# sebhaan/geobo

Measured on AMD Instinct MI355X. Metric: voxels/sec posterior (mean+var) for 64^3 x 2-prop joint inversion; fp64 roofline %, higher is better.
Workload: dtype f64

## Files before the change

geobo_amd/_lib.py:

```python
import ctypes as C
import os

LIB_PATH = os.environ.get("GEOBO_HIP_LIB") or os.path.join(os.path.dirname(os.path.abspath(__file__)), "lib", "libgeobo_hip.so")

_dp = C.c_void_p
_i64 = C.c_int64
_f64 = C.c_double
_int = C.c_int
_sz = C.c_size_t

SIGNATURES = {
    "geobo_version": (_int, []),
    "geobo_pad_m": (_i64, [_i64]),
    "geobo_pad_n": (_i64, [_i64]),
    "geobo_k_block": (_int, [_int, _dp, _dp, _dp, _i64, _dp, _dp, _dp, _i64, _f64, _f64, _f64, _f64, _dp, _i64, _dp]),
    "geobo_k_block_f32": (_int, [_int, _dp, _dp, _dp, _i64, _dp, _dp, _dp, _i64, _f64, _f64, _f64, _f64, _dp, _i64, _dp]),
    "geobo_k_block_grid": (_int, [_int, _int, _int, _dp, _dp, _i64, _i64, _i64, _i64, _int, _dp, _i64, _dp]),
    "geobo_lattice_wbuild": (_int, [_i64, _int, _int, _int, _dp, _dp, _dp, _dp]),
    "geobo_lattice_wplanes": (_int, [_i64, _int, _int, _int, _dp, _dp, _dp, _dp]),
    "geobo_xz2d_fold_inv_strided": (_int, [_int, _i64, _int, _dp, _i64, _i64, _dp, _dp, _dp, _i64, _i64, _i64, _dp]),
    "geobo_xz2d_fold_inv_mul": (_int, [_int, _i64, _int, _dp, _i64, _dp, _i64, _dp, _dp, _dp, _i64, _i64, _i64, _dp]),
    "geobo_xz2d_fold_conv_fwd": (_int, [_int, _i64, _int, _dp, _i64, _dp, _i64, _dp, _i64, _dp, _dp, _dp, _i64, _i64, _dp]),
    "geobo_sumsq_accum": (_int, [_i64, _i64, _dp, _i64, _dp, _i64, _int, _dp, _i64, _dp]),
    "geobo_lamdot_z": (_int, [_i64, _int, _int, _int, _dp, _dp, _dp, _dp]),
    "geobo_centro_fill": (_int, [_dp, _i64, _i64, _i64, _dp]),
    "geobo_transpose": (_int, [_i64, _i64, _dp, _i64, _dp, _i64, _dp]),
    "geobo_mirror_rows": (_int, [_dp, _i64, _i64, _i64, _i64, _int, _dp]),
    "geobo_mirror_dev_ws_bytes": (_sz, []),
    "geobo_mirror_dev": (_int, [_dp, _i64, _dp, _i64, _i64, _int, _int, _dp, _dp, _sz, _dp]),
    "geobo_colgemv_ws_bytes": (_sz, [_i64, _i64]),
    "geobo_colgemv": (_int, [_i64, _i64, _dp, _i64, _dp, _dp, _dp, _sz, _dp]),
    "geobo_rowgemv": (_int, [_i64, _i64, _dp, _i64, _dp, _dp, _dp]),
    "geobo_convert": (_int, [_int, _dp, _i64, _dp, _i64, _i64, _i64, _dp]),
    "geobo_round_f32": (_int, [_dp, _i64, _dp]),
    "geobo_k_eval": (_int, [_int, _dp, _i64, _f64, _f64, _f64, _f64, _dp, _dp]),
    "geobo_a_sens": (_int, [_int, C.POINTER(_f64), _dp, _i64, _int, _int, _int, _dp, _dp, _dp, _f64, _f64, _dp, _i64, _dp]),
    "geobo_a_sens_slab": (_int, [_int, C.POINTER(_f64), _dp, _i64, _int, _int, _int, _dp, _dp, _dp, _f64, _f64, _int, _int, _dp, _i64, _i64, _dp]),
    "geobo_potential": (_int, [_int, C.POINTER(_f64), _dp, _dp, _dp, _i64, _dp, _dp]),
    "geobo_ak_fused": (_int, [_int, _dp, _i64, _i64, _i64, _dp, _dp, _dp, _i64, _i64, _f64, _f64, _f64, _f64, _dp, _i64, _dp]),
    "geobo_ak_points": (_int, [_int, _dp, _i64, _i64, _i64, _dp, _dp, _dp, _dp, _dp, _dp, _i64, _f64, _f64, _f64, _f64, _dp, _i64, _dp]),
    "geobo_cov_table": (_int, [_int, _int, _int, _int, _f64, _f64, _f64, _f64, _f64, _f64, _f64, _dp, _dp]),
    "geobo_ak_fused_grid": (_int, [_dp, _i64, _i64, _i64, _int, _int, _int, _dp, _i64, _i64, _dp, _i64, _dp]),
    "geobo_gemm_nt": (_int, [_i64, _i64, _i64, _f64, _dp, _i64, _dp, _i64, _f64, _dp, _i64, _int, _i64, _dp]),
    "geobo_tile_order": (_i64, [_int, _int, _int, _int, _int, _int, _int, C.POINTER(_int), _i64]),
    "geobo_gemm_map": (_int, [_int, _int, _int, _int, _int, _int, _int, _int, C.POINTER(_int)]),
    "geobo_gemm_nt_splitk": (_int, [_i64, _i64, _i64, _int, _dp, _i64, _dp, _i64, _dp, _i64, _int, _i64, _dp, _sz, _dp]),
    "geobo_gemm_nn": (_int, [_i64, _i64, _i64, _f64, _dp, _i64, _dp, _i64, _f64, _dp, _i64, _int, _int, _dp]),
    "geobo_gemm_batched": (_int, [_int, _i64, _i64, _i64, _f64, _dp, _i64, _i64, _dp, _i64, _i64, _f64, _dp, _i64, _i64, _i64, _i64, _int, _dp]),
    "geobo_gemm_fold_lamdot": (_int, [_i64, _i64, _i64, _dp, _i64, _dp, _i64, _i64, _dp, _int, _i64, _dp, _i64, _dp]),
    "geobo_gemm_fold": (_int, [_int, _int, _i64, _i64, _i64, _dp, _i64, _i64, _dp, _i64, _i64, _dp, _i64, _i64, _i64, _i64, _i64, _dp]),
    "geobo_scale_broadcast": (_int, [_dp, _dp, _i64, _i64, _dp, _dp]),
    "geobo_scale_broadcast2": (_int, [_dp, _dp, _dp, _i64, _i64, _dp, _dp, _dp]),
    "geobo_a_sens_lattice_ws_bytes": (_sz, [_int, _int, _int]),
    "geobo_a_sens_lattice": (_int, [_int, C.POINTER(_f64), _i64, _int, _int, _int, _dp, _dp, _dp, _dp, _dp, _f64, _f64, _int, _int, _dp, _i64,
                                    _i64, _dp, _sz, _dp]),
    "geobo_xz2d": (_int, [_int, _int, _int, _i64, _int, _dp, _i64, _i64, _dp, _i64, _dp, _i64, _dp, _i64, _i64, _dp]),
    "geobo_xz2d_fold": (_int, [_int, _int, _i64, _int, _dp, _i64, _i64, _dp, _dp, _dp, _i64, _i64, _dp]),
    "geobo_xz2d_fold_quad": (_int, [_int, _int, _i64, _int, _dp, _i64, _i64, _dp, _dp, _dp, _i64, _i64, _dp]),
    "geobo_xcorr_reduce_fold": (_int, [_int, _i64, _int, _dp, _i64, _i64, _dp, _dp, _dp, _i64, _i64, _dp]),
    "geobo_xz2d_fold_lattice": (_int, [_int, _i64, _int, _dp, _dp, _i64, _dp, _i64, _dp, _dp, _dp, _i64, _i64, _dp]),
    "geobo_xz2d_fold_inv_ss_slots": (_int, [_int, _i64, _int]),
    "geobo_xz2d_fold_inv_ss": (_int, [_int, _i64, _int, _dp, _i64, _i64, _dp, _i64, _i64, _dp, _dp, _dp, _dp]),
    "geobo_ymul": (_int, [_int, _int, _i64, _i64, _dp, _i64, _dp, _i64, _dp, _i64, _dp]),
    "geobo_ymul_fold": (_int, [_int, _int, _i64, _i64, _dp, _i64, _dp, _i64, _dp, _i64, _dp]),
    "geobo_xcorr_reduce": (_int, [_int, _int, _i64, _int, _dp, _i64, _i64, _dp, _i64, _dp, _dp, _i64, _i64, _dp]),
    "geobo_toeplitz_y": (_int, [_int, _i64, _i64, _i64, _int, _dp, _dp, _dp, _dp, _dp, _int, _int, _dp]),
    "geobo_toeplitz_y2t": (_int, [_int, _i64, _i64, _i64, _dp, _dp, _dp, _dp, _dp, _dp, _dp, _dp, _dp]),
    "geobo_toeplitz_y2s": (_int, [_int, _i64, _i64, _i64, _dp, _dp, _dp, _dp, _dp, _dp, _dp, _dp]),
    "geobo_toeplitz_y3": (_int, [_int, _i64, _i64, _i64, _int, _dp, C.POINTER(_dp), C.POINTER(_dp), _int, _int, _dp]),
    "geobo_toeplitz_y3_add": (_int, [_int, _i64, _i64, _i64, _int, _dp, C.POINTER(_dp), C.POINTER(_dp), _int, _int, _dp]),
    "geobo_spectral_y_basis_doubles": (_i64, [_int]),
    "geobo_spectral_y_basis": (_int, [_int, _dp, _dp]),
    "geobo_spectral_y": (_int, [_int, _i64, _i64, _i64, _int, _dp, _dp, _dp, _dp, _dp, _int, _int, _dp, _dp]),
    "geobo_spectral_y_lattice": (_int, [_int, _i64, _i64, _i64, _int, _dp, _dp, _dp, _i64, _dp, _dp, _dp, _dp, _dp, _int, _int, _dp, _dp]),
    "geobo_spectral_y2s": (_int, [_int, _i64, _i64, _i64, _dp, _dp, _dp, _dp, _dp, _dp, _dp, _dp, _dp]),
    "geobo_spectral_y3": (_int, [_int, _i64, _i64, _i64, _int, _dp, C.POINTER(_dp), C.POINTER(_dp), _int, _int, _int, _dp, _dp]),
    "geobo_spectral_y3t": (_int, [_int, _i64, _i64, _i64, _int, _dp, _dp, C.POINTER(_dp), C.POINTER(_dp), C.POINTER(_dp), _dp, _dp]),
    "geobo_spectral_axis": (_int, [_int, _int, _i64, _i64, _i64, _i64, _i64, _i64, _dp, _dp, _dp, _int, _dp]),
    "geobo_potrf_ws_bytes": (_sz, [_i64]),
    "geobo_potrf_ctx_create": (_int, [C.POINTER(C.c_void_p)]),
    "geobo_potrf_ctx_destroy": (_int, [_dp]),
    "geobo_potrf_inv": (_int, [_i64, _dp, _i64, _dp, _i64, _dp, _dp, _sz, _dp, _int, _dp]),
    "geobo_posterior_ws_bytes": (_sz, [_i64, _i64]),
    "geobo_posterior_reduce": (_int, [_i64, _i64, _dp, _i64, _dp, _i64, _dp, _f64, _dp, _dp, _i64, _dp, _sz, _dp]),
    "geobo_kinv_dot_ws_bytes": (_sz, [_i64, _int]),
    "geobo_kinv_dot": (_int, [_i64, _dp, _i64, _dp, _int, C.POINTER(_dp), _i64, C.POINTER(_i64), _dp, _dp, _sz, _dp]),
    "geobo_philox_fill": (_int, [_int, C.c_uint64, C.c_uint64, _i64, _i64, _i64, _i64, C.c_uint64, _dp, _dp]),
    "geobo_torus_table": (_int, [_int, _int, _int, _int, _f64, _f64, _f64, _f64, _f64, _f64, _f64, _dp, _dp]),
    "geobo_fft_lines": (_int, [_int, _i64]),
    "geobo_fft_axis": (_int, [_int, _i64, _int, _i64, _int, _int, _dp, _dp, _int, _i64, _i64, _dp]),
    "geobo_sample_factor_ws_bytes": (_sz, []),
    "geobo_sample_factor": (_int, [_int, _int, _int, _int, _dp, _dp, _dp, _dp, _sz, _dp, _dp]),
    "geobo_sample_zpass": (_int, [_int, _i64, _i64, _int, _int, _int, _int, _dp, _dp, C.c_uint64, _dp, _dp]),
    "geobo_spectral_mix": (_int, [_int, _i64, _int, _int, _int, _dp, _f64, _dp, _dp, _dp]),
    "geobo_set_gram": (_int, [_i64, _int, _dp, _i64, _dp, _i64, _i64, _int, _dp, _dp]),
    "geobo_set_logdet": (_int, [_i64, _int, _dp, _dp, _i64, _f64, _dp, _dp, _i64, _dp, _dp, _dp]),
    "geobo_kinv_diag_ws_bytes": (_sz, [_i64]),
    "geobo_kinv_diag": (_int, [_i64, _dp, _i64, _dp, _dp, _dp, _dp, _sz, _dp]),
    "geobo_set_loo": (_int, [_i64, _int, _dp, _dp, _dp, _i64, _dp, _dp, _dp, _dp, _dp, _dp]),
    "geobo_block_cov_ws_bytes": (_sz, [_i64, _int, _int, _int, _int, _int, _int]),
    "geobo_block_cov": (_int, [_i64, _dp, _dp, _dp, _i64, _int, _int, _int, _int, _int, _int, _int, _dp, _dp, _sz, _dp]),
    "geobo_box_means": (_int, [_i64, _dp, _i64, _i64, _int, _int, _int, _int, _int, _int, _dp, _dp, _dp]),
    "geobo_cutoff_stats_ws_bytes": (_sz, [_i64, _i64, _int]),
    "geobo_cutoff_stats": (_int, [_i64, _dp, _i64, _i64, _i64, _int, _int, C.POINTER(_f64), C.POINTER(_f64), _dp, _dp, _dp, _dp, _dp, _dp, _sz, _dp]),
    "geobo_bodies_ws_bytes": (_sz, [_i64, _int, _int, _int, _int]),
    "geobo_bodies": (_int, [_i64, _dp, _i64, _i64, _int, _int, _int, _int, _int, C.POINTER(_f64), C.POINTER(_f64), _dp, _dp, _int, _i64, _i64,
                            C.POINTER(C.c_int32), _dp, _dp, _dp, _dp, _dp, _dp, _int, _dp, _sz, _dp]),
    "geobo_trace_stats_ws_bytes": (_sz, [_i64, _i64, _int]),
    "geobo_trace_stats": (_int, [_i64, _dp, _i64, _i64, _int, _int, _int, _int, _int, C.POINTER(_f64), C.POINTER(_f64), _dp, _i64, _dp, _dp, _int,
                                 _int, _int, _dp, _dp, _dp, _dp, _dp, _dp, _dp, _dp, _dp, _dp, _dp, _sz, _dp]),
    "geobo_factor_append": (_int, [_int, _dp, _i64, _dp, _i64, _dp, _dp, _i64, _dp, _i64, _dp, _dp, _dp, _dp]),
    "geobo_rows_downdate": (_int, [_dp, _i64, _i64, _i64, _dp, _dp, _dp, _dp]),
    "geobo_trmv_stats": (_int, [_i64, _dp, _i64, _dp, _dp, _i64, _dp, _dp, _dp]),
    "geobo_mfma_f64_peak": (_int, [_int, _int, _dp, _dp]),
    "geobo_mfma_mix": (_int, [_int, _int, _int, _int, _dp, _dp]),
}


class GeoboHipUnavailable(RuntimeError):
    pass


_lib = None


def load():
    global _lib
    if _lib is not None:
        return _lib
    if not os.path.exists(LIB_PATH):
        raise GeoboHipUnavailable(
            "%s not found. Build the HIP extension first: `python -m geobo_amd.build` "
            "(hipcc --offload-arch=gfx950). There is no CPU fallback for the inversion hot path." % LIB_PATH)
    import torch
    try:
        lib = C.CDLL(LIB_PATH)
    except OSError as e:
        raise GeoboHipUnavailable("cannot load %s: %s" % (LIB_PATH, e)) from e
    for name, (res, args) in SIGNATURES.items():
        try:
            fn = getattr(lib, name)
        except AttributeError as e:
            raise GeoboHipUnavailable("libgeobo_hip.so lacks symbol %s (stale build?)" % name) from e
        fn.restype = res
        fn.argtypes = args
    _lib = lib
    return lib
# ... 9 lines not shown
```

geobo_amd/csrc/xz2d.hip:

```cpp
#include <hip/hip_runtime.h>
#include <atomic>
#include <stdint.h>
#include "geobo_hip.h"
#include "lds_optin.h"

namespace {

typedef double v4d __attribute__((ext_vector_type(4)));
typedef double v2d __attribute__((ext_vector_type(2)));
typedef __attribute__((address_space(3))) void* lds_ptr_t;
typedef const __attribute__((address_space(1))) void* glb_ptr_t;

struct XZArgs {
  const double* in; int64_t in_row, in_plane;
  double* out; int64_t out_row, out_plane;
  const double* Mz; int64_t ldmz;
  const double* Mx; int64_t ldmx;
  int ppr;
  int64_t nplanes;
};

constexpr int RING = 4;

constexpr int vmcnt_imm(int v) { return (v & 15) | (7 << 4) | (15 << 8) | ((v >> 4) << 14); }
// ... 321 lines not shown
        for (int r = 0; r < 4; ++r) {
          if constexpr (FOLD)
            op[(int64_t)(2 * (16 * w + q + 4 * r) + mt) * g.C + 16 * nt] = mt ? acc[0][nt][r] - acc[1][nt][r] : acc[0][nt][r] + acc[1][nt][r];
          else
            op[(int64_t)(32 * w + 16 * mt + q + 4 * r) * g.C + 16 * nt] = acc[mt][nt][r];
        }
  };
  for (; tile < g.ntiles; tile += gridDim.x) {
    __builtin_amdgcn_s_waitcnt(vmcnt_imm(0));
    __builtin_amdgcn_s_barrier();
    const int64_t nxt = tile + gridDim.x;
    if (nxt < g.ntiles) stage(nxt, b ^ 1);
    if (prev_tile >= 0) store(prev, prev_tile);
    v4d acc[2][4];
#pragma unroll
    for (int mt = 0; mt < 2; ++mt)
#pragma unroll
      for (int nt = 0; nt < 4; ++nt) acc[mt][nt] = (v4d){0., 0., 0., 0.};
    if constexpr (FOLD) {
      unsigned xe[4], xo[4];
#pragma unroll
      for (int nt = 0; nt < 4; ++nt) {
        xe[nt] = (unsigned)(uintptr_t)(lds_ptr_t)&xs[b][(2 * q) * CB + 16 * (nt ^ ((2 * q) & 3)) + lr];
        xo[nt] = (unsigned)(uintptr_t)(lds_ptr_t)&xs[b][(2 * q + 1) * CB + 16 * (nt ^ ((2 * q + 1) & 3)) + lr];
      }
      double be[2][4], bo[2][4];
#pragma unroll
      for (int nt = 0; nt < 4; ++nt) {
        asm volatile("ds_read_b64 %0, %1" : "=v"(be[0][nt]) : "v"(xe[nt]));
        asm volatile("ds_read_b64 %0, %1" : "=v"(bo[0][nt]) : "v"(xo[nt]));
      }
#pragma unroll
      for (int t = 0; t < 8; ++t) {
        if (t + 1 < 8) {
#pragma unroll
          for (int nt = 0; nt < 4; ++nt) {
            asm volatile("ds_read_b64 %0, %1 offset:%2" : "=v"(be[(t + 1) & 1][nt]) : "v"(xe[nt]), "n"(8 * (t + 1) * CB * 8));
            asm volatile("ds_read_b64 %0, %1 offset:%2" : "=v"(bo[(t + 1) & 1][nt]) : "v"(xo[nt]), "n"(8 * (t + 1) * CB * 8));
          }
          asm volatile("s_waitcnt lgkmcnt(8)" : "+v"(be[t & 1][0]), "+v"(be[t & 1][1]), "+v"(be[t & 1][2]), "+v"(be[t & 1][3]),
                       "+v"(bo[t & 1][0]), "+v"(bo[t & 1][1]), "+v"(bo[t & 1][2]), "+v"(bo[t & 1][3]));
        } else {
          asm volatile("s_waitcnt lgkmcnt(0)" : "+v"(be[t & 1][0]), "+v"(be[t & 1][1]), "+v"(be[t & 1][2]), "+v"(be[t & 1][3]),
                       "+v"(bo[t & 1][0]), "+v"(bo[t & 1][1]), "+v"(bo[t & 1][2]), "+v"(bo[t & 1][3]));
        }
#pragma unroll
        for (int nt = 0; nt < 4; ++nt) {
          acc[0][nt] = __builtin_amdgcn_mfma_f64_16x16x4f64(a[0][t], be[t & 1][nt], acc[0][nt], 0, 0, 0);
          acc[1][nt] = __builtin_amdgcn_mfma_f64_16x16x4f64(a[1][t], bo[t & 1][nt], acc[1][nt], 0, 0, 0);
        }
      }
    } else {
    unsigned xaddr[4];
#pragma unroll
    for (int nt = 0; nt < 4; ++nt) xaddr[nt] = (unsigned)(uintptr_t)(lds_ptr_t)&xs[b][q * CB + 16 * (nt ^ q) + lr];
    double bv[2][4];
#pragma unroll
    for (int nt = 0; nt < 4; ++nt) asm volatile("ds_read_b64 %0, %1" : "=v"(bv[0][nt]) : "v"(xaddr[nt]));
#pragma unroll
    for (int t = 0; t < 16; ++t) {
      if (t + 1 < 16) {
#pragma unroll
        for (int nt = 0; nt < 4; ++nt)
          asm volatile("ds_read_b64 %0, %1 offset:%2" : "=v"(bv[(t + 1) & 1][nt]) : "v"(xaddr[nt]), "n"(4 * (t + 1) * CB * 8));
        asm volatile("s_waitcnt lgkmcnt(4)" : "+v"(bv[t & 1][0]), "+v"(bv[t & 1][1]), "+v"(bv[t & 1][2]), "+v"(bv[t & 1][3]));
      } else {
        asm volatile("s_waitcnt lgkmcnt(0)" : "+v"(bv[t & 1][0]), "+v"(bv[t & 1][1]), "+v"(bv[t & 1][2]), "+v"(bv[t & 1][3]));
      }
#pragma unroll
      for (int mt = 0; mt < 2; ++mt)
#pragma unroll
        for (int nt = 0; nt < 4; ++nt)
          acc[mt][nt] = __builtin_amdgcn_mfma_f64_16x16x4f64(a[mt][t], bv[t & 1][nt], acc[mt][nt], 0, 0, 0);
    }
    }
#pragma unroll
    for (int mt = 0; mt < 2; ++mt)
#pragma unroll
      for (int nt = 0; nt < 4; ++nt) prev[mt][nt] = acc[mt][nt];
    prev_tile = tile;
    b ^= 1;
  }
  if (prev_tile >= 0) store(prev, prev_tile);
}

}

extern "C" int geobo_xz2d(int inverse, int nx, int nz, int64_t rows, int planes_per_row, const double* in, int64_t in_row,
                          int64_t in_plane, const double* Mx, int64_t ldmx, const double* Mz, int64_t ldmz, double* out,
                          int64_t out_row, int64_t out_plane, void* stream) {
  if (!in || !out || !Mx || !Mz) return GEOBO_E_ARG;
  if (rows <= 0 || planes_per_row <= 0) return GEOBO_OK;
  if ((in_row & 1) || (in_plane & 1) || ((uintptr_t)in & 15)) return GEOBO_E_ALIGN;
  XZArgs g;
  g.in = in; g.in_row = in_row; g.in_plane = in_plane; g.out = out; g.out_row = out_row; g.out_plane = out_plane;
  g.Mz = Mz; g.ldmz = ldmz; g.Mx = Mx; g.ldmx = ldmx; g.ppr = planes_per_row; g.nplanes = rows * planes_per_row;
  hipStream_t st = (hipStream_t)stream;
  if (nz == 32 && nx == 64) {
    return inverse ? launch<128, 64, 64, 32>(g, st) : launch<64, 32, 128, 64>(g, st);
  }
  if (nz != 64) return GEOBO_E_UNSUPPORTED;
  if (!inverse) {
    if (nx == 64) return launch<64, 64, 128, 128>(g, st);
    if (nx == 48) return launch<48, 64, 96, 128>(g, st);
  } else {
    if (nx == 64) return launch<128, 128, 64, 64>(g, st);
    if (nx == 48) return launch<96, 128, 48, 64>(g, st);
  }
  return GEOBO_E_UNSUPPORTED;
}

extern "C" int geobo_xcorr_reduce(int nx, int nz, int64_t rows, int planes, const double* in, int64_t in_row, int64_t in_plane,
                                  const double* Mx, int64_t ldmx, const double* lamT, double* out, int64_t out_row,
                                  int64_t out_plane, void* stream) {
  if (!in || !out || !Mx || !lamT) return GEOBO_E_ARG;
  if (rows <= 0 || planes <= 0) return GEOBO_OK;
  if ((in_row & 1) || (in_plane & 1) || ((uintptr_t)in & 15)) return GEOBO_E_ALIGN;
  if (nx != 64 || nz != 64) return GEOBO_E_UNSUPPORTED;
  XCArgs g;
  g.in = in; g.in_row = in_row; g.in_plane = in_plane; g.Mx = Mx; g.ldmx = ldmx; g.lamT = lamT;
  g.out = out; g.out_row = out_row; g.out_plane = out_plane; g.rows = rows; g.nplanes = rows * planes;
  constexpr int NX = 64, NZ = 64, PX = 128;
  constexpr size_t lds = (size_t)RING * 16 * NZ * 8 + (size_t)NX * (PX + 16) * 8 + 2 * 4 * PX * 8;
  constexpr int NW = 8;
  auto kern = xcorr_kernel<NX, NZ, PX, NW>;
  static std::atomic<uint64_t> attr_done{0};
  if (int rc = ensure_lds_attr(attr_done, kern, lds)) return rc;
  const int64_t nwg = g.nplanes < 1024 ? g.nplanes : 1024;
  hipLaunchKernelGGL(kern, dim3((unsigned)nwg), dim3(64 * NW), lds, (hipStream_t)stream, g);
  return hipGetLastError() == hipSuccess ? GEOBO_OK : GEOBO_E_LAUNCH;
}

extern "C" int geobo_ymul(int m, int k, int64_t C, int64_t rows, const double* G, int64_t ldg, const double* in, int64_t in_row,
                          double* out, int64_t out_row, void* stream) {
  if (!G || !in || !out) return GEOBO_E_ARG;
  if (rows <= 0 || C <= 0) return GEOBO_OK;
  if (m != 128 || k != 64) return GEOBO_E_UNSUPPORTED;
  if (C % 64 || (in_row & 1) || ((uintptr_t)in & 15) || (C & 1)) return GEOBO_E_ALIGN;
  YMulArgs g;
  g.in = in; g.in_row = in_row; g.G = G; g.ldg = ldg; g.out = out; g.out_row = out_row; g.C = C; g.R = rows;
  g.ntiles = rows * (C / 64);
  const int64_t nwg = g.ntiles < 512 ? g.ntiles : 512;
  hipLaunchKernelGGL(ymul_kernel<false>, dim3((unsigned)nwg), dim3(256), 0, (hipStream_t)stream, g);
  return hipGetLastError() == hipSuccess ? GEOBO_OK : GEOBO_E_LAUNCH;
}

extern "C" int geobo_ymul_fold(int m, int k, int64_t C, int64_t rows, const double* G, int64_t ldg, const double* in, int64_t in_row,
                               double* out, int64_t out_row, void* stream) {
  if (!G || !in || !out) return GEOBO_E_ARG;
  if (rows <= 0 || C <= 0) return GEOBO_OK;
  if (m != 128 || k != 64) return GEOBO_E_UNSUPPORTED;
  if (C % 64 || (in_row & 1) || ((uintptr_t)in & 15) || (C & 1)) return GEOBO_E_ALIGN;
  YMulArgs g;
  g.in = in; g.in_row = in_row; g.G = G; g.ldg = ldg; g.out = out; g.out_row = out_row; g.C = C; g.R = rows;
  g.ntiles = rows * (C / 64);
  const int64_t nwg = g.ntiles < 512 ? g.ntiles : 512;
  hipLaunchKernelGGL(ymul_kernel<true>, dim3((unsigned)nwg), dim3(256), 0, (hipStream_t)stream, g);
  return hipGetLastError() == hipSuccess ? GEOBO_OK : GEOBO_E_LAUNCH;
}
```

geobo_amd/csrc/xz2d_fold.hip:

```cpp
#include <hip/hip_runtime.h>
#include <atomic>
#include <stdint.h>
#include <type_traits>
#include "geobo_hip.h"
#include "lds_optin.h"

#ifndef XZF_NT_ST
#define XZF_NT_ST 0
#endif
#ifndef XZF_NT_LD
#define XZF_NT_LD 0
#endif

namespace {

typedef double v4d __attribute__((ext_vector_type(4)));
typedef double v2d __attribute__((ext_vector_type(2)));
typedef __attribute__((address_space(3))) void* lds_ptr_t;
typedef const __attribute__((address_space(1))) void* glb_ptr_t;

struct FoldArgs {
  const double* in; int64_t in_row, in_plane;
  double* out; int64_t out_row, out_plane;
  int64_t out_rs;
  const double* Fz;
  const double* Fx;
  int ppr; int64_t nplanes;
  const int64_t* row_off; const double* edge; int64_t edge_row;
  const double* in2; int64_t in2_row, r2_first; double* ss;
  int in_rowB, in_halfB, in_botB;
  int out_rowB, out_halfB, out_botB;
};

constexpr int vmcnt_imm(int v) { return (v & 15) | (7 << 4) | (15 << 8) | ((v >> 4) << 14); }

__device__ __forceinline__ int rowperm(int i) { return 8 * (i >> 3) + 2 * (i & 3) + ((i >> 2) & 1); }

__device__ __forceinline__ int rowperm4(int i) { return 4 * (i & 3) + (i >> 2); }

template <int I, int E, class F>
__device__ __forceinline__ void static_for(F&& f) {
  if constexpr (I < E) {
    f(std::integral_constant<int, I>{});
    static_for<I + 1, E>(f);
  }
}

template <int N, int RING>
struct FwdCfg {
  static constexpr int NW = 4, RT = N / 16, KP = N / 8, ROWB = N * 8, CHB = 16 * ROWB, ND = CHB / 1024 / NW;
  static constexpr int LPR = ROWB / 16, RPI = 64 / LPR, MT = N / 16;
  static constexpr size_t LDS = (size_t)RING * CHB + (size_t)N * N * 8;
  static_assert(N == 64 && ND >= 1 && RT >= RING - 1 && RT % RING == 0 && N / 16 == NW, "shape");
};

template <int N, bool QUAD>
__global__ void __launch_bounds__(256, 2) xz_fold_fwd_kernel(FoldArgs g) {
  constexpr int RING = 4;
  const int in_rowB = QUAD ? g.in_rowB : N * 8, in_halfB = QUAD ? g.in_halfB : N * 4, in_botB = QUAD ? g.in_botB : 0;
  const int out_rowB = QUAD ? g.out_rowB : 2 * N * 8, out_halfB = QUAD ? g.out_halfB : N * 8, out_botB = QUAD ? g.out_botB : 0;
  using K = FwdCfg<N, RING>;
  constexpr int RT = K::RT, KP = K::KP, MT = K::MT, H = N / 2;
  extern __shared__ __attribute__((aligned(16))) double smem[];
  char* const ring = reinterpret_cast<char*>(smem);
  double* const mxf = smem + RING * K::CHB / 8;
  const unsigned ring_lds = (unsigned)(uintptr_t)(lds_ptr_t)ring;
  const unsigned mxf_lds = ring_lds + RING * K::CHB;
  const int tid = threadIdx.x, lane = tid & 63;
  const int w = __builtin_amdgcn_readfirstlane(tid >> 6);
  const int lr = lane & 15, q = lane >> 4;

  constexpr bool R4 = !QUAD;
  if constexpr (R4) {
    for (int idx = tid; idx < 4 * 16 * 16; idx += 64 * K::NW) {
      const int rho = idx >> 8, om = (idx >> 4) & 15, j = idx & 15, i = 4 * j + rho;
      const double c = g.Fx[(((int64_t)(4 * om) * H + (i >> 1)) << 1) + (i & 1)];
      const double sn = g.Fx[(((int64_t)(4 * om + 1) * H + (i >> 1)) << 1) + (i & 1)];
      *reinterpret_cast<v2d*>(mxf + ((((rho * 16 + om) * 16) + (j ^ om)) << 1)) = (v2d){c, om ? sn : ((j & 1) ? -c : c)};
    }
  } else {
  for (int idx = tid; idx < N * H; idx += 64 * K::NW) {
    const int bx = idx / H, j = idx % H;
    *reinterpret_cast<v2d*>(mxf + ((bx * H + (j ^ (bx & 15))) << 1)) = *reinterpret_cast<const v2d*>(g.Fx + ((int64_t)idx << 1));
  }
  }
  const unsigned fx4 = mxf_lds + lr * 256 + (((lr & 12) | (q ^ (lr & 3))) << 4);
  double gE[KP], gO[KP];
#pragma unroll
  for (int t = 0; t < KP; ++t) {
    const v2d f = *reinterpret_cast<const v2d*>(g.Fz + (((int64_t)(16 * w + lr) * H + 4 * t + q) << 1));
    gE[t] = f.x;
    gO[t] = f.y;
  }
  unsigned raddr[KP];
#pragma unroll
  for (int t = 0; t < KP; ++t) raddr[t] = ring_lds + lr * K::ROWB + (((4 * t + q) ^ lr) << 4);
  unsigned faddr[2][2];
#pragma unroll
  for (int r1 = 0; r1 < 2; ++r1)
#pragma unroll
    for (int h = 0; h < 2; ++h) faddr[r1][h] = mxf_lds + lr * (H * 16) + (((8 * r1 + 4 * h + q) ^ lr) << 4);

  const int64_t first = blockIdx.x, pstep = gridDim.x;
  if (first >= g.nplanes) return;
  const int drow = lane / K::LPR, dpos = lane % K::LPR;
  unsigned doff[K::ND];
#pragma unroll
  for (int j = 0; j < K::ND; ++j) {
    const int row = (w + K::NW * j) * K::RPI + drow;
    const int sl = dpos ^ (row & 15);
    doff[j] = (R4 ? rowperm4(row) : rowperm(row)) * in_rowB + ((sl & (K::LPR / 2 - 1)) << 4) + (sl / (K::LPR / 2)) * in_halfB;
  }
// ... 156 lines not shown
}

template <int KP, int T>
__device__ __forceinline__ void inv_step1(v2d (&a)[KP], const double (&gz)[KP], double sgn, v4d (&d)[4]) {
  asm volatile("s_waitcnt lgkmcnt(%1)" : "+v"(a[T]) : "n"(KP - 1 - T));
  const double uv = __builtin_fma(sgn, a[T].y, a[T].x);
  d[T & 3] = __builtin_amdgcn_mfma_f64_16x16x4f64(uv, gz[T], d[T & 3], 0, 0, 0);
  if constexpr (T + 1 < KP) inv_step1<KP, T + 1>(a, gz, sgn, d);
}

template <int KH, int T, int G0, int KP>
__device__ __forceinline__ void inv_step1h(v2d (&a)[KH], const double (&gz)[KP], double sgn, v4d (&d)[2]) {
  asm volatile("s_waitcnt lgkmcnt(%1)" : "+v"(a[T]) : "n"(KH - 1 - T));
  const double uv = __builtin_fma(sgn, a[T].y, a[T].x);
  d[T & 1] = __builtin_amdgcn_mfma_f64_16x16x4f64(uv, gz[G0 + T], d[T & 1], 0, 0, 0);
  if constexpr (T + 1 < KH) inv_step1h<KH, T + 1, G0, KP>(a, gz, sgn, d);
}

template <int KW, int T, int KP>
__device__ __forceinline__ void inv_step1r(v2d (&a)[KW], const double (&gz)[KP], double sgn, v4d (&d)[2], unsigned xs, int q, int lr) {
  asm volatile("s_waitcnt lgkmcnt(%1)" : "+v"(a[T % KW]) : "n"(T + KW < KP ? KW - 1 : KP - 1 - T));
  const double uv = __builtin_fma(sgn, a[T % KW].y, a[T % KW].x);
  if constexpr (T + KW < KP)
    asm volatile("ds_read_b128 %0, %1" : "=v"(a[T % KW]) : "v"(xs + (((4 * (T + KW) + q) ^ lr) << 4)), "v"(uv));
  d[T & 1] = __builtin_amdgcn_mfma_f64_16x16x4f64(uv, gz[T], d[T & 1], 0, 0, 0);
  if constexpr (T + 1 < KP) inv_step1r<KW, T + 1, KP>(a, gz, sgn, d, xs, q, lr);
}

struct R4Lane {
  double s1, s2, s3;
  double cB, cP, dB, dP, dQ;
  int eP, eQ;
};

__device__ __forceinline__ R4Lane r4_lane(int rho, int q) {
  R4Lane c;
  const double r2 = 1.4142135623730951;
  c.s1 = (rho & 1) ? -1.0 : 1.0;
  c.s2 = rho >= 2 ? -1.0 : 1.0;
  c.s3 = (rho == 1 || rho == 2) ? 1.0 : -1.0;
  c.eP = (rho & 1) ? 3 : 2;
  c.eQ = (rho & 1) ? 2 : 3;
  if (q == 0) {
    c.cB = rho < 2 ? 1.0 : -1.0; c.cP = 0.0; c.dB = 0.0;
    c.dP = rho == 0 ? r2 : rho == 2 ? 0.0 : 1.0;
    c.dQ = rho == 0 ? 0.0 : rho == 1 ? 1.0 : rho == 2 ? r2 : -1.0;
  } else {
    c.cB = 0.0; c.cP = c.s2; c.dB = 1.0; c.dP = 0.0; c.dQ = c.s3;
  }
  return c;
}

template <int T, int SB>
__device__ __forceinline__ void r4_issue(v2d (&oo)[4], unsigned xq, unsigned pP, unsigned pQ) {
  asm volatile("ds_read_b128 %0, %1 offset:%2" : "=v"(oo[0]) : "v"(xq ^ (unsigned)((4 * T) << 4)), "n"(SB));
  asm volatile("ds_read_b128 %0, %1 offset:%2" : "=v"(oo[1]) : "v"(xq ^ (unsigned)((4 * T + 1) << 4)), "n"(SB));
  asm volatile("ds_read_b128 %0, %1 offset:%2" : "=v"(oo[2]) : "v"(xq ^ ((unsigned)((4 * T) << 4) | pP)), "n"(SB));
  asm volatile("ds_read_b128 %0, %1 offset:%2" : "=v"(oo[3]) : "v"(xq ^ ((unsigned)((4 * T) << 4) | pQ)), "n"(SB));
}

template <bool FIRST>
__device__ __forceinline__ void r4_sums(const v2d (&o)[4], const R4Lane& c, double& Cp, double& Sp) {
  const double A_ = __builtin_fma(c.s1, o[0].y, o[0].x), B_ = __builtin_fma(c.s1, o[1].y, o[1].x);
  const double P_ = __builtin_fma(c.s1, o[2].y, o[2].x), Q_ = __builtin_fma(c.s1, o[3].y, o[3].x);
  if constexpr (FIRST) {
    Cp = __builtin_fma(c.cP, P_, __builtin_fma(c.cB, B_, A_));
    Sp = __builtin_fma(c.dQ, Q_, __builtin_fma(c.dP, P_, c.dB * B_));
  } else {
    Cp = __builtin_fma(c.s2, P_, A_);
    Sp = __builtin_fma(c.s3, Q_, B_);
  }
}

template <int N, int RING>
struct InvCfg {
  static constexpr int NW = 4, P = 2 * N, RT = P / 16, KP = N / 4, ROWB = P * 8, CHB = 16 * ROWB, ND = CHB / 1024 / NW;
  static constexpr int LPR = ROWB / 16, RPI = 64 / LPR > 0 ? 64 / LPR : 1, MT = N / 32;
  static constexpr size_t LDS = (size_t)RING * CHB + (size_t)N * N * 8;
  static_assert(N == 64 && ND >= 1 && RT >= RING - 1 && N / 16 == NW && LPR == 64, "shape");
};

template <int N, int MODE, bool QUAD>
__global__ void __launch_bounds__(256, 2) xz_fold_inv_kernel(FoldArgs g) {
  constexpr bool RED = MODE == 1, MUL = MODE == 2;
  const int in_rowB = QUAD ? g.in_rowB : 2 * N * 8, in_halfB = QUAD ? g.in_halfB : N * 8, in_botB = QUAD ? g.in_botB : 0;
  const int out_halfB = QUAD ? g.out_halfB : N * 4, out_botB = QUAD ? g.out_botB : 0;
  constexpr bool R4 = !QUAD;
  constexpr int RING = R4 ? 4 : 3;
  using K = InvCfg<N, RING>;
  constexpr int RT = K::RT, KP = K::KP, MT = K::MT, H = N / 2;
  static_assert((size_t)RING * K::CHB + (R4 ? 16384 : N * N * 8) <= InvCfg<N, 3>::LDS, "LDS");
  extern __shared__ __attribute__((aligned(16))) double smem[];
  char* const ring = reinterpret_cast<char*>(smem);
  double* const mxf = smem + RING * K::CHB / 8;
  const unsigned ring_lds = (unsigned)(uintptr_t)(lds_ptr_t)ring;
  const int tid = threadIdx.x, lane = tid & 63;
  const int w = __builtin_amdgcn_readfirstlane(tid >> 6);
  const int lr = lane & 15, q = lane >> 4;
  const int par = w >> 1, jt = w & 1;

  if constexpr (R4) {
    for (int idx = tid; idx < 4 * 16 * 16; idx += 64 * K::NW) {
      const int rho = idx >> 8, j = (idx >> 4) & 15, om = idx & 15, i = 4 * j + rho;
      const double c = g.Fx[(((int64_t)(4 * om) * H + (i >> 1)) << 1) + (i & 1)];
      const double sn = g.Fx[(((int64_t)(4 * om + 1) * H + (i >> 1)) << 1) + (i & 1)];
      *reinterpret_cast<v2d*>(mxf + ((((rho * 16 + j) * 16) + (om ^ j)) << 1)) = (v2d){c, om ? sn : ((j & 1) ? -c : c)};
    }
  } else {
  for (int idx = tid; idx < N * H; idx += 64 * K::NW) {
    const int bx = idx / H, j = idx % H;
    *reinterpret_cast<v2d*>(mxf + ((j * N + (bx ^ (j & 15))) << 1)) = *reinterpret_cast<const v2d*>(g.Fx + ((int64_t)idx << 1));
  }
  }
  const unsigned fx4 = (unsigned)(uintptr_t)(lds_ptr_t)mxf + lr * 256 + (((lr & 12) | (q ^ (lr & 3))) << 4);
  double gz[R4 ? 1 : KP];
  double gzc[4], gzs[4];
  if constexpr (R4) {
    const int i = 4 * lr + w;
#pragma unroll
    for (int t = 0; t < 4; ++t) {
      const int om = t + 4 * q;
      const double c = g.Fz[(((int64_t)(4 * om) * H + (i >> 1)) << 1) + (i & 1)];
      const double sn = g.Fz[(((int64_t)(4 * om + 1) * H + (i >> 1)) << 1) + (i & 1)];
      gzc[t] = c;
      gzs[t] = om ? sn : ((lr & 1) ? -c : c);
    }
    gz[0] = 0.0;
  } else {
#pragma unroll
    for (int t = 0; t < KP; ++t) gz[t] = g.Fz[(((int64_t)(4 * t + q) * H + 16 * jt + lr) << 1) + par];
  }
  const double sgn = par ? -1.0 : 1.0;
  const R4Lane r4 = r4_lane(w, q);
  const unsigned xq0 = ring_lds + lr * K::ROWB + (unsigned)((q << 8) | (lr << 4));
  unsigned faddr[2][2];
#pragma unroll
  for (int r1 = 0; r1 < 2; ++r1)
#pragma unroll
    for (int h = 0; h < 2; ++h)
      faddr[r1][h] = (unsigned)(uintptr_t)(lds_ptr_t)mxf + lr * (N * 16) + (((8 * r1 + 4 * h + q) ^ lr) << 4);

  const int64_t first = blockIdx.x, pstep = gridDim.x;
  if (first >= g.nplanes) return;
  auto nterms = [&](int64_t p) { return (RED && g.in2 && p / g.ppr >= g.r2_first) ? 2 : 1; };
  auto plane_ptr = [&](int64_t p, int term) {
    const int64_t r = p / g.ppr;
    if (RED && term == 1) return g.in2 + (r - g.r2_first) * g.in2_row + (p % g.ppr) * g.in_plane;
    return g.in + r * g.in_row + (p % g.ppr) * g.in_plane;
  };
  auto stage = [&](const double* plane, int c, int slot) {
#pragma unroll
    for (int j = 0; j < K::ND; ++j) {
      const int row = w + K::NW * j;
      const int sl = lane ^ (row & 15);
      const int mrow = R4 ? 32 * (c >> 1) + 8 * (row & 3) + 4 * (c & 1) + (row >> 2) : 16 * c + rowperm(row);
      const char* src = reinterpret_cast<const char*>(plane) + (int64_t)mrow * in_rowB + (c >= RT / 2 ? in_botB : 0) +
                        ((sl & 31) << 4) + (sl >> 5) * in_halfB;
      __builtin_amdgcn_global_load_lds((glb_ptr_t)src, (lds_ptr_t)(ring + slot * K::CHB + row * 1024), 16, 0, XZF_NT_LD ? 2 : 0);
    }
  };
  using rsrc_t = __amdgpu_buffer_rsrc_t;
  using u32x4 = decltype(__builtin_amdgcn_raw_buffer_load_b128(*static_cast<rsrc_t*>(nullptr), 0, 0, 0));
  auto planeA = [&](int64_t p) {
    return __builtin_amdgcn_make_buffer_rsrc(const_cast<double*>(g.in + (p % g.ppr) * g.in_plane), 0, RT * K::CHB, 0x00020000);
  };
  auto planeB = [&](int64_t p) {
    return __builtin_amdgcn_make_buffer_rsrc(const_cast<double*>(g.in2 + (p / g.ppr) * g.in2_row), 0, RT * K::CHB, 0x00020000);
// ... 106 lines not shown
        d2[0] = d2[1] = (v4d){0., 0., 0., 0.};
#pragma unroll
        for (int t = 0; t < KH; ++t) asm volatile("ds_read_b128 %0, %1" : "=v"(ah[t]) : "v"(xs + (((4 * t + q) ^ lr) << 4)));
        inv_step1r<KH, 0, KP>(ah, gz, sgn, d2, xs, q, lr);
        tc = d2[0] + d2[1];
      } else {
      v4d d[4];
      d[0] = d[1] = d[2] = d[3] = (v4d){0., 0., 0., 0.};
      v2d a[KP];
#pragma unroll
      for (int t = 0; t < KP; ++t) {
        const unsigned addr = xs + (((4 * t + q) ^ lr) << 4);
        asm volatile("ds_read_b128 %0, %1" : "=v"(a[t]) : "v"(addr));
      }
      inv_step1<KP, 0>(a, gz, sgn, d);
      tc = (d[0] + d[1]) + (d[2] + d[3]);
      }
      if constexpr (R4) {
        if constexpr ((c & 1) == 0) {
          tcA = tc;
        } else {
          constexpr int cp = c >> 1;
          v2d f[4];
          const unsigned fa4 = fx4 ^ (unsigned)(cp << 6);
#pragma unroll
          for (int rho = 0; rho < 4; ++rho) asm volatile("ds_read_b128 %0, %1 offset:%2" : "=v"(f[rho]) : "v"(fa4), "n"(rho * 4096));
          const double Ap = tcA[0] + tcA[1], Am = tcA[0] - tcA[1], Bp = tcA[2] + tcA[3], Bm = tcA[2] - tcA[3];
          const double Pp = tc[0] + tc[1], Pm = tc[0] - tc[1], Qp = tc[2] + tc[3], Qm = tc[2] - tc[3];
          double Cs[4] = {Ap + Pp, Am + Qm, Ap - Pp, Am - Qm};
          double Ss[4] = {Bp - Qp, Bm + Pm, Bp + Qp, Bm - Pm};
          if constexpr (cp == 0) {
            const bool w0 = q == 0;
            const double r2 = 1.4142135623730951;
            Cs[0] = w0 ? Ap + Bp : Cs[0]; Cs[1] = w0 ? Am + Bm : Cs[1]; Cs[2] = w0 ? Ap - Bp : Cs[2]; Cs[3] = w0 ? Am - Bm : Cs[3];
            Ss[0] = w0 ? r2 * Pp : Ss[0]; Ss[1] = w0 ? Pm + Qm : Ss[1]; Ss[2] = w0 ? r2 * Qp : Ss[2]; Ss[3] = w0 ? Qm - Pm : Ss[3];
          }
          static_for<0, 4>([&](auto rr) {
            constexpr int rho = decltype(rr)::value;
            asm volatile("s_waitcnt lgkmcnt(%1)" : "+v"(f[rho]) : "n"(3 - rho));
            xe[rho >> 1][rho & 1] = __builtin_amdgcn_mfma_f64_16x16x4f64(f[rho].x, Cs[rho], xe[rho >> 1][rho & 1], 0, 0, 0);
          });
          static_for<0, 4>([&](auto rr) {
            constexpr int rho = decltype(rr)::value;
            xe[rho >> 1][rho & 1] = __builtin_amdgcn_mfma_f64_16x16x4f64(f[rho].y, Ss[rho], xe[rho >> 1][rho & 1], 0, 0, 0);
          });
        }
      } else
      static_for<0, 2>([&](auto hh) {
        constexpr int h = decltype(hh)::value;
        v2d f[MT];
        static_for<0, MT>([&](auto mm) {
          constexpr int m = decltype(mm)::value;
          lds_read_b128<m * 16 * N * 16 + (c >> 1) * 256>(f[m], faddr[c & 1][h]);
        });
        const double u = tc[2 * h] + tc[2 * h + 1], v = tc[2 * h] - tc[2 * h + 1];
        static_for<0, MT>([&](auto mm) {
          constexpr int m = decltype(mm)::value;
          wait_lgkmcnt<MT - 1 - m>(f[m]);
          xe[m][h] = __builtin_amdgcn_mfma_f64_16x16x4f64(f[m].x, u, xe[m][h], 0, 0, 0);
          xo[m][h] = __builtin_amdgcn_mfma_f64_16x16x4f64(f[m].y, v, xo[m][h], 0, 0, 0);
        });
      });
    });
    warm = true;
    slot0 = (slot0 + RT) % RING;
    cur = nxt;
    curA = nxtA;
    curB = nxtB;
    }
    if constexpr (RED && R4) {
#pragma unroll
      for (int m = 0; m < MT; ++m) {
        sse[m] += xe[m][0] * xe[m][0];
        sso[m] += xe[m][1] * xe[m][1];
      }
    } else if constexpr (RED) {
#pragma unroll
      for (int m = 0; m < MT; ++m) {
        const v4d ev = xe[m][0] + xe[m][1], od = xo[m][0] + xo[m][1];
        sse[m] += ev * ev;
        sso[m] += od * od;
      }
    } else {
      if constexpr (MUL) fetch(curA, curB, 2);
      else __builtin_amdgcn_s_waitcnt(vmcnt_imm(0));
      int64_t ors = g.out_rs;
      asm volatile("" : "+s"(ors));
      double* const op = g.out + (p / g.ppr) * g.out_row + (p % g.ppr) * g.out_plane + 2 * q * ors +
                         (R4 ? 4 * lr + w : 2 * lr + par + jt * (out_halfB >> 3));
      if constexpr (R4) {
        double* const op4 = op + (int64_t)(2 * q) * ors;
#pragma unroll
        for (int rho = 0; rho < 4; ++rho)
#pragma unroll
          for (int r = 0; r < 4; ++r) op4[(int64_t)(16 * r + rho) * ors] = xe[rho >> 1][rho & 1][r];
      } else
#pragma unroll
      for (int m = 0; m < MT; ++m) {
        const v4d ev = xe[m][0] + xe[m][1], od = xo[m][0] + xo[m][1];
        double* const om = op + (m >= MT / 2 ? (out_botB >> 3) : 0);
#pragma unroll
        for (int r = 0; r < 4; ++r) {
          const int j0 = 16 * m + 4 * r;
          om[(int64_t)(2 * j0) * ors] = ev[r];
          om[(int64_t)(2 * j0 + 1) * ors] = od[r];
        }
      }
    }
  }
  if constexpr (RED) {
    __builtin_amdgcn_s_waitcnt(vmcnt_imm(0));
    double* const sp = g.ss + ((int64_t)(blockIdx.x / g.ppr) * g.ppr + (first % g.ppr)) * (N * N) + (R4 ? 4 * lr + w : 2 * (16 * jt + lr) + par);
#pragma unroll
    for (int m = 0; m < MT; ++m)
#pragma unroll
      for (int r = 0; r < 4; ++r) {
        if constexpr (R4) {
          const int x0 = 4 * (q + 4 * r) + 2 * m;
          sp[(int64_t)x0 * N] += sse[m][r];
          sp[(int64_t)(x0 + 1) * N] += sso[m][r];
        } else {
        const int j = 16 * m + q + 4 * r;
        sp[(int64_t)(2 * j) * N] += sse[m][r];
        sp[(int64_t)(2 * j + 1) * N] += sso[m][r];
        }
      }
  }
}

#ifndef XZF_CF_RING
#define XZF_CF_RING 3
#endif
#ifndef XZF_CF_NT_ST
#define XZF_CF_NT_ST 1
#endif

template <int N, int RING>
struct ConvFwdCfg {
  using KI = InvCfg<N, RING>;
  using KF = FwdCfg<N, 4>;
  static constexpr size_t RINGB = (size_t)RING * KI::CHB, LDS = RINGB + 2 * 16384;
  static_assert(RING >= 3 && RINGB >= (size_t)KF::RT * KF::CHB && KF::RT == 4 && KI::RT == 8, "the plane overlays the ring");
};

template <int N, int RING>
__global__ void __launch_bounds__(256, 2) xz_conv_fwd_kernel(FoldArgs g) {
  using KC = ConvFwdCfg<N, RING>;
  using KI = typename KC::KI;
  using KF = typename KC::KF;
  constexpr int H = N / 2, RTI = KI::RT, RTF = KF::RT, KPF = KF::KP, ND = KI::ND;
  constexpr int out_rowB = 2 * N * 8;
  extern __shared__ __attribute__((aligned(16))) double smem[];
  char* const ring = reinterpret_cast<char*>(smem);
  double* const mxi = smem + KC::RINGB / 8;
  double* const mxf = mxi + 2048;
  const unsigned ring_lds = (unsigned)(uintptr_t)(lds_ptr_t)ring;
  const int tid = threadIdx.x, lane = tid & 63;
  const int w = __builtin_amdgcn_readfirstlane(tid >> 6);
  const int lr = lane & 15, q = lane >> 4;

  for (int idx = tid; idx < 4 * 16 * 16; idx += 64 * 4) {
    const int rho = idx >> 8, a = (idx >> 4) & 15, b = idx & 15;
    {
      const int j = a, om = b, i = 4 * j + rho;
      const double c = g.Fx[(((int64_t)(4 * om) * H + (i >> 1)) << 1) + (i & 1)];
      const double sn = g.Fx[(((int64_t)(4 * om + 1) * H + (i >> 1)) << 1) + (i & 1)];
      *reinterpret_cast<v2d*>(mxi + ((((rho * 16 + j) * 16) + (om ^ j)) << 1)) = (v2d){c, om ? sn : ((j & 1) ? -c : c)};
    }
    {
      const int om = a, j = b, i = 4 * j + rho;
      const double c = g.Fx[(((int64_t)(4 * om) * H + (i >> 1)) << 1) + (i & 1)];
      const double sn = g.Fx[(((int64_t)(4 * om + 1) * H + (i >> 1)) << 1) + (i & 1)];
      *reinterpret_cast<v2d*>(mxf + ((((rho * 16 + om) * 16) + (j ^ om)) << 1)) = (v2d){c, om ? sn : ((j & 1) ? -c : c)};
    }
  }
  const unsigned fxoff = lr * 256 + (((lr & 12) | (q ^ (lr & 3))) << 4);
  const unsigned fx4i = (unsigned)(uintptr_t)(lds_ptr_t)mxi + fxoff, fx4f = (unsigned)(uintptr_t)(lds_ptr_t)mxf + fxoff;
  double gzc[4], gzs[4];
  {
    const int i = 4 * lr + w;
#pragma unroll
    for (int t = 0; t < 4; ++t) {
      const int om = t + 4 * q;
      const double c = g.Fz[(((int64_t)(4 * om) * H + (i >> 1)) << 1) + (i & 1)];
      const double sn = g.Fz[(((int64_t)(4 * om + 1) * H + (i >> 1)) << 1) + (i & 1)];
      gzc[t] = c;
      gzs[t] = om ? sn : ((lr & 1) ? -c : c);
    }
  }
// ... 425 lines not shown
      ((uintptr_t)Fx & 15) || ((uintptr_t)Fz & 15))
    return GEOBO_E_ALIGN;
  if (n != 32 || in_plane * 8 >= (1ll << 29) || out_plane * 8 >= (1ll << 29)) return GEOBO_E_UNSUPPORTED;
  const int N = 64, h = N / 2;
  FoldArgs g;
  g.in = in; g.in_row = in_row; g.in_plane = 4 * in_plane; g.out = out; g.out_row = out_row; g.out_plane = 4 * out_plane;
  g.Fz = Fz; g.Fx = Fx; g.ppr = groups_per_row; g.nplanes = rows * groups_per_row;
  g.row_off = nullptr; g.edge = nullptr; g.edge_row = 0;
  g.in2 = nullptr; g.in2_row = 0; g.r2_first = 0; g.ss = nullptr;
  if (!inverse) {
    g.out_rs = N;
    g.in_rowB = h * 8; g.in_halfB = (int)(in_plane * 8); g.in_botB = (int)(2 * in_plane * 8) - h * h * 8;
    g.out_rowB = N * 8; g.out_halfB = (int)(out_plane * 8); g.out_botB = (int)(2 * out_plane * 8) - N * N * 8;
    return launch_fwd<64, true>(g, (hipStream_t)stream);
  }
  g.out_rs = h;
  g.in_rowB = N * 8; g.in_halfB = (int)(in_plane * 8); g.in_botB = (int)(2 * in_plane * 8) - N * N * 8;
  g.out_rowB = 0; g.out_halfB = (int)(out_plane * 8); g.out_botB = (int)(2 * out_plane * 8) - h * h * 8;
  return launch_inv<64, 0, true>(g, (hipStream_t)stream);
}

extern "C" int geobo_xz2d_fold_lattice(int n, int64_t rows, int planes_per_row, const double* Q, const int64_t* row_off,
                                       int64_t q_plane, const double* edge, int64_t edge_row, const double* Fx, const double* Fz,
                                       double* out, int64_t out_row, int64_t out_plane, void* stream) {
  if (!Q || !row_off || !edge || !out || !Fx || !Fz) return GEOBO_E_ARG;
  if (rows <= 0 || planes_per_row <= 0) return GEOBO_OK;
  if (planes_per_row < 3) return GEOBO_E_ARG;
  if ((q_plane & 1) || (edge_row & 1) || (out_row & 1) || (out_plane & 1) || ((uintptr_t)Q & 15) || ((uintptr_t)edge & 15) ||
      ((uintptr_t)out & 15) || ((uintptr_t)Fx & 15) || ((uintptr_t)Fz & 15))
    return GEOBO_E_ALIGN;
  if (n != 64) return GEOBO_E_UNSUPPORTED;
  FoldArgs g;
  g.in = Q; g.in_row = 0; g.in_plane = q_plane; g.out = out; g.out_row = out_row; g.out_plane = out_plane;
  g.Fz = Fz; g.Fx = Fx; g.ppr = planes_per_row; g.nplanes = rows * planes_per_row; g.out_rs = n;
  g.row_off = row_off; g.edge = edge; g.edge_row = edge_row;
  g.in2 = nullptr; g.in2_row = 0; g.r2_first = 0; g.ss = nullptr;
  dense_fwd(g, 64);
  return launch_fwd<64>(g, (hipStream_t)stream);
}

extern "C" int geobo_xz2d_fold_inv_ss_slots(int n, int64_t rows, int planes_per_row) {
  if (n != 64 || rows <= 0 || planes_per_row <= 0) return 0;
  const int64_t np = rows * planes_per_row;
  const int64_t nwg = (np < 2048 ? np : 2048) / planes_per_row * planes_per_row;
  return (int)(nwg / planes_per_row);
}

extern "C" int geobo_xz2d_fold_inv_ss(int n, int64_t rows, int planes_per_row, const double* in, int64_t in_row, int64_t in_plane,
                                      const double* in2, int64_t in2_row, int64_t r2_first, const double* Fx, const double* Fz,
                                      double* ss, void* stream) {
  if (!in || !Fx || !Fz || !ss) return GEOBO_E_ARG;
  if (rows <= 0 || planes_per_row <= 0) return GEOBO_OK;
  if (in2 && (r2_first < 0 || r2_first > rows)) return GEOBO_E_ARG;
  if ((in_row & 1) || (in_plane & 1) || (in2_row & 1) || ((uintptr_t)in & 15) || ((uintptr_t)in2 & 15) || ((uintptr_t)Fx & 15) ||
      ((uintptr_t)Fz & 15))
    return GEOBO_E_ALIGN;
  if (n != 64 || planes_per_row > 2048) return GEOBO_E_UNSUPPORTED;
  FoldArgs g;
  g.in = in; g.in_row = in_row; g.in_plane = in_plane; g.out = nullptr; g.out_row = 0; g.out_plane = 0; g.out_rs = n;
  g.Fz = Fz; g.Fx = Fx; g.ppr = planes_per_row; g.nplanes = rows * planes_per_row;
  g.row_off = nullptr; g.edge = nullptr; g.edge_row = 0;
  g.in2 = in2; g.in2_row = in2_row; g.r2_first = in2 ? r2_first : rows; g.ss = ss;
  dense_inv(g, 64);
  return launch_inv<64, 1>(g, (hipStream_t)stream);
}

extern "C" int geobo_xz2d_fold_inv_strided(int n, int64_t rows, int planes_per_row, const double* in, int64_t in_row, int64_t in_plane,
                                           const double* Fx, const double* Fz, double* out, int64_t out_row, int64_t out_plane,
                                           int64_t out_rowstride, void* stream) {
  if (!in || !out || !Fx || !Fz) return GEOBO_E_ARG;
  if (rows <= 0 || planes_per_row <= 0) return GEOBO_OK;
  if (out_rowstride < n) return GEOBO_E_ARG;
  if ((in_row & 1) || (in_plane & 1) || ((uintptr_t)in & 15) || ((uintptr_t)Fx & 15) || ((uintptr_t)Fz & 15)) return GEOBO_E_ALIGN;
  if (n != 64) return GEOBO_E_UNSUPPORTED;
  FoldArgs g;
  g.in = in; g.in_row = in_row; g.in_plane = in_plane; g.out = out; g.out_row = out_row; g.out_plane = out_plane; g.out_rs = out_rowstride;
  g.Fz = Fz; g.Fx = Fx; g.ppr = planes_per_row; g.nplanes = rows * planes_per_row;
  g.row_off = nullptr; g.edge = nullptr; g.edge_row = 0;
  g.in2 = nullptr; g.in2_row = 0; g.r2_first = 0; g.ss = nullptr;
  dense_inv(g, 64);
  return launch_inv<64, 0>(g, (hipStream_t)stream);
}

extern "C" int geobo_xz2d_fold_inv_mul(int n, int64_t rows, int planes_per_row, const double* a, int64_t a_plane, const double* b,
                                       int64_t b_row, const double* Fx, const double* Fz, double* out, int64_t out_row,
                                       int64_t out_plane, int64_t out_rowstride, void* stream) {
  if (!a || !b || !out || !Fx || !Fz) return GEOBO_E_ARG;
  if (rows <= 0 || planes_per_row <= 0) return GEOBO_OK;
  if (out_rowstride < n) return GEOBO_E_ARG;
  if ((a_plane & 1) || (b_row & 1) || ((uintptr_t)a & 15) || ((uintptr_t)b & 15) || ((uintptr_t)Fx & 15) || ((uintptr_t)Fz & 15))
    return GEOBO_E_ALIGN;
  if (n != 64) return GEOBO_E_UNSUPPORTED;
  FoldArgs g;
  g.in = a; g.in_row = 0; g.in_plane = a_plane; g.out = out; g.out_row = out_row; g.out_plane = out_plane; g.out_rs = out_rowstride;
  g.Fz = Fz; g.Fx = Fx; g.ppr = planes_per_row; g.nplanes = rows * planes_per_row;
  g.row_off = nullptr; g.edge = nullptr; g.edge_row = 0;
  g.in2 = b; g.in2_row = b_row; g.r2_first = 0; g.ss = nullptr;
  dense_inv(g, 64);
  return launch_inv<64, 2>(g, (hipStream_t)stream);
}

extern "C" int geobo_xz2d_fold_conv_fwd(int n, int64_t rows, int planes_per_row, const double* a, int64_t a_plane, const double* b,
                                        int64_t b_row, const double* slab, int64_t slab_row, const double* Fx, const double* Fz,
                                        double* out, int64_t out_row, int64_t out_plane, void* stream) {
  if (!a || !b || !out || !Fx || !Fz) return GEOBO_E_ARG;
  if (rows <= 0 || planes_per_row <= 0) return GEOBO_OK;
  if ((a_plane & 1) || (b_row & 1) || (out_row & 1) || (out_plane & 1) || ((uintptr_t)a & 15) || ((uintptr_t)b & 15) ||
      ((uintptr_t)out & 15) || ((uintptr_t)slab & 7) || ((uintptr_t)Fx & 15) || ((uintptr_t)Fz & 15))
    return GEOBO_E_ALIGN;
  if (n != 64) return GEOBO_E_UNSUPPORTED;
  FoldArgs g;
  g.in = a; g.in_row = 0; g.in_plane = a_plane; g.out = out; g.out_row = out_row; g.out_plane = out_plane; g.out_rs = n;
  g.Fz = Fz; g.Fx = Fx; g.ppr = planes_per_row; g.nplanes = rows * planes_per_row;
  g.row_off = nullptr; g.edge = slab; g.edge_row = slab_row;
  g.in2 = b; g.in2_row = b_row; g.r2_first = 0; g.ss = nullptr;
  dense_fwd(g, 64);
  return launch_conv_fwd(g, (hipStream_t)stream);
}
```

geobo_amd/engine.py:

```python
import math
import os
import time

import numpy as np
import torch

from . import geometry, hip
from .plan import COLUMN_FORM_MAX_BYTES, engine_options, plan_route
from .columnform import ColumnExchangeMixin
from .rowform import RowFormMixin
from .operators import StreamedOperator
from .transposed import TransposedPosteriorMixin
from .information import SetStatisticsMixin
from .crossval import CrossValidationMixin
from .blocksupport import BlockSupportMixin
from .pointpred import PointPredictionMixin
from .resources import ResourceMixin
from .geobodies import GeobodyMixin
from .intercepts import InterceptMixin
from .append import AppendRowsMixin
from .step import Prior, Step
from .sharding import (EmulatedGroup, allreduce_sum_, assemble_columns, backend_of, exchange_blocks, exchange_blocks_finish,
                       exchange_blocks_start, gather_rows, gather_slices, shard_columns)

F64 = hip.F64


class CholeskyError(RuntimeError):

    def __init__(self, info):
        super().__init__("Cholesky failed at pivot %d" % info)
        self.info = info


class FactorisationTimeout(RuntimeError):
    """The persistent tile-DAG factorisation gave up on a hand-off (info = -7: a spin ran into its 4 s wall-clock bound -- a device
    shared with other processes can do that); the result is undefined.  Inversion retries the step once on the stream schedule."""


class _LastStep(dict):
    complete = None

    def __getitem__(self, key):
        if key == "AK_partial" and self.complete is not None:
            fill, self.complete = self.complete, None
            fill()
        return dict.__getitem__(self, key)


def create_cov_lengths(gplength):
    p = np.asarray(gplength)
    if p[1] == p[0]:
        p[1] = 1.01 * p[0]
    if p[2] == p[0]:
        p[1] = 1.02 * p[0]
    if p[2] == p[1]:
        p[2] = 1.01 * p[1]
    return p


def weight_matrix(crossweights):
    w1, w2, w3 = [float(v) for v in np.asarray(crossweights)]
    return [[1.0, w3, w1], [w3, 1.0, w2], [w1, w2, 1.0]]


WEIGHT_PAIRS = ((0, 2), (1, 2), (0, 1))

_XGROUPS = {}


def _exchange_group(ranks, backend):
    key = (ranks, backend)
    if key not in _XGROUPS:
        _XGROUPS[key] = torch.distributed.new_group(ranks=list(ranks), backend=backend)
    return _XGROUPS[key]


def lattice_gram_form(exchange, chunked, world, Ms, c0, c1, plane, N):
    if exchange and not chunked:
        return "rows" if (Ms // world) % 128 == 0 else None
    Ly = (c1 - c0) // plane
    if world > 4 or (c1 - c0) % plane or Ly % 16 or c1 > N or Ly <= 0:
        return None
    return "columns"


def _on_device(fn):
    import functools

    @functools.wraps(fn)
    def wrapper(self, *args, **kw):
        with torch.cuda.device(self.device):
            return fn(self, *args, **kw)
    return wrapper


class PosteriorEngine(RowFormMixin, TransposedPosteriorMixin, ColumnExchangeMixin, SetStatisticsMixin, CrossValidationMixin, BlockSupportMixin,
                      PointPredictionMixin, ResourceMixin, GeobodyMixin, InterceptMixin, AppendRowsMixin):
    def __init__(self, settings, device=None, rank=0, world=1, group=None, profile=False, method="auto", assembly="f64",
                 operators="resident"):
        hip.require_gpu()
        if assembly not in ("f64", "f32") or operators not in ("resident", "streamed", "auto"):
            raise ValueError("assembly must be 'f64' or 'f32', operators 'resident', 'streamed' or 'auto'")
        self.f32 = assembly == "f32"
        self.streamed = operators == "streamed"
        self.auto_ops = operators == "auto"
        self.s = settings
        self.device = torch.device(device if device is not None else "cuda:%d" % torch.cuda.current_device())
        if self.device.type != "cuda":
            raise ValueError("PosteriorEngine needs a CUDA (ROCm) device, got %r" % (device,))
        if self.device.index is None:
            self.device = torch.device("cuda:%d" % torch.cuda.current_device())
        self.rank, self.world, self.group = rank, world, group
        self.profile = profile
        self.timings = {}
        s = settings
        self.nx, self.ny, self.nz = int(s.xNcube), int(s.yNcube), int(s.zNcube)
        self.N = self.nx * self.ny * self.nz
        self.N_pad = hip.pad_n(self.N)
        self.Ms = self.nx * self.ny
        self.Ms_pad = hip.pad_m(self.Ms)
        self.c0, self.c1 = shard_columns(self.N_pad, world, rank)
        self.nc = self.c1 - self.c0
        self._xyz = None
        self._A = {}
        self._ws = {}
        self._host = {}
        self._auto_denied = set()
        self._pending_exchange = None
        self.use_grid = self.nz >= 16 and self.nz % 2 == 0
        if method not in ("auto", "dense", "spectral"):
            raise ValueError("method must be 'auto', 'dense' or 'spectral'")
        self.method = method
        env = os.environ
        self.route = plan_route(self.nx, self.ny, self.nz, world=world, rank=rank, assembly=assembly, operators=operators, method=method,
                                env=env)
        self.options = engine_options(env)
        self.use_spectral = self.route.spectral
        if method == "spectral" and not self.use_spectral:
            raise ValueError("spectral method needs grid extents % 16 == 0 and column shards on y-slab boundaries")
        if self.route.operators == "streamed":
            self.streamed = True
        if self.route.note and self.N >= 32768:
            import warnings
            warnings.warn("geobo_amd route %s: %s" % (self.route.describe(), self.route.note), RuntimeWarning, stacklevel=3)
        self._spectral = None
        self._lattice_plan = None
        self._gram, self._lam, self._edgeV = None, {}, {}
        self._lamW, self._edgeVt = {}, {}
        self.aka_mirror_on = self.options.aka_mirror
        self.aka_mirror, self._mirror, self._mirror_meas = {}, {}, None
        self.z_spectrum_on = self.options.z_spectrum
        self.rows_static = self.route.rows
        self.exchange = self.route.exchange
        self._deny = {}
        self.step_route = None
        self._step = None
        self.last = None
        if self.streamed and not self.use_spectral:
            raise ValueError("streamed operators feed the spectral product: needs the spectral method's grid conditions")
        self._xgroup = group
        self.async_exchange = self.options.async_exchange
        if (self.exchange and self.options.exchange_comm == "own" and self.async_exchange
                and not isinstance(group, EmulatedGroup) and torch.distributed.is_available() and torch.distributed.is_initialized()):
            ranks = torch.distributed.get_process_group_ranks(group) if group is not None else list(range(torch.distributed.get_world_size()))
            if len(ranks) == world:
                self._xgroup = _exchange_group(tuple(ranks), torch.distributed.get_backend(group))
        self._Arows, self._Aedge, self._rowsrc, self._op_args = {}, {}, {}, {}
        self._slab_ops = set()
        self._potrf_ctx = None
        self.force_collectives = self.options.force_collectives
        self.kernel_events = None
        self.aka_hook = None

    def grid_points(self):
        if self._xyz is None:
            s = self.s
            xr = np.arange(1, self.nx + 1) * s.xvoxsize
            yr = np.arange(1, self.ny + 1) * s.yvoxsize
            zr = np.arange(1, self.nz + 1) * s.zvoxsize
            X, Y, Z = np.meshgrid(xr, yr, zr)
            out = []
            for a in (X, Y, Z):
                v = np.empty(self.N_pad)
                v[:self.N] = a.ravel()
                v[self.N:] = v[self.N - 1]
                out.append(hip.to_dev(v, self.device))
            self._xyz = tuple(out)
        return self._xyz

    def node_axes(self):
        return geometry.node_axes(self.s)

    @_on_device
    def operator(self, func, sensor_locations, B=None, axes=None, full=False):
        s = self.s
        loc = np.ascontiguousarray(sensor_locations, dtype=np.float64)
        assert loc.shape == (self.Ms, 3), "A_sens handles exactly xNcube*yNcube sensors (sensormodel.py:54,58)"
        xe, ye, ze = self.node_axes() if axes is None else axes
        skey = (loc.tobytes(), xe.tobytes(), ye.tobytes(), ze.tobytes())
        if self._lattice_plan is None or self._lattice_plan[0] != skey:
            self._lattice_plan = (skey, hip.lattice_plan(loc, xe, ye, ze, self.nx, self.ny, self.nz, self.device))
        plan = self._lattice_plan[1]
        Bkey = None if B is None else tuple(np.asarray(B, dtype=float))
        if self._deny.get("survey", (skey,))[0] != skey:
            self._allow_rows("survey")
        if self._deny.get(func, ((skey, Bkey),))[0] != (skey, Bkey):
            self._allow_rows(func)
        if self.rows_static and not self._rows_denied and not full and (plan is None or not plan["rowmajor"]):
            self._deny_rows("survey", skey, "the survey is not a row-major x-y lattice of the cube")
        rows_mode = self.rows_static and not self._rows_denied and not full
        self._op_args[func] = (sensor_locations, B, axes)
        partial = self.exchange and not full and not rows_mode
        dkey = (func, Bkey, None if plan is None else self._lattice_plan[0])
        stream_it = (self.streamed or (self.auto_ops and dkey not in self._auto_denied and self._implicit_operators_pay(plan))) and not full
        if rows_mode and self.auto_ops and not stream_it and self.world == 1 and not self.route.single:
            stream_it = True
        key = (func, loc.tobytes(), Bkey, partial, stream_it, rows_mode)
        if key in self._A:
            return self._A[key]
# ... 235 lines not shown
        if not self.profile:
            return None
        torch.cuda.synchronize(self.device)
        now = time.perf_counter()
        if t0 is not None:
            self.timings[name] = self.timings.get(name, 0.0) + (now - t0)
        return now

    @property
    def _rowpath(self):
        return self._step is not None and self._step.rowpath

    def _new_step(self, prior, props, sel_t, noise, **kw):
        Md = 0 if sel_t is None else sel_t.numel()
        return Step(prior, tuple(props), sel_t, Md, hip.pad_m(2 * self.Ms_pad + Md), noise, **kw)

    def _assemble_AK(self, step, A_g, A_m):
        xyz = self.grid_points()
        props, sel_t, Md, M_pad = step.props, step.sel_t, step.Md, step.M_pad
        off_d = 2 * self.Ms_pad
        nc = self.nc
        step.rowpath = False
        if self.rows_static:
            self._spectral_product()
            if self._rows_agree(self._rows_ok(A_g, A_m)):
                self._finish_exchange()
                step.rowpath = True
                step.fullrows = {}
                return None
        ak_bytes = M_pad * len(props) * nc * (4 if self.f32 else 8)
        if ak_bytes > COLUMN_FORM_MAX_BYTES and self.use_spectral:
            raise RuntimeError("A K of this grid would take %.0f GB on this rank and only the row form avoids it (%s)"
                               % (ak_bytes / 1e9, self.route.note or "GEOBO_ROWS=0 / GEOBO_POSTERIOR=dense switch it off"))
        AK = self._workspace2d(step.ak_slot, M_pad, len(props) * nc, dtype=hip.F32 if self.f32 else F64)
        for r0, r1 in ((self.Ms, self.Ms_pad), (self.Ms_pad + self.Ms, off_d), (off_d + Md, M_pad)):
            if r1 > r0:
                AK[r0:r1].zero_()
        if self.c1 > self.N:
            for jj in range(len(props)):
                AK[:, jj * nc + max(self.N - self.c0, 0):(jj + 1) * nc].zero_()
        if self.use_spectral:
            self._assemble_AK_spectral(step, AK, A_g, A_m)
        for jj, j in enumerate(props):
            cols = slice(jj * nc, (jj + 1) * nc)
            for s_, A in ((0, A_g), (1, A_m)):
                if self.use_spectral:
                    break
                out = AK[s_ * self.Ms_pad:(s_ + 1) * self.Ms_pad, cols]
                out64 = out if not self.f32 else self._workspace2d("ak_block64", self.Ms_pad, nc)
                if self.use_grid:
                    tab = step.prior.table(self, s_, j)
                    self._timed("ak_fused_grid", 2.0 * self.Ms_pad * self.N_pad * nc,
                                lambda: hip.ak_fused_grid(A, self.nx, self.ny, self.nz, tab, self.c0, nc, out64),
                                alg=2.0 * self.Ms * self.N * min(nc, max(self.N - self.c0, 0)))
                else:
                    self._timed("ak_fused", 2.0 * self.Ms_pad * self.N_pad * nc,
                                lambda: step.prior.ak_fused(self, s_, j, A, xyz, nc, out64),
                                alg=2.0 * self.Ms * self.N * min(nc, max(self.N - self.c0, 0)))
                if self.f32:
                    hip.convert(out64, out)
            if Md:
                self._cov_rows(step.prior, 2, j, sel_t, self.c0, AK[off_d:off_d + Md, cols])
        return AK

    def _cov_rows(self, prior, i, j, rows_t, col0, out):
        ncv = min(out.shape[1], max(self.N - col0, 0))
        if ncv <= 0:
            return out
        if self.use_grid and col0 % 2 == 0:
            tab = prior.table(self, i, j)
            return hip.k_block_grid(tab, self.nx, self.ny, self.nz, rows_t, col0, out[:, :ncv])
        xyz = self.grid_points()
        rows = tuple(c[rows_t] for c in xyz)
        colc = tuple(c[col0:col0 + out.shape[1]] for c in xyz)
        return prior.k_block(self, i, j, rows, colc, out)

    def _assemble_AK_spectral(self, step, AK, A_g, A_m):
        sp, nc, props = self._spectral_product(), self.nc, step.props
        plane = self.nx * self.nz
        y0, y1 = self.c0 // plane, self.c1 // plane
        if self.exchange:
            return self._assemble_AK_spectral_exchange(step, AK)
        for s_, A in ((0, A_g), (1, A_m)):
            lams, outs = [], []
            for jj, j in enumerate(props):
                gen = sp.eigenvalues(step.prior.table(self, s_, j))
                step.gens[(s_, j)] = gen
                if step.sym and (s_, j) not in ((0, 0), (0, 1), (1, 1)):
                    continue
                lams.append(gen)
                outs.append(AK[s_ * self.Ms_pad:s_ * self.Ms_pad + self.Ms, jj * nc:(jj + 1) * nc])
            pooled = (isinstance(A, StreamedOperator) and A.lattice is not None and A.lattice.jy is not None and not self.f32
                      and sp.pool_applies())
            Mrun = step.mirror if (s_ == 1 and step.mirror) else self.Ms
            fl = sp.flops(Mrun, len(lams), y1 - y0, fwd_planes=sp.pool_planes(Mrun) if pooled else None)
            fv = sp.flops_valu(Mrun, len(lams), y1 - y0)
            if not self.f32 and not isinstance(A, StreamedOperator):
                self._timed("spectral_product", fl, lambda: sp.product(A, Mrun, lams, [o[:Mrun] for o in outs], y0, y1), valu=fv)
                continue

            def batches():
                Rb = sp.R
                abuf = self._op_rows_buffer() if isinstance(A, StreamedOperator) else None
                scr = [self._workspace2d("ak_rows64_%d" % jj, Rb, nc) for jj in range(len(lams))] if self.f32 else None
                pool = sp.plane_pool(A.lattice, Mrun, A.lattice.jy, A.lattice.jx) if pooled else None
                for r0 in range(0, Mrun, Rb):
                    R = min(Rb, Mrun - r0)
                    if pool is not None:
                        src = pool.rows(r0)
                    elif abuf is not None and A.lattice is not None:
                        src = A.lattice.rows(r0)
                    else:
                        src = A.rows_into(abuf, r0, R) if abuf is not None else A[r0:r0 + R]
                    dst = [b[:R] for b in scr] if scr is not None else [o[r0:r0 + R] for o in outs]
                    sp.product(src, R, lams, dst, y0, y1)
                    if scr is not None:
                        for jj in range(len(lams)):
                            hip.convert(dst[jj], outs[jj][r0:r0 + R])
            self._timed("spectral_product", fl, batches, valu=fv)

    def _edge_spectrum(self, func, k, ycols):
        key = (func, k)
        hit = self._edgeV.get(key)
        if hit is None or hit[0] != ycols.data_ptr():
            hit = self._edgeV[key] = (ycols.data_ptr(), self._gram.edge_eigen(ycols))
        return hit[1]

    MIRROR_BOUND = 2.0 ** -48

    def _mirror_static(self, plan):
        return bool(self.aka_mirror_on and plan is not None and plan["rowmajor"] and self.route.family == "single" and self.world == 1
                    and not self.exchange and not self.f32 and self.Ms_pad == self.Ms)

    def _mirror_record(self, func, A, mirror):
        meas, self._mirror_meas = self._mirror_meas, None
        if mirror is None or meas is None:
            return
        dq, mq, de, me = meas
        scale = max(mq, me)
        ok = bool(dq <= self.MIRROR_BOUND * scale and de <= self.MIRROR_BOUND * scale and scale > 0.0)
        self._mirror[func] = (A, ok)
        self.aka_mirror[func] = dict(deviation=max(dq, de) / scale if scale > 0.0 else float("nan"), bound=self.MIRROR_BOUND,
                                     table=(dq, mq), slabs=(de, me), symmetric=ok, taken=False)

    def _mirror_rows(self, step, A_m):
        hit = self._mirror.get("magn")
        if not (self.aka_mirror_on and step.sym and hit is not None and hit[0] is A_m and hit[1] and 1 in step.props):
            return 0
        R = self._spectral_product().R
        return min(self.Ms, ((self.Ms + 1) // 2 + R - 1) // R * R)

    def _gram_eigen(self, plan, lws, rows=False, mirror=None):
        from .lattice_gram import LatticeGram
        plane = self.nx * self.nz
        Ly = (self.c1 - self.c0) // plane
        if (not self.use_spectral or not plan["rowmajor"] or self.Ms_pad != self.Ms
                or not LatticeGram.supported(self.nx, self.ny, self.nz) or not self.route.opt("aka_lattice")):
            return None
        if not rows:
            if not LatticeGram.fast(self.nx, self.ny, self.nz):
                return None
            form = lattice_gram_form(self.exchange, self.f32 or self.streamed, self.world, self.Ms, self.c0, self.c1, plane, self.N)
            if form is None:
                return None
        if self._gram is None:
            self._gram = LatticeGram(self._spectral_product(), self.device)
        if mirror is None:
            return self._timed("aka_lattice_eigen", 0.0, lambda: self._gram.eigen(hip.a_sens_lattice_stencil(lws, self.nx, self.ny, self.nz)))
        Q, E0, E1 = mirror

        def measured():
            nqx, ws = 2 * self.nx - 1, self._workspace("mirror_ws", (hip.mirror_dev_ws_doubles(),))
            out = self._workspace("mirror_out", (4,))
            Q2 = Q.view(2 * self.ny - 3, nqx * self.nz)
            hip.mirror_dev(Q2, Q2, 2 * self.ny - 3, nqx, self.nz, out=out[0:2], ws=ws)
            hip.mirror_dev(E0, E1, self.Ms, self.nx, self.nz, out=out[2:4], ws=ws)
            lam = self._gram.eigen(Q, extra=out)
            self._mirror_meas = tuple(self._gram.extra_host)
            return lam
        return self._timed("aka_lattice_eigen", 0.0, measured)

    def _assemble_AkA(self, step, AK, A_g, A_m):
        nc = self.nc
        props, Md, M_pad = step.props, step.Md, step.M_pad
        off_d = 2 * self.Ms_pad
        AkA = self._workspace(step.aka_slot, (M_pad, M_pad))
        AkA.zero_()
        if step.rowpath or (self._row_gram() and step.fullrows):
            return self._assemble_AkA_rows(step, AkA)
        if step.sym:
            return self._assemble_AkA_sym(step, AkA, AK, A_g, A_m)
        for s_, A in ((0, A_g), (1, A_m)):
            jj = props.index(s_)
            r0 = s_ * self.Ms_pad
            rows = M_pad - r0
            tiles = sum(min(2 * (bi + 1), self.Ms_pad // 128) for bi in range(rows // 256))
            splits = 1
            for cand in ((8, 4, 2) if tiles < 512 else (4, 2)):
                if nc % (16 * cand) == 0 and nc // cand >= 2048 and tiles < 4096:
                    splits = cand
                    break
            streamed = isinstance(A, StreamedOperator)
# ... 132 lines not shown
            ctx=self._potrf_ctx, schedule=potrf_schedule or self.options.potrf), alg=(2 * self.Ms + len(sel)) ** 3 * 2.0 / 3.0)
        L = AkA
        self._finish_exchange()
        u, stats = hip.trmv_stats(Linv, y, L)
        t = self._tick("cholesky", t)
        out = dict(info=0, M_pad=M_pad, lengths=[float(v) for v in lengths])

        def check_factor():
            h_info = self._to_host_async(info, "info")
            st = self._to_host_async(stats, "stats") if calclogl else None
            resid = getattr(self._spectral, "sym_residual", None)
            h_res = self._to_host_async(resid.reshape(1), "sym_residual") if resid is not None else None
            if resid is not None:
                self._spectral.sym_residual = None
            torch.cuda.current_stream(self.device).synchronize()
            info_h = int(h_info[0])
            if info_h == -7:
                raise FactorisationTimeout("geobo_potrf_inv: the tile DAG timed out on a hand-off (info = -7)")
            if info_h != 0:
                raise CholeskyError(info_h)
            if h_res is not None:
                if not float(h_res[0]) <= 1e-12:
                    raise RuntimeError("the covariance blocks (0, 1) and (1, 0) differ (relative %.3e): this prior is not symmetric; "
                                       "set GEOBO_Y2S=0 for the four-product y stage" % float(h_res[0]))
            if calclogl:
                out["uu"], out["logdet"] = float(st[0]), float(st[1])
                out["logl"] = -0.5 * (st[0] + st[1] + self.N * math.log(2 * math.pi))
            else:
                out["logl"] = 0.0
        mv = None
        if not want_mean_var:
            check_factor()
        if want_mean_var and step.rowpath:
            mu_f, var_f = self._posterior_rows(step, Linv, u)
            mv = (mu_f, var_f, self.N)
            N_ = len(props) * self.N
            hq = self._to_host_async(torch.cat([mu_f.reshape(-1)[:N_], var_f.reshape(-1)[:N_]]), 0)
            check_factor()
            t = self._tick("posterior", t)
            out["mu"], out["var"] = self._results_to_host(mu_f, var_f, props, queued=hq)
            self._tick("d2h", t)
        elif want_mean_var:
            Mv = 2 * self.Ms_pad + len(sel)
            fl = 2.0 * AK.shape[1] * sum(64.0 * 64 * g + 2560.0 for g in range((Mv + 63) // 64))
            Mu = 2 * self.Ms + len(sel)
            nv = len(props) * min(self.nc, max(self.N - self.c0, 0))
            zp = self._zpath_ok(step, AK)
            if step.sym and not zp:
                raise RuntimeError("internal: A K was assembled for the transposed posterior, which is not available")
            if zp:
                mu_l, var_l = self._posterior_zpath(step, Linv, AK, u, A_g, A_m)
            elif AK.dtype == F64:
                mu_l, var_l = self._timed("posterior_reduce", fl, lambda: hip.posterior_reduce(
                    Linv, AK, u, gp_amp * 1.0, self._workspace("post_ws", (hip.posterior_ws_doubles(M_pad, AK.shape[1]),)), m_valid=Mv),
                    alg=(1.0 * Mu * Mu + 4.0 * Mu) * nv)
            else:
                ncols = AK.shape[1]
                pw = max(128, min(ncols, int((3 << 30) // (8 * M_pad)) // 128 * 128))

                def panels():
                    ws = self._workspace("post_ws", (hip.posterior_ws_doubles(M_pad, pw),))
                    parts = [hip.posterior_reduce(Linv, self._panel64("post_panel64", AK[:, cs:min(ncols, cs + pw)], cols=pw), u,
                                                  gp_amp * 1.0, ws, m_valid=Mv) for cs in range(0, ncols, pw)]
                    return torch.cat([p[0] for p in parts]), torch.cat([p[1] for p in parts])
                mu_l, var_l = self._timed("posterior_reduce", fl, panels, alg=(1.0 * Mu * Mu + 4.0 * Mu) * nv)
            one = self.world == 1 and self.N == self.N_pad
            mv = (mu_l, var_l, self.nc) if self.world == 1 else None
            N_ = len(props) * self.N
            hq = self._to_host_async(torch.cat([mu_l.reshape(-1)[:N_], var_l.reshape(-1)[:N_]]), 0) if one else None
            check_factor()
            t = self._tick("posterior", t)
            if one:
                out["mu"], out["var"] = self._results_to_host(mu_l, var_l, props, queued=hq)
            else:
                mu = assemble_columns(gather_slices(mu_l, len(props), self.N_pad, self.world, self.group), props, self.N,
                                      self.N_pad, self.world, to_host=self._to_host)
                var = assemble_columns(gather_slices(var_l, len(props), self.N_pad, self.world, self.group), props, self.N,
                                       self.N_pad, self.world, to_host=self._to_host)
                out["mu"], out["var"] = mu, var
            self._tick("d2h", t)
        whole = AK is not None and not step.sym
        self.last = _LastStep(L=L, Linv=Linv, u=u, AK=AK if whole else None, AK_partial=None if whole else AK, AK_complete=whole, props=props,
                              sel=sel, ops=(A_g, A_m), step=step, mv=mv, uu=out.get("uu"), logdet=out.get("logdet"))
        if step.mirror and step.mirror < self.Ms:
            jj, nc, Msp, Mm = props.index(1), self.nc, self.Ms_pad, step.mirror
            self.last.complete = lambda: hip.mirror_rows(AK[Msp:Msp + self.Ms, jj * nc:jj * nc + self.N], self.Ms, Mm, self.nx * self.ny, self.nz)
        return out

    def _derivative_gram(self, A_g, A_m, sel_t, prior, slot):
        step = self._new_step(prior, (0, 1, 2), sel_t, None, ak_slot="dK_AK", aka_slot=slot,
                              sym=not self.rows_static and self._sym_ok(A_g, A_m))
        return self._assemble_AkA(step, self._assemble_AK(step, A_g, A_m), A_g, A_m)

    @_on_device
    def logl_grad(self, A_g, A_m, sel, y_g, y_m, y_d, lengths, crossweights, kernelfunc, gp_sigma, gp_amp, directions,
                  potrf_schedule=None):
        if self.world > 1:
            raise ValueError("logl_grad runs on one rank (world = %d): the multi-rank gradient is not implemented" % self.world)
        if self.f32:
            raise ValueError("logl_grad needs the fp64 assembly (assembly='f32' keeps fp32 covariance tables)")
        directions = [np.asarray(d, dtype=float).reshape(3) for d in directions]
        if len(directions) > 3:
            raise ValueError("at most three length directions per evaluation")
        props = (0, 1, 2)
        r = self.posterior(A_g, A_m, sel, y_g, y_m, y_d, lengths, crossweights, kernelfunc, gp_sigma, gp_amp=gp_amp, props=props,
                           calclogl=True, want_mean_var=False, keep_K=True, potrf_schedule=potrf_schedule)
        W = weight_matrix(crossweights)
        Linv, u = self.last["Linv"], self.last["u"]
        M_pad = Linv.shape[0]
        sel = np.asarray(sel, dtype=np.int64)
        sel_t = torch.as_tensor(sel, device=self.device) if sel.size else None
        alpha = hip.colgemv(Linv, u, ws=self._workspace("grad_colgemv_ws", (hip.colgemv_ws_doubles(M_pad, M_pad),)))
        G0 = self._workspace("K_signal", (M_pad, M_pad))
        wvals = [W[a][b] for a, b in WEIGHT_PAIRS]
        if any(w == 0.0 for w in wvals):
            Wu = [[0.0] * 3 for _ in range(3)]
            for (a, b), w in zip(WEIGHT_PAIRS, wvals):
                if w == 0.0:
                    Wu[a][b] = Wu[b][a] = 1.0
            G0.add_(self._derivative_gram(A_g, A_m, sel_t, Prior(kernelfunc, lengths, Wu, gp_amp), "dK_unit"))
        Gs = [G0] + [self._derivative_gram(A_g, A_m, sel_t, Prior(kernelfunc, lengths, W, gp_amp, deriv=d), "dK_dir%d" % t)
                     for t, d in enumerate(directions)]
        segs = ((0, self.Ms), (self.Ms_pad, self.Ms_pad + self.Ms), (2 * self.Ms_pad, 2 * self.Ms_pad + len(sel)))
        out = self._timed("kinv_dot", M_pad ** 3 / 3.0, lambda: hip.kinv_dot(
            Linv, alpha, Gs, segs, ws=self._workspace("kinv_dot_ws", (hip.kinv_dot_ws_doubles(M_pad, len(Gs)),))))
        o = self._to_host(out, "kinv_dot").reshape(len(Gs), 3, 3).copy()
        pair = lambda t, a, b: float(o[t, a, b])
        diag = sum(pair(0, a, a) for a in range(3))
        d_w = np.empty(3)
        off = 0.0
        for k, ((a, b), w) in enumerate(zip(WEIGHT_PAIRS, wvals)):
            if w == 0.0:
                d_w[k] = 0.5 * pair(0, a, b)
            else:
                d_w[k] = 0.5 * pair(0, a, b) / w
                off += pair(0, a, b)
        d_dir = np.array([0.5 * sum(pair(t, a, b) for a in range(3) for b in range(a, 3)) for t in range(1, len(Gs))])
        return dict(uu=r["uu"], logdet=r["logdet"], d_amp=0.5 * (diag + off) / gp_amp, d_w=d_w, d_dir=d_dir)

    @_on_device
    def posterior_covariance(self, kernelfunc, lengths, crossweights, gp_amp=1.0, limit_bytes=48 << 30):
        last = getattr(self, "last", None)
        if last is not None and not last.get("AK_complete", True):
            raise RuntimeError("full covariance needs A K from the last posterior(), and this step kept only the blocks AkA needs "
                               "(symmetric / row form of the transposed order): rerun with GEOBO_POSTERIOR=dense for predict3(full_cov=True)")
        if last is None or tuple(last["props"]) != (0, 1, 2) or self.world != 1 or last["AK"].dtype != F64:
            raise RuntimeError("full covariance needs a single-rank fp64 posterior() with all three property blocks")
        n3 = 3 * self.N_pad
        if n3 * n3 * 8 * 2 > limit_bytes:
            raise MemoryError("full posterior covariance of %d voxels needs %.1f GB; use the diagonal (np.diag(cov))"
                              % (self.N, n3 * n3 * 8 / 1e9))
        W = weight_matrix(crossweights)
        Linv, AK = last["Linv"], last["AK"]
        M_pad = Linv.shape[0]
        V = torch.empty((M_pad, n3), dtype=F64, device=self.device)
        hip.gemm_nn(Linv, AK, V, x_lower=True)
        Vt = V.t().contiguous()
        del V
        C = torch.empty((n3, n3), dtype=F64, device=self.device)
        xyz = self.grid_points()
        for i in range(3):
            for j in range(3):
                hip.k_block(hip.kernel_id(kernelfunc, i != j), xyz, xyz, lengths[i], lengths[j], W[i][j], gp_amp,
                            C[i * self.N_pad:(i + 1) * self.N_pad, j * self.N_pad:(j + 1) * self.N_pad])
        hip.gemm_nt(Vt, Vt, C, alpha=-1.0, beta=1.0)
        idx = torch.cat([torch.arange(self.N, device=self.device) + j * self.N_pad for j in range(3)])
        return C[idx][:, idx].cpu().numpy()

    def _operator_rows(self, A, rows=256, slot="cond_op_rows"):
# ... 56 lines not shown
```

geobo_amd/hip.py:

```python
import ctypes as C

import numpy as np
import torch

from . import _lib

F64 = torch.float64

KERNEL_IDS = {"d2": 0, "exp": 1, "exp_x": 2, "matern32": 3, "matern32_x": 4, "sparse": 5, "sparse_x": 6,
              "exp_dl": 7, "exp_x_dl1": 8, "exp_x_dl2": 9, "matern32_dl": 10, "matern32_x_dl1": 11, "matern32_x_dl2": 12,
              "sparse_dl": 13, "sparse_x_dl1": 14, "sparse_x_dl2": 15}
FUNC_IDS = {"grav": 0, "magn": 1}
from .plan import (PAD_M, PAD_N, SPECTRAL_AXIS_N, SPECTRAL_Y3T_NY, SPECTRAL_Y_NY, TOEPLITZ_ADD_NY, TOEPLITZ_NY, TOEPLITZ_Y2T_NY,
                   XZ2D_FOLD_N, XZ2D_SHAPES, YMUL_SHAPES)


def kernel_id(name, cross, deriv=None):
    if name not in ("exp", "matern32", "sparse"):
        raise ValueError("unknown kernelfunc %r (expected 'sparse', 'exp' or 'matern32')" % (name,))
    if deriv is None:
        return KERNEL_IDS[name + ("_x" if cross else "")]
    if isinstance(deriv, bool) or deriv not in (1, 2):
        raise ValueError("deriv must be None, 1 or 2, got %r" % (deriv,))
    if not cross:
# ... 471 lines not shown
        _lib.check(lib.geobo_gemm_batched((1 if y_is_kn else 0) | (X_KM if x_km else 0), int(m), int(n), int(k), float(alpha),
                                          C.c_void_p(X.data_ptr() + done * strideX * esz), int(ldx), int(strideX),
                                          C.c_void_p(Y.data_ptr() + done * strideY * esz), int(ldy), int(strideY), float(beta),
                                          C.c_void_p(C_.data_ptr() + done * strideC * esz), int(ldc), int(strideC),
                                          int(m_valid), int(n_valid), int(nb), _stream()), "geobo_gemm_batched")
        done += nb
    return C_


def scale_broadcast(a, b, out):
    lib = require_gpu()
    _lib.check(lib.geobo_scale_broadcast(_p(_chk(a, "a")), _p(_chk(b, "b")), a.numel(), b.numel(), _p(out), _stream()),
               "geobo_scale_broadcast")
    return out


def scale_broadcast2(a, b0, b1, out0, out1):
    lib = require_gpu()
    _lib.check(lib.geobo_scale_broadcast2(_p(_chk(a, "a")), _p(_chk(b0, "b0")), _p(_chk(b1, "b1")), a.numel(), b0.numel(),
                                          _p(out0), _p(out1), _stream()), "geobo_scale_broadcast2")




def xz2d(inverse, nx, nz, rows, ppr, src, in_row, in_plane, Mx, Mz, out, out_row, out_plane):
    lib = require_gpu()
    _lib.check(lib.geobo_xz2d(1 if inverse else 0, int(nx), int(nz), int(rows), int(ppr), _p(_chk(src, "src")), int(in_row),
                              int(in_plane), _p(_chk(Mx, "Mx")), int(Mx.stride(0)), _p(_chk(Mz, "Mz")), int(Mz.stride(0)),
                              _p(_chk(out, "out")), int(out_row), int(out_plane), _stream()), "geobo_xz2d")




def xz2d_fold(inverse, n, rows, ppr, src, in_row, in_plane, Fx, Fz, out, out_row, out_plane):
    lib = require_gpu()
    _lib.check(lib.geobo_xz2d_fold(1 if inverse else 0, int(n), int(rows), int(ppr), _p(_chk(src, "src")), int(in_row), int(in_plane),
                                   _p(_chk(Fx, "Fx")), _p(_chk(Fz, "Fz")), _p(_chk(out, "out")), int(out_row), int(out_plane), _stream()),
               "geobo_xz2d_fold")


def xz2d_fold_quad(inverse, n, rows, groups, src, in_row, in_plane, Fx, Fz, out, out_row, out_plane):
    lib = require_gpu()
    _lib.check(lib.geobo_xz2d_fold_quad(1 if inverse else 0, int(n), int(rows), int(groups), _p(_chk(src, "src")), int(in_row), int(in_plane),
                                        _p(_chk(Fx, "Fx")), _p(_chk(Fz, "Fz")), _p(_chk(out, "out")), int(out_row), int(out_plane), _stream()),
               "geobo_xz2d_fold_quad")


def xz2d_fold_inv_ss_slots(n, rows, ppr):
    return _lib.load().geobo_xz2d_fold_inv_ss_slots(int(n), int(rows), int(ppr))


def xz2d_fold_inv_ss(n, rows, ppr, src, in_row, in_plane, Fx, Fz, ss, src2=None, in2_row=0, r2_first=0):
    lib = require_gpu()
    assert _chk(ss, "ss").numel() >= xz2d_fold_inv_ss_slots(n, rows, ppr) * ppr * n * n
    _lib.check(lib.geobo_xz2d_fold_inv_ss(int(n), int(rows), int(ppr), _p(_chk(src, "src")), int(in_row), int(in_plane),
                                          _p(_chk(src2, "src2")) if src2 is not None else None, int(in2_row), int(r2_first),
                                          _p(_chk(Fx, "Fx")), _p(_chk(Fz, "Fz")), _p(ss), _stream()), "geobo_xz2d_fold_inv_ss")


def tile_rows(m, m_valid, tile=256, group=64):
    m_valid = m if not m_valid or m_valid > m else m_valid
    out = []
    for r0 in range(0, m, tile):
        v = min(max(m_valid - r0, 0), tile)
        out.append((v + group - 1) // group * group)
    return out


def xz2d_fold_lattice(n, rows, ppr, Q, row_off, q_plane, edge, edge_row, Fx, Fz, out, out_row, out_plane):
    lib = require_gpu()
    assert row_off.dtype == torch.int64 and row_off.is_contiguous() and row_off.numel() >= rows
    _lib.check(lib.geobo_xz2d_fold_lattice(int(n), int(rows), int(ppr), _p(_chk(Q, "Q")), row_off.data_ptr(), int(q_plane),
                                           _p(_chk(edge, "edge")), int(edge_row), _p(_chk(Fx, "Fx")), _p(_chk(Fz, "Fz")),
                                           _p(_chk(out, "out")), int(out_row), int(out_plane), _stream()), "geobo_xz2d_fold_lattice")




def ymul(m, k, C, rows, G, src, in_row, out, out_row, fold=False):
    lib = require_gpu()
    fn, name = (lib.geobo_ymul_fold, "geobo_ymul_fold") if fold else (lib.geobo_ymul, "geobo_ymul")
    _lib.check(fn(int(m), int(k), int(C), int(rows), _p(_chk(G, "G")), int(G.stride(0)), _p(_chk(src, "src")), int(in_row),
                  _p(_chk(out, "out")), int(out_row), _stream()), name)


def xcorr_reduce(nx, nz, rows, planes, src, in_row, in_plane, Mx, lam, out, out_row, out_plane):
    lib = require_gpu()
    _lib.check(lib.geobo_xcorr_reduce(int(nx), int(nz), int(rows), int(planes), _p(_chk(src, "src")), int(in_row), int(in_plane),
                                      _p(_chk(Mx, "Mx")), int(Mx.stride(0)), _p(_chk(lam, "lam")), _p(_chk(out, "out")),
                                      int(out_row), int(out_plane), _stream()), "geobo_xcorr_reduce")


def xcorr_reduce_fold(n, rows, planes, src, in_row, in_plane, F, lam, out, out_row, out_plane):
    lib = require_gpu()
    _lib.check(lib.geobo_xcorr_reduce_fold(int(n), int(rows), int(planes), _p(_chk(src, "src")), int(in_row), int(in_plane),
                                           _p(_chk(F, "F")), _p(_chk(lam, "lam")), _p(_chk(out, "out")), int(out_row), int(out_plane),
                                           _stream()), "geobo_xcorr_reduce_fold")


def a_sens_lattice_stencil(ws, nx, ny, nz):
    np_ = (2 * ny - 2) * (2 * nx) * (nz + 1)
    return ws[np_:np_ + (2 * ny - 3) * (2 * nx - 1) * nz].view(2 * ny - 3, 2 * nx - 1, nz)






def toeplitz_y(ny, C, R, src, tabs, outs, y0=0, y1=None, plane=None, accumulate=False):
    lib = require_gpu()
    y1 = ny if y1 is None else y1
    n = len(tabs)
    assert 1 <= n <= 3 and len(outs) == n
    tp, op = _ptrs(tabs, "tab"), _ptrs(outs, "out")
    fn, name = (lib.geobo_toeplitz_y3_add, "geobo_toeplitz_y3_add") if accumulate else (lib.geobo_toeplitz_y3, "geobo_toeplitz_y3")
    _lib.check(fn(int(ny), int(C), int(C if plane is None else plane), int(R), n, _p(_chk(src, "src")), tp, op, int(y0), int(y1), _stream()), name)




def toeplitz_y2t(ny, C, R, src_g, src_m, tabs_g, tabs_m, outs, plane=None):
    lib = require_gpu()
    assert len(tabs_g) == 2 and len(tabs_m) == 2 and len(outs) == 2
    _lib.check(lib.geobo_toeplitz_y2t(int(ny), int(C), int(C if plane is None else plane), int(R), _p(_chk(src_g, "src_g")), _p(_chk(src_m, "src_m")),
                                      _p(_chk(tabs_g[0], "tab")), _p(_chk(tabs_g[1], "tab")), _p(_chk(tabs_m[0], "tab")), _p(_chk(tabs_m[1], "tab")),
                                      _p(_chk(outs[0], "out")), _p(_chk(outs[1], "out")), _stream()), "geobo_toeplitz_y2t")


def toeplitz_y2s(ny, C, R, src_g, src_m, tab_d0, tab_x, tab_d1, outs, plane=None):
    lib = require_gpu()
    assert len(outs) == 2
    _lib.check(lib.geobo_toeplitz_y2s(int(ny), int(C), int(C if plane is None else plane), int(R), _p(_chk(src_g, "src_g")), _p(_chk(src_m, "src_m")),
                                      _p(_chk(tab_d0, "tab")), _p(_chk(tab_x, "tab")), _p(_chk(tab_d1, "tab")),
                                      _p(_chk(outs[0], "out")), _p(_chk(outs[1], "out")), _stream()), "geobo_toeplitz_y2s")


_spectral_y_basis = {}


def spectral_y_basis(ny, device=None):
    lib = require_gpu()
    dev = torch.cuda.current_device() if device is None else torch.device(device).index
    b = _spectral_y_basis.get((ny, dev))
    if b is None:
        n = int(lib.geobo_spectral_y_basis_doubles(int(ny)))
        if n <= 0:
            raise RuntimeError("geobo_spectral_y: ny = %d is not instantiated" % ny)
        b = torch.empty(n, dtype=F64, device="cuda:%d" % dev)
        _lib.check(lib.geobo_spectral_y_basis(int(ny), _p(b), _stream()), "geobo_spectral_y_basis")
        _spectral_y_basis[(ny, dev)] = b
    return b


def spectral_y(ny, C, R, src, tabs, outs, y0=0, y1=None, plane=None, accumulate=False):
    lib = require_gpu()
    y1 = ny if y1 is None else y1
    n = len(tabs)
    assert 1 <= n <= 3 and len(outs) == n
    tp, op = _ptrs(tabs, "tab"), _ptrs(outs, "out")
    _lib.check(lib.geobo_spectral_y3(int(ny), int(C), int(C if plane is None else plane), int(R), n, _p(_chk(src, "src")), tp, op, int(y0), int(y1),
                                     1 if accumulate else 0, _p(spectral_y_basis(ny, src.device)), _stream()), "geobo_spectral_y3")


def spectral_y_lattice(ny, C, R, pool, row_off, edge, edge_row, order, tabs, outs, y0=0, y1=None, plane=None):
    lib = require_gpu()
    y1 = ny if y1 is None else y1
# ... 598 lines not shown
```

geobo_amd/lattice_gram.py:

```python
import numpy as np

import torch

from . import hip

F64 = hip.F64


class LatticeGram:
    def __init__(self, sp, device):
        self.sp, self.device = sp, device
        self.nx, self.ny, self.nz = sp.nx, sp.ny, sp.nz
        self.Px, self.Py = sp.Px, sp.Py
        gy0 = sp.G["y"].clone()
        gy0[:, 0] = 0.0
        gy0[:, self.ny - 1] = 0.0
        self.Gy0 = gy0
        per_row = self.Py * self.Px * self.nz * 8
        self.R = self.Rz = 256 if self.fast(self.nx, self.ny, self.nz) else max(8, min(256, (2 << 30) // per_row))
        self.J = (self.ny + 63) // 64 * 64
        self._lam_oz = {}

    EDGE_ROWS = 1024

# ... 132 lines not shown
            hip.lattice_wplanes(Rb, Py, Px, nz, lam3, lh, W)
            hip.xz2d_fold_inv_strided(ny, Rb, nz, W, nz * Py * Px, Py * Px, sp.F["y"], sp.F["x"], out[r0:], out.stride(0), nx, nz * nx)

    def edge_eigen_t(self, E):
        nx, ny, nz, J = self.nx, self.ny, self.nz, self.J
        Kc_s, Ks_s, K64 = self._edge_spectra(E)
        spare = (hip.pad_n(2 * nz) - 2 * nz + 2 * nz - 1) // (2 * nz)
        Vt = torch.zeros((nx + max(spare, 1), 2, nz, 2, J), dtype=F64, device=self.device)
        Kc_t, Ks_t = Kc_s.transpose(1, 2), Ks_s.transpose(1, 2)
        Vt[1:nx, 0, :, 0, :ny], Vt[1:nx, 0, :, 1, :ny] = Kc_t[1:], -Ks_t[1:]
        Vt[1:nx, 1, :, 0, :ny], Vt[1:nx, 1, :, 1, :ny] = Ks_t[1:], Kc_t[1:]
        Vt[0, 0, :, 0, :ny] = Kc_t[0]
        Vt[0, 1, :, 1, :ny] = K64.t()
        return Vt.view(-1, 2 * nz, 2 * J)

    def edge_apply_transpose(self, Lrows, nrows, Vt, out, zx=False):
        nx, ny, nz, sp, J = self.nx, self.ny, self.nz, self.sp, self.J
        RB = self.EDGE_ROWS
        F2, FiT = self._edge_consts()
        nyp, nxp, nzp = hip.pad_n(ny), hip.pad_n(nx), hip.pad_n(nz)
        assert Lrows.stride(1) == 1 and Lrows.stride(0) % 2 == 0 and out.stride(1) == 1
        end = Lrows.storage_offset() + (nrows - 1) * Lrows.stride(0) + nyp * nx
        if end > Lrows.untyped_storage().nbytes() // 8:
            Lc = sp.buf("LG_EX", nrows * ny * nx + nyp * nx)[:nrows * ny * nx].view(nrows, ny * nx)
            Lc.copy_(Lrows[:nrows, :ny * nx])
            Lrows = Lc
        for r0 in range(0, nrows, RB):
            R = min(RB, nrows - r0)
            Rp = (R + 127) // 128 * 128
            Lh = sp.buf("LG_EXh", RB * 2 * nx * max(nz, J))
            if ny < J:
                Lh.zero_()
            hip.gemm_batched(False, hip.pad_n(2 * nx), nyp, nx, F2, nx, 0, Lrows[r0:], nx, Lrows.stride(0), Lh, J, 2 * nx * J, 2 * nx, ny, R)
            o2 = sp.buf("LG_EO2", nx * 2 * max(J, nz) * RB)
            if zx:
                hip.gemm_batched(False, hip.pad_n(2 * nz), Rp, 2 * J, Vt, 2 * J, 2 * nz * 2 * J, Lh, 2 * nx * J, 2 * J, o2, Rp, 2 * nz * Rp, 2 * nz, R, nx)
                hip.gemm_batched(False, Rp, nxp, 2 * nx, o2, nz * Rp, Rp, FiT, 2 * nx, 0, out[r0:], out.stride(0), nx, R, nx, nz, x_km=True)
            else:
                hip.gemm_batched(False, Rp, hip.pad_n(2 * nz), 2 * J, Lh, 2 * nx * J, 2 * J, Vt, 2 * J, 2 * nz * 2 * J, o2, 2 * nx * nz, 2 * nz, R, 2 * nz, nx)
                hip.gemm_batched(True, nxp, nzp, 2 * nx, FiT, 2 * nx, 0, o2, nz, 2 * nx * nz, out[r0:], nz, out.stride(0), nx, nz, R)

    @staticmethod
    def fast(nx, ny, nz):
        from .plan import lattice_gram_fast
        return lattice_gram_fast(nx, ny, nz)

    @staticmethod
    def supported(nx, ny, nz):
        from .plan import lattice_gram_supported
        return lattice_gram_supported(nx, ny, nz)

    def eigen(self, Q, tol=1e-11, extra=None):
        nx, ny, nz, Px, Py = self.nx, self.ny, self.nz, self.Px, self.Py
        cy, cx = ny - 2, nx - 1
        sp = self.sp
        Qh = sp.buf("LG_Qh", ny * nx * nz)[:ny * nx * nz].view(ny, nx, nz)
        Qh.zero_()
        Qh[:ny - 1] = Q[cy:cy + ny - 1, cx:cx + nx]
        dev = [Q.abs().max()]
        for sy, sx in ((-1, 1), (1, -1), (-1, -1)):
            ys = torch.arange(0, ny - 1, device=self.device) * sy + cy
            xs = torch.arange(0, nx, device=self.device) * sx + cx
            dev.append((Q[ys][:, xs] - Qh[:ny - 1]).abs().max())
        dev = torch.stack(dev)
        dev = (dev if extra is None else torch.cat([dev, extra.reshape(-1)])).tolist()
        dev, self.extra_host = dev[:4], dev[4:]
        if max(dev[1:]) > tol * dev[0]:
            return None
        T = sp.buf("LG_T", ny * Px * nz)
        hip.gemm_batched(True, hip.pad_n(Px), hip.pad_n(nz), nx, sp.E["x"], nx, 0, Qh, nz, nx * nz, T, nz, Px * nz, Px, nz, ny)
        lam = torch.empty(Py * Px * nz + 4096, dtype=F64, device=self.device)
        hip.gemm_batched(True, hip.pad_n(Py), hip.pad_n(Px * nz), ny, sp.E["y"], ny, 0, T, Px * nz, 0, lam, Px * nz, 0, Py, Px * nz, 1)
        lam[:Py * Px * nz].mul_(1.0 / float(Py * Px))
        return lam[:Py * Px * nz].view(Py, Px, nz).transpose(1, 2).contiguous().view(-1)

    def flops(self, rows, Ly=None):
        nx, ny, nz, Px, Py = self.nx, self.ny, self.nz, self.Px, self.Py
        Ly = ny if Ly is None else Ly
        f = self.sp.forms.gram_x == "fold"
        h = hb = 0.25 if f else 1.0
        zsum = 0.0 if self.fast(nx, ny, nz) else 2.0 * Py * Px * nz
        hy = 0.5 if (f and Ly in self.sp.forms.ymul_slabs) else 1.0
        return rows * (2.0 * (hy * hip.pad_n(Py) * nx * nz * Ly + h * Py * Px * nx * nz + hb * (ny * Py * Px + ny * nx * Px)) + zsum)

    def gram_rows(self, X, nrows, lam, out, y0=0, y1=None):
        nx, ny, nz, Px, Py = self.nx, self.ny, self.nz, self.Px, self.Py
        y1 = ny if y1 is None else y1
        Ly = y1 - y0
        assert Ly % 16 == 0
        sp, f = self.sp, self.sp.forms
        plane = nx * nz
        assert X.stride(1) == 1 and out.stride(1) == 1 and X.stride(0) % 2 == 0 and out.stride(0) % 2 == 0
        gy = self.Gy0[:, y0:]
        for r0 in range(0, nrows, self.R):
            R = min(self.R, nrows - r0)
            y1b = sp.buf("LG_Y1", R * Py * plane)
            if Ly in f.ymul_slabs and plane % 64 == 0:
                hip.ymul(Py, Ly, plane, R, gy, X[r0:], X.stride(0), y1b, Py * plane, fold=f.fold and y0 % 2 == 0)
            elif f.gram_y_axis4 and y0 == 0 and Ly == ny and plane % 16 == 0 and 2 * ny * plane * 8 < (1 << 31) and X.stride(0) >= ny * plane:
                hip.spectral_axis(False, ny, plane, plane, plane, X.stride(0), Py * plane, R, X[r0:], y1b, mask_ends=True)
            else:
                hip.axis_pass(f.fold and y0 % 2 == 0, True, False, hip.pad_n(Py), hip.pad_n(plane), Ly, gy, ny, 0, X[r0:], plane, X.stride(0),
                              y1b, plane, Py * plane, Py, plane, R)
            s = sp.buf("LG_S", R * Py * Px)
            if f.gram_x == "fold":
                hip.xcorr_reduce_fold(nx, R, Py, y1b, Py * plane, plane, sp.F["x"], lam, s, Py * Px, Px)
            elif f.gram_x == "plain":
                hip.xcorr_reduce(nx, nz, R, Py, y1b, Py * plane, plane, sp.G["x"], lam, s, Py * Px, Px)
            elif f.gram_x == "fold_lamdot":
                hip.gemm_fold_lamdot(Px, nz, nx, sp.G["x"], nx, y1b, nz, plane, self.lam_oz(lam), Py, s, R * Py)
            else:
                D = sp.buf("LG_D", R * Py * Px * nz)
                hip.axis_pass(f.fold, True, False, hip.pad_n(Px), hip.pad_n(nz), nx, sp.G["x"], nx, 0, y1b, nz, plane, D, nz, Px * nz, Px, nz, R * Py)
                hip.lamdot_z(R * Py, Py, Px, nz, D, self.lam_oz(lam), s)
            self._plane_yx(True, R, s, Py * Px, out[r0:], out.stride(0))

    def lam_oz(self, lam):
        hit = self._lam_oz.get(lam.data_ptr())
        if hit is None or hit[0] is not lam:
            self._lam_oz = {k: v for k, v in self._lam_oz.items() if v[0] is not lam}
            if len(self._lam_oz) > 4:
                self._lam_oz = {}
            hit = self._lam_oz[lam.data_ptr()] = (lam, lam.view(self.Py, self.nz, self.Px).transpose(1, 2).contiguous().view(-1))
        return hit[1]
```

geobo_amd/plan.py:

```python
from dataclasses import asdict, dataclass, make_dataclass

PAD_M, PAD_N = 256, 128
XZ2D_SHAPES = ((48, 64), (64, 64), (64, 32))
XZ2D_FOLD_N = (64,)
TOEPLITZ_NY = (16, 32, 48, 64, 80, 96, 112, 128)
SPECTRAL_AXIS_N = (80, 96, 112, 128)
SPECTRAL_Y_NY = (32, 48, 64, 80, 96, 112, 128)
TOEPLITZ_Y2T_NY = (32, 48, 64)
TOEPLITZ_ADD_NY = (80, 96, 112, 128)
SPECTRAL_Y3T_NY = (80, 96, 112, 128)
YMUL_SHAPES = ((128, 64),)
INTEGER_BASIS_N = (32, 64)
ROWS_MIN_VOXELS = 1 << 18
ROWS_MIN_PLANE = 96 * 96
ROWS_MIN_VOXELS_MID, ROWS_MIN_PLANE_MID = 3 << 17, 64 * 64
COLUMN_FORM_MAX_BYTES = 160 << 30
ROWS_MIN_VOXELS_FUSED = 1 << 17


SWITCHES = {"fused_xz": "GEOBO_SPECTRAL_FUSED_XZ",
            "fold": "GEOBO_XZ_FOLD",
            "quad": "GEOBO_XZ_QUAD",
            "dense_y": "GEOBO_SPECTRAL_DENSE_Y",
            "y_mfma": "GEOBO_Y_MFMA",
            "axis_mfma": "GEOBO_AXIS_MFMA",
            "y2s": "GEOBO_Y2S",
            "z_fused": "GEOBO_Z_FUSED",
            "z_mul": "GEOBO_Z_MUL",
            "z_lattice": "GEOBO_Z_LATTICE",
            "aka_lattice": "GEOBO_AKA_LATTICE"}


def switches(env=None):
    env = {} if env is None else env
    return {k: env.get(v, "1") != "0" for k, v in SWITCHES.items()}


_on = lambda v: v != "0"
ENGINE_OPTIONS = {"aka_mirror": ("GEOBO_AKA_MIRROR", True, _on),
                  "z_spectrum": ("GEOBO_Z_SPECTRUM", True, _on),
                  "async_exchange": ("GEOBO_ASYNC_EXCHANGE", True, _on),
                  "exchange_comm": ("GEOBO_EXCHANGE_COMM", "shared", str),
                  "force_collectives": ("GEOBO_FORCE_COLLECTIVES", False, lambda v: v == "1"),
                  "row_chunk": ("GEOBO_ROW_CHUNK", 0, int),
                  "potrf": ("GEOBO_POTRF", "auto", lambda v: "dag" if v[:1] == "d" else "streams")}
EngineOptions = make_dataclass("EngineOptions", [(k, type(d)) for k, (_, d, _p) in ENGINE_OPTIONS.items()], frozen=True)


def engine_options(env=None):
    env = {} if env is None else env
    return EngineOptions(**{k: parse(env[var]) if var in env else default for k, (var, default, parse) in ENGINE_OPTIONS.items()})


def half_integer(n):
    return n not in INTEGER_BASIS_N


@dataclass(frozen=True)
class Forms:
    xz: str
    x_axis4: bool
    y: str
    y_two_term: str
    y3t: bool
    y2s: bool
    fold: bool
    ss: str
    lattice_feed: bool
    plane_yx: str
    gram_x: str
    gram_y_axis4: bool
    zx: bool
    z_mul: bool
    ymul_slabs: tuple

    def folded_axes(self):
        xz = self.xz == "fold" or self.lattice_feed or self.ss == "fused"
        return tuple(a for a, used in (("x", xz or self.gram_x == "fold" or self.plane_yx == "fold"), ("y", self.plane_yx == "fold"), ("z", xz)) if used)


def stage_forms(nx, ny, nz, opts=None):
    sw = switches(None) if opts is None else opts
    fold, fused = sw["fold"], (nx, nz) in XZ2D_SHAPES and sw["fused_xz"]
    folds = lambda a, b: fold and a == b and a in XZ2D_FOLD_N
    pair = (nx, nz) == (32, 32) and (64, 32) in XZ2D_SHAPES and ny % 2 == 0 and sw["fused_xz"]
    quad = pair and ny % 4 == 0 and fold and 64 in XZ2D_FOLD_N and sw["quad"]
    xz = "fold" if (fused and folds(nx, nz)) else "fused" if fused else "quad" if quad else "pair" if pair else "gemm"
    axis4 = lambda n: n in SPECTRAL_AXIS_N and half_integer(n) and sw["axis_mfma"]
    dense_y = ny in TOEPLITZ_NY and sw["dense_y"]
    y = "spectrum" if not dense_y else "mfma" if (ny in SPECTRAL_Y_NY and sw["y_mfma"]) else "toeplitz"
    y_two_term = "y2t" if ny in TOEPLITZ_Y2T_NY else "add" if ny in TOEPLITZ_ADD_NY else "separate"
    fused_ss = xz == "fold" and dense_y
    zx = nx == ny == nz == 64 and folds(ny, nx) and sw["z_fused"]
    return Forms(xz=xz, x_axis4=axis4(nx), y=y, y_two_term=y_two_term, y3t=y == "mfma" and ny in SPECTRAL_Y3T_NY,
                 y2s=fused_ss and y_two_term == "y2t" and sw["y2s"], fold=fold, ss="fused" if fused_ss else "stored", lattice_feed=fused_ss and ny >= 3,
                 plane_yx="fold" if folds(ny, nx) else "fused" if (ny, nx) in XZ2D_SHAPES else "gemm",
                 gram_x="fold" if folds(nx, nz) else "plain" if (nx, nz) == (64, 64) else "fold_lamdot" if (fold and nz <= 128) else "gemm",
                 gram_y_axis4=axis4(ny), zx=zx, z_mul=zx and sw["z_mul"], ymul_slabs=tuple(k for m, k in YMUL_SHAPES if m == 2 * ny))


def _pad(v, m):
    return (int(v) + m - 1) // m * m


def shard_columns(n_pad, world, rank):
    units = n_pad // PAD_N
    return units * rank // world * PAD_N, units * (rank + 1) // world * PAD_N


@dataclass(frozen=True)
class Route:
    spectral: bool
    family: str
    rows: bool
    single: bool
    exchange: bool
    exchange_without_rows: bool
    operators: str
    kernels: tuple
    note: str
    ak_bytes: int = 0
    rows_mandatory: bool = False
    switches: tuple = ()
    forms: object = None

    def opt(self, name):
        return dict(self.switches).get(name, True)

    def opts(self):
        return dict(switches(None), **dict(self.switches))

    def describe(self):
        k = dict(self.kernels)
        return "%s/%s xz=%s y=%s gram=%s ss=%s%s" % ("spectral" if self.spectral else "dense", self.family, k["xz"], k["y"], k["gram"],
# ... 77 lines not shown
```

geobo_amd/spectral.py:

```python
import math
import os

import numpy as np
import torch

from . import hip, plan
from .plan import INTEGER_BASIS_N, half_integer

F64 = hip.F64
SLACK = 4096


def base_modes(n):
    assert n % 4 == 0
    q = n // 4
    modes = [("cos", 0), ("mid", n // 2), ("cos", q), ("sin", q)]
    for om in range(1, q):
        modes += [("cos", om), ("sin", om), ("cos", n // 2 - om), ("sin", n // 2 - om)]
    return modes


def half_modes(n):
    assert n % 4 == 0
    modes = []
# ... 205 lines not shown
            jy, jx = A.jy[a:a + R], A.jx[a:a + R]
            hit = self._pool_tabs[key] = (torch.from_numpy(pool_order(jy, jx)).to(self.device), pool_distinct_planes(self.ny, jy, jx))
        return hit

    def _ystage_pooled(self, A, R, tabs, outs, y0, y1):
        ny, C, Cp = self.ny, self.Px * self.Pz, self.Cp
        order, distinct = self._pool_batch(A, R)
        a = A.r0
        fn = lambda: hip.spectral_y_lattice(ny, C, R, A.pool, A.row_off[a:], A.edge[a * 2 * Cp:], 2 * Cp, order, tabs, outs, y0, y1, plane=Cp)
        name = "kernel:toeplitz_y" if len(tabs) >= 2 else "kernel:toeplitz_y_single"
        return self._launch(name, 8.0 * C * (distinct + R * len(tabs) * (y1 - y0)), R, self.y_stage_flop(1, len(tabs), y1 - y0), fn)

    dense_y = property(lambda self: self.forms.y != "spectrum")
    y_mfma = property(lambda self: self.forms.y == "mfma")
    fused_xz = property(lambda self: self.forms.xz in ("fold", "fused"))

    def _ystage(self, R, src, tabs, outs, y0, y1, accumulate=False):
        ny, C, plane = self.ny, self.Px * self.Pz, self.Cp
        if self.y_mfma and (ny > 64 or not accumulate) and (ny <= 64 or 2 * (y1 - y0) >= ny):
            fn = lambda: hip.spectral_y(ny, C, R, src, tabs, outs, y0, y1, plane=plane, accumulate=accumulate)
        else:
            fn = lambda: hip.toeplitz_y(ny, C, R, src, tabs, outs, y0, y1, plane=plane, accumulate=accumulate)
        name = "kernel:toeplitz_y" if len(tabs) >= 2 or ny > 64 else "kernel:toeplitz_y_single"
        return self._launch(name, 8.0 * R * C * (ny + (2 if accumulate else 1) * len(tabs) * (y1 - y0)), R, self.y_stage_flop(1, len(tabs), y1 - y0), fn)

    def _launch(self, name, nbytes, rows, flop, fn):
        if self.kernel_timer is None:
            return fn()
        return self.kernel_timer(name, nbytes, fn, valu=rows * flop[1], flop=rows * flop[0])

    def _join(self, specs, gens, R, ylo, yhi, y2s=None, squaring=False):
        ny, C, Cp, meet = self.ny, self.Px * self.Pz, self.Cp, self.forms.y_two_term
        nb = len(gens[0])
        outs = [self.buf(("S", "S1", "S2")[i], R * (yhi - ylo) * Cp) for i in range(nb)]
        if isinstance(specs[0], PooledRows):
            for i in range(0, nb, 2):
                self._ystage_pooled(specs[0], R, gens[0][i:i + 2], outs[i:i + 2], ylo, yhi)
            return outs, []
        if len(specs) == 1:
            self._ystage(R, specs[0], gens[0], outs, ylo, yhi)
            return outs, []
        assert (ylo, yhi) == (0, ny)
        (sg, sm), (gg, gm) = specs, gens
        y3t = self.forms.y3t and not squaring
        if meet == "y2t" and nb == 2:
            if y2s is not None:
                y2s_fn = hip.spectral_y2s if self.y_mfma else hip.toeplitz_y2s
                name, fn = "kernel:toeplitz_y2s", lambda: y2s_fn(ny, C, R, sg, sm, y2s[0], y2s[1], y2s[2], outs, plane=Cp)
            else:
                name, fn = "kernel:toeplitz_y2t", lambda: hip.toeplitz_y2t(ny, C, R, sg, sm, gg, gm, outs, plane=Cp)
            self._launch(name, 8.0 * R * C * 4 * ny, R, self.y_stage_flop(2, 2, shared=y2s is not None), fn)
            return outs, None
        if meet == "add" and y3t:
            fn = lambda: hip.spectral_y3t(ny, C, R, sg, sm, gg, gm, outs, plane=Cp)
            self._launch("kernel:toeplitz_y", 8.0 * R * C * ny * (2 + nb), R, self.y_stage_flop(2, nb), fn)
            return outs, []
        self._ystage(R, sg, gg, outs, ylo, yhi)
        if meet == "add":
            self._ystage(R, sm, gm, outs, ylo, yhi, accumulate=True)
            return outs, []
        outs2 = [self.buf(("Sb", "S1b")[i], R * ny * Cp) for i in range(nb)]
        self._ystage(R, sm, gm, outs2, ylo, yhi)
        return outs, outs2

    def _rows_spectrum(self, A, r0, R, out_name):
        if isinstance(A, PooledRows):
            return A.rows(r0)
        if isinstance(A, ConvolvedRows):
            return A.rows(r0).spectrum(self, R, out_name)
        if isinstance(A, LatticeRows):
            return self.forward_zx(A.rows(r0), R, self.G, out_name=out_name)
        return self.forward_zx(A[r0:], R, self.G, src_row_stride=A.stride(0), out_name=out_name)

    def _drive(self, batches, terms, sink, ylo, yhi, y2s=None, squaring=False):
        P_c = len(terms[0][2])
        for r0, R, nt in batches:
            specs = [self._rows_spectrum(A, r0 - first, R, name) for (A, first, _), name in zip(terms[:nt], ("T2", "T2b"))]
            step = 2 if squaring or (nt == 2 and self.forms.y_two_term == "y2t") else 3
            for j in range(0, P_c, step):
                js = range(j, min(j + step, P_c))
                tabs = y2s[1:] if y2s is not None and y2s[0] == j else None
                sink(r0, R, js, *self._join(specs, [[g[jj] for jj in js] for _, _, g in terms[:nt]], R, ylo, yhi, tabs, squaring))

    def _store(self, slabs, ylo, yhi):
        def sink(r0, R, js, outs, _):
            for i, jj in enumerate(js):
                self.backward_xz(outs[i], R, ylo, yhi, [(ya, yb, o[jj][r0:], o[jj].stride(0)) for ya, yb, o in slabs])
        return sink

    def buf(self, name, n):
        b = self._bufs.get(name)
        if b is None or b.numel() < n + SLACK:
            b = self._bufs[name] = _buf(n, self.device)
        return b

    def _paired(self, Mx, rows, cols):
        key = (Mx.data_ptr(), rows, cols)
        m2 = self._pairs.get(key)
        if m2 is None:
            m2 = torch.zeros((2 * rows, 2 * cols), dtype=Mx.dtype, device=Mx.device)
            m2[:rows, :cols] = Mx[:rows, :cols]
            m2[rows:, cols:] = Mx[:rows, :cols]
            self._pairs[key] = m2
        return m2

    def forward_zx(self, src, R, M, src_row_stride=None, out_name="T2"):
        nx, ny, nz, Px, Pz, Cp = self.nx, self.ny, self.nz, self.Px, self.Pz, self.Cp
        xz, analysis = self.forms.xz, M is self.G
        lds = self.N if src_row_stride is None else int(src_row_stride)
        t2 = self.buf(out_name, R * ny * Cp)
        if isinstance(src, LatticeRows):
            assert self.forms.lattice_feed and analysis
            hip.xz2d_fold_lattice(nx, R, ny, src.Q, src.row_off[src.r0:], src.q_plane, src.edge[src.r0:], src.edge.stride(0),
                                  self.F["x"], self.F["z"], t2, ny * Cp, Cp)
        elif xz == "fold" and analysis:
            hip.xz2d_fold(False, nx, R, ny, src, lds, nx * nz, self.F["x"], self.F["z"], t2, ny * Cp, Cp)
        elif xz in ("fold", "fused"):
            hip.xz2d(False, nx, nz, R, ny, src, lds, nx * nz, M["x"], M["z"], t2, ny * Cp, Cp)
        elif xz == "quad" and analysis:
            hip.xz2d_fold_quad(False, nx, R, ny // 4, src, lds, nx * nz, self.Fq, self.Fq, t2, ny * Cp, Cp)
        elif xz in ("quad", "pair"):
            hip.xz2d(False, 2 * nx, nz, R, ny // 2, src, lds, 2 * nx * nz, self._paired(M["x"], Px, nx), M["z"], t2, ny * Cp, 2 * Cp)
        else:
            fold = self.forms.fold and analysis
            t1 = self.buf("T1", R * ny * nx * Pz)
            hip.axis_pass(fold, False, False, hip.pad_n(ny * nx), hip.pad_n(Pz), nz, src, nz, lds, M["z"], nz, 0, t1, Pz, ny * nx * Pz, ny * nx, Pz, R)
            if self.forms.x_axis4 and analysis and Pz % 16 == 0:
                hip.spectral_axis(False, nx, Pz, Pz, Pz, nx * Pz, Px * Pz, R * ny, t1, t2)
            else:
                hip.axis_pass(fold, True, False, hip.pad_n(Px), hip.pad_n(Pz), nx, M["x"], nx, 0, t1, Pz, nx * Pz, t2, Pz, Px * Pz, Px, Pz, R * ny)
        return t2

    def forward(self, src, R, M, out_name="T3", src_row_stride=None):
        ny, Px, Py, Pz = self.ny, self.Px, self.Py, self.Pz
        t2 = self.forward_zx(src, R, M, src_row_stride)
        t3 = self.buf(out_name, R * self.P3)
        hip.gemm_batched(True, hip.pad_n(Py), hip.pad_n(Px * Pz), ny, M["y"], ny, 0, t2, Px * Pz, ny * Px * Pz, t3, Px * Pz,
                         self.P3, Py, Px * Pz, R)
        return t3

    def backward(self, spec, R, y0, y1, out, ldo):
        Px, Py, Pz = self.Px, self.Py, self.Pz
        slab = y1 - y0
        gyt = self.GT["y"][y0:]
        u2 = self.buf("U2", R * slab * Px * Pz)
        hip.gemm_batched(True, hip.pad_n(slab), hip.pad_n(Px * Pz), Py, gyt, Py, 0, spec, Px * Pz, self.P3, u2, Px * Pz,
                         slab * Px * Pz, slab, Px * Pz, R)
        self.backward_xz(u2, R, y0, y1, [(y0, y1, out, ldo)])

    def backward_xz(self, u2, R, ylo, yhi, targets):
        nx, nz, Px, Pz, Cp = self.nx, self.nz, self.Px, self.Pz, self.Cp
        Ly, xz = yhi - ylo, self.forms.xz
        whole = lambda k: all((yb - ya) % k == 0 for ya, yb, _, _ in targets)
        if xz == "fold":
            for ya, yb, out, ldo in targets:
                hip.xz2d_fold(True, nx, R, yb - ya, u2[(ya - ylo) * Cp:], Ly * Cp, Cp, self.F["x"], self.F["z"], out, ldo, nx * nz)
        elif xz == "fused":
            for ya, yb, out, ldo in targets:
                hip.xz2d(True, nx, nz, R, yb - ya, u2[(ya - ylo) * Cp:], Ly * Cp, Cp, self.GT["x"], self.GT["z"], out, ldo, nx * nz)
        elif xz == "quad" and whole(4):
            for ya, yb, out, ldo in targets:
                hip.xz2d_fold_quad(True, nx, R, (yb - ya) // 4, u2[(ya - ylo) * Cp:], Ly * Cp, Cp, self.Fq, self.Fq, out, ldo, nx * nz)
        elif xz in ("quad", "pair") and whole(2):
            for ya, yb, out, ldo in targets:
                hip.xz2d(True, 2 * nx, nz, R, (yb - ya) // 2, u2[(ya - ylo) * Cp:], Ly * Cp, 2 * Cp,
                         self._paired(self.GT["x"], nx, Px), self.GT["z"], out, ldo, 2 * nx * nz)
        else:
            fold = self.forms.fold
            u1 = self.buf("U1", R * Ly * nx * Pz)
            if self.forms.x_axis4 and Pz % 16 == 0:
                hip.spectral_axis(True, nx, Pz, Pz, Pz, Px * Pz, nx * Pz, R * Ly, u2, u1)
            else:
                hip.axis_pass(fold, True, True, hip.pad_n(nx), hip.pad_n(Pz), Px, self.GT["x"], Px, 0, u2, Pz, Px * Pz, u1, Pz, nx * Pz, nx, Pz, R * Ly)
            for ya, yb, out, ldo in targets:
                slab = yb - ya
                hip.axis_pass(fold, False, True, hip.pad_n(slab * nx), hip.pad_n(nz), Pz, u1[(ya - ylo) * nx * Pz:], Pz, Ly * nx * Pz,
                              self.GT["z"], Pz, 0, out, nz, ldo, slab * nx, nz, R)

    def flops(self, rows, nblocks, slab, fwd_planes=None):
        nx, ny, nz, Px, Py, Pz = self.nx, self.ny, self.nz, self.Px, self.Py, self.Pz
        pn = hip.pad_n
        fwd = 2.0 * (ny * nx * pn(Pz) * nz + ny * pn(Px) * pn(Pz) * nx)
        bwd = 2.0 * (slab * pn(nx) * pn(Pz) * Px + pn(slab * nx) * pn(nz) * Pz)
        xz = self.forms.xz
        if xz == "gemm" and self.forms.fold:
            fwd, bwd = 0.5 * fwd, 0.5 * bwd
        elif xz == "quad":
            fwd = 0.25 * ny * (64.0 * 64 * 128 + 128.0 * 64 * 128)
            bwd = 0.25 * slab * (128.0 * 128 * 64 + 64.0 * 128 * 64)
        elif xz == "pair":
            fwd += 2.0 * ny * Px * Pz * nx
            bwd += 2.0 * slab * nx * Pz * Px
        elif xz == "fold":
            fwd = 2.0 * ny * (0.5 * nx * pn(Pz) * nz + 0.25 * pn(Px) * pn(Pz) * nx)
            bwd = 0.25 * bwd
        if not self.dense_y:
            fwd += 2.0 * pn(Py) * Px * Pz * ny
            bwd += 2.0 * pn(slab) * Px * Pz * Py
        if fwd_planes is not None:
            fwd *= float(fwd_planes) / (rows * ny)
        return rows * (fwd + nblocks * bwd + (self.y_stage_flop(1, nblocks, slab)[0] if self.dense_y else 0.0))

    def y_stage_flop(self, terms, nblocks, slab=None, shared=False):
        ny, C = self.ny, self.Px * self.Pz
        if self.y_mfma and (ny <= 64 or slab is None or 2 * slab >= ny):
            valu = C * ny * (4.0 * terms + (7.0 * nblocks if terms == 1 else 10.0 * nblocks))
            return C * 1.0 * ny * ny * (terms + nblocks) + valu, valu
        outs = ny if (ny <= 64 or slab is None) else (slab + 15) // 16 * 16
        nprod = terms * nblocks * (0.75 if shared and terms == 2 and nblocks == 2 else 1.0)
        f = 2.0 * ny * outs * C * nprod
        return f, f

    def flops_valu(self, rows, nblocks, slab=None):
        return rows * self.y_stage_flop(1, nblocks, slab)[1] if self.dense_y else 0.0

    def eigenvalues(self, table_mirrored, toeplitz_z=False):
        nx, ny, nz = self.nx, self.ny, self.nz
        T = table_mirrored[:ny * nx * 2 * nz].view(ny, nx, 2 * nz)[:, :, nz - 1:2 * nz - 1].contiguous()
        if toeplitz_z:
            assert self.dense_y and nx == ny == nz
            T = T.permute(2, 0, 1).contiguous()
        src = self.buf("Tsrc", self.N)
        src[:self.N] = T.reshape(-1)
        if self.dense_y:
            C, Cp = self.Px * self.Pz, self.Cp
            gen = self.forward_zx(src, 1, self.E, out_name="Lam")[:ny * Cp].view(ny, Cp)[:, :C].clone().view(-1)
            gen.mul_(1.0 / float(C))
            return gen
        lam = self.forward(src, 1, self.E, out_name="Lam")[:self.P3].clone()
        lam.mul_(1.0 / float(self.P3))
        return lam

    def product(self, A, Ms, lam_list, outs, y0=0, y1=None, slabs=None):
        y1 = self.ny if y1 is None else y1
        if slabs is None:
            slabs = [(y0, y1, outs)]
        N = self.N
        if isinstance(A, PooledRows):
            assert self.pool_applies() and self.dense_y
        elif isinstance(A, LatticeRows):
            assert self.forms.lattice_feed
        else:
            assert A.stride(1) == 1 and A.stride(0) >= N and A.stride(0) % 2 == 0
        if self.dense_y:
            return self._product_dense_y(A, Ms, lam_list, slabs)
        for r0 in range(0, Ms, self.R):
            R = min(self.R, Ms - r0)
            spec = self.forward(A[r0:], R, self.G, src_row_stride=A.stride(0))
            n = R * self.P3
            j = 0
            while j < len(lam_list):
                if j + 1 < len(lam_list):
                    s0, s1 = self.buf("S", n), self.buf("S1", n)
                    hip.scale_broadcast2(spec[:n], lam_list[j], lam_list[j + 1], s0[:n], s1[:n])
                    for ya, yb, o in slabs:
                        self.backward(s0, R, ya, yb, o[j][r0:], o[j].stride(0))
                        self.backward(s1, R, ya, yb, o[j + 1][r0:], o[j + 1].stride(0))
                    j += 2
                else:
                    s0 = self.buf("S", n)
                    hip.scale_broadcast(spec[:n], lam_list[j], s0[:n])
                    for ya, yb, o in slabs:
                        self.backward(s0, R, ya, yb, o[j][r0:], o[j].stride(0))
                    j += 1

    def _product_dense_y(self, A, Ms, gens, slabs):
        ylo, yhi = min(s[0] for s in slabs), max(s[1] for s in slabs)
        batches = [(r0, min(self.R, Ms - r0), 1) for r0 in range(0, Ms, self.R)]
        self._drive(batches, [(A, 0, gens)], self._store(slabs, ylo, yhi), ylo, yhi)

    def fused_ss(self):
        return self.forms.ss == "fused"

    GENERIC_SS_SLOTS = 8

    def ss_slots(self):
        return hip.xz2d_fold_inv_ss_slots(self.nx, self.R, self.ny) if self.fused_ss() else self.GENERIC_SS_SLOTS

    def y2s_tables(self, gens_g, gens_m, pair=(0, 1), check=True):
        a, b = pair
        applies = self.forms.y2s and b == a + 1 and a % 2 == 0 and b < len(gens_g)
        if not check:
            return (a, gens_g[a] - gens_g[b], gens_g[b], gens_m[b] - gens_g[b]) if applies else None
        self.sym_residual = None
        if not applies:
            return None
        x = gens_g[b]
        den = torch.maximum(x.abs().max(), gens_m[a].abs().max())
        self.sym_residual = (x - gens_m[a]).abs().max() / den.clamp_min(torch.finfo(x.dtype).tiny)
        return (a, gens_g[a] - x, x, gens_m[b] - x)

    def reduce_ss(self, Zg, Mg, gens_g, Zm, m_first, gens_m, ss, y2s=None):
        nx, ny, N, Cp, R = self.nx, self.ny, self.N, self.Cp, self.R
        P_c = len(gens_g)
        if Zm is None:
            m_first = Mg
        one = min(m_first, Mg)
        batches = [(r0, min(R, one - r0), 1) for r0 in range(0, one, R)] + [(r0, min(R, Mg - r0), 2) for r0 in range(m_first, Mg, R)]
        if self.fused_ss():
            def square(r0, Rb, js, outs, outs2):
                for i, jj in enumerate(js):
                    second = {} if outs2 is None else dict(src2=outs2[i] if outs2 else None, in2_row=ny * Cp, r2_first=0)
                    hip.xz2d_fold_inv_ss(nx, Rb, ny, outs[i], ny * Cp, Cp, self.F["x"], self.F["z"], ss[jj], **second)
            return self._drive(batches, [(Zg, 0, gens_g), (Zm, m_first, gens_m)], square, 0, ny, y2s=y2s, squaring=True)
        stored_join = self.dense_y and self.forms.y_two_term == "add"
        for r0, Rb, nt in batches:
            vg = [self.buf("SSV%d" % jj, R * N)[:R * N].view(R, N) for jj in range(P_c)]
            vm = None
            if nt == 2 and stored_join:
                self._drive([(0, Rb, 2)], [(Zg[r0:], 0, gens_g), (Zm[r0 - m_first:], 0, gens_m)], self._store([(0, ny, vg)], 0, ny), 0, ny)
            else:
                self.product(Zg[r0:], Rb, gens_g, vg)
                if nt == 2:
                    vm = [self.buf("SSW%d" % jj, R * N)[:R * N].view(R, N) for jj in range(P_c)]
                    self.product(Zm[r0 - m_first:], Rb, gens_m, vm)
            for jj in range(P_c):
                hip.sumsq_accum(vg[jj], vm[jj] if vm else None, Rb, ss[jj].view(ss[jj].shape[0], -1))

    def has_two_term_product(self, nblocks):
        meet = self.forms.y_two_term
        return self.dense_y and ((meet == "y2t" and nblocks % 2 == 0) or meet == "add")

    def product_two_term(self, Zg, Zm, rows, gens_g, gens_m, outs, y2s=None):
        assert self.has_two_term_product(len(gens_g)) and rows <= self.R
        self._drive([(0, rows, 2)], [(Zg, 0, gens_g), (Zm, 0, gens_m)], self._store([(0, self.ny, outs)], 0, self.ny), 0, self.ny, y2s=y2s)

    def flops_ss(self, rows_one, rows_two, nblocks, shared=False):
        nx, ny, nz, Px, Pz = self.nx, self.ny, self.nz, self.Px, self.Pz
        fwd = 1.0 * ny * (nx * nz * Pz + 0.5 * Px * nx * Pz)
        inv1, inv2 = 0.5 * ny * Px * Pz * nz, 0.5 * ny * nx * Px * nz
        terms = rows_one + 2 * rows_two
        y = rows_one * self.y_stage_flop(1, nblocks)[0] + rows_two * self.y_stage_flop(2, nblocks, shared=shared)[0]
        return terms * (fwd + nblocks * inv1) + (rows_one + rows_two) * nblocks * inv2 + y

    def valu_ss(self, rows_one, rows_two, nblocks, shared=False):
        return rows_one * self.y_stage_flop(1, nblocks)[1] + rows_two * self.y_stage_flop(2, nblocks, shared=shared)[1]
```

geobo_amd/step.py:

```python
from dataclasses import dataclass, field


class Prior:

    def __init__(self, name, lengths, W, amp, deriv=None):
        self.name, self.lengths, self.W, self.amp = name, lengths, W, amp
        self.deriv = None if deriv is None else [float(v) for v in deriv]

    def terms(self, i, j):
        from .hip import kernel_id
        w, d = self.W[i][j], self.deriv
        if d is None:
            return [(kernel_id(self.name, i != j), w)]
        if i == j:
            return [(kernel_id(self.name, False, 1), w * d[j])]
        return [(kernel_id(self.name, True, 1), w * d[j]), (kernel_id(self.name, True, 2), w * d[i])]

    def table(self, eng, i, j):
        tabs = [eng._cov_table(kid, self.lengths[j], self.lengths[i], w, self.amp) for kid, w in self.terms(i, j)]
        for t in tabs[1:]:
            tabs[0].add_(t)
        return tabs[0]

    def k_block(self, eng, i, j, rows, cols, out):
        from . import hip
        terms = self.terms(i, j)
        hip.k_block(terms[0][0], rows, cols, self.lengths[j], self.lengths[i], terms[0][1], self.amp, out)
        for kid, w in terms[1:]:
            tmp = eng._workspace2d("dcov_tmp", out.shape[0], out.shape[1])
            hip.k_block(kid, rows, cols, self.lengths[j], self.lengths[i], w, self.amp, tmp)
            out.add_(tmp)
        return out

    def ak_fused(self, eng, s, j, A, xyz, nc, out):
        from . import hip
        terms = self.terms(s, j)
        hip.ak_fused(terms[0][0], A, xyz, eng.c0, nc, self.lengths[j], self.lengths[s], terms[0][1], self.amp, out)
        for kid, w in terms[1:]:
            tmp = eng._workspace2d("dak_tmp", out.shape[0], nc)
            hip.ak_fused(kid, A, xyz, eng.c0, nc, self.lengths[j], self.lengths[s], w, self.amp, tmp)
            out[:, :nc].add_(tmp)
        return out

    def ak_points(self, eng, s, j, A, q_xyz, out):
        from . import hip
        terms = self.terms(s, j)
        xyz = eng.grid_points()
        hip.ak_points(terms[0][0], A, xyz, q_xyz, self.lengths[j], self.lengths[s], terms[0][1], self.amp, out)
        for kid, w in terms[1:]:
            tmp = eng._workspace2d("dak_points_tmp", out.shape[0], out.shape[1])
            hip.ak_points(kid, A, xyz, q_xyz, self.lengths[j], self.lengths[s], w, self.amp, tmp)
            out.add_(tmp)
        return out


@dataclass
class Step:
    prior: Prior
    props: tuple
    sel_t: object
    Md: int
    M_pad: int
    noise: object = None
    ak_slot: str = "AK"
    aka_slot: str = "AkA"
    keep_signal: bool = False
    sym: bool = False
    rowpath: bool = False
    mirror: int = 0
    gens: dict = field(default_factory=dict)
    fullrows: dict = field(default_factory=dict)
```

geobo_amd/transposed.py:

```python

import torch

from . import hip
from .operators import StreamedOperator

F64 = hip.F64


class TransposedPosteriorMixin:
    def _sym_ok(self, A_g, A_m):
        if not self._zpath_static_ok():
            return False
        return (self._gram is not None and self._gram.edge_supported() and self.Ms_pad == self.nx * self.ny
                and all(self._lam.get(f) is not None and self._lam[f][0] is A for f, A in (("grav", A_g), ("magn", A_m))))

    def _assemble_AkA_sym(self, step, AkA, AK, A_g, A_m):
        gram, pl, ny, Msp, nc = self._gram, self.nx * self.nz, self.ny, self.Ms_pad, self.nc
        Md, off_d, props = step.Md, 2 * self.Ms_pad, step.props
        lam = {0: self._lam["grav"][1], 1: self._lam["magn"][1]}
        ops = {0: A_g, 1: A_m}

        def edge_cols(sp_, k, iy):
            A = ops[sp_]
            if isinstance(A, StreamedOperator):
                return A.edge[:, k * pl:(k + 1) * pl] if A.lattice is not None else A.slab_into(self._workspace2d("op_slab", Msp, pl), iy, iy + 1)
            return A[:, iy * pl:(iy + 1) * pl]

        def rows_times_AT(X, nrows, sp_, out):
            gram.gram_rows(X, nrows, lam[sp_], out, 0, ny)
            for k, iy in enumerate((0, ny - 1)):
                gram.edge_rows(X[:, iy * pl:], nrows, self._edge_spectrum(("grav", "magn")[sp_], k, edge_cols(sp_, k, iy)), out)
        blk = lambda r0, j: AK[r0:, props.index(j) * nc:(props.index(j) + 1) * nc]

        Mm = step.mirror or self.Ms

        def run():
            rows_times_AT(blk(0, 0), self.Ms, 0, AkA[0:, 0:Msp])
            rows_times_AT(blk(0, 1), self.Ms, 1, AkA[0:, Msp:2 * Msp])
            rows_times_AT(blk(Msp, 1), Mm, 1, AkA[Msp:, Msp:2 * Msp])
            hip.transpose(AkA[:Msp, Msp:2 * Msp], AkA[Msp:2 * Msp, :Msp])
            if Md:
                rows_times_AT(blk(off_d, 0), Md, 0, AkA[off_d:, 0:Msp])
                rows_times_AT(blk(off_d, 1), Md, 1, AkA[off_d:, Msp:2 * Msp])
        self._timed("aka_lattice", gram.flops(2 * self.Ms + Mm + 2 * Md, ny), run)
        if step.mirror:
            self._timed("aka_centro_fill", 0.0, lambda: hip.centro_fill(AkA[Msp:Msp + self.Ms, Msp:Msp + self.Ms], self.Ms, (self.Ms + 1) // 2))
        return self._finish_AkA(step, AkA)

    def _zpath_static_ok(self):
        if not self.route.single or self.exchange:
            return False
        self._spectral_product()
        return True

    def _zpath_ok(self, step, AK):
        return (self._zpath_static_ok() and AK is not None and AK.dtype == F64
                and all((s_, j) in step.gens for s_ in (0, 1) for j in step.props))

    def _resident_operator(self, A, func):
        if not isinstance(A, StreamedOperator):
            return A
        R = self._workspace2d("A_" + func, self.Ms_pad, self.N_pad)
        xed, yed, zed = A.axes_dev
        hip.a_sens(A.func, A.Bv, A.locd, self.nx, self.ny, self.nz, xed, yed, zed, A.mul, A.div, R, plan=A.plan, ws=A.lws)
        return R

    def _lattice_Z(self, Lview, nrows, func, A, out, zx=False, edge=None):
        gram, pl, ny = self._gram, self.nx * self.nz, self.ny
        lam = self._lam[func][1]
        hit = self._lamW.get((func, zx))
        if hit is None or hit[0] is not lam:
            hit = self._lamW[(func, zx)] = (lam, gram.transpose_tables3(lam) if zx else gram.transpose_tables(lam))
        if zx:
            gram.apply_transpose_zx(Lview, nrows, hit[1], out)
        else:
            gram.apply_transpose(Lview, nrows, hit[1], out)
        self._lattice_slabs(Lview, nrows, func, A, [out[:, iy * pl:(iy + 1) * pl] for iy in (0, ny - 1)], zx=zx, edge=edge)

    def _lattice_slabs(self, Lview, nrows, func, A, outs, zx=False, edge=None):
        gram, pl, ny = self._gram, self.nx * self.nz, self.ny
        for k, iy in enumerate((0, ny - 1)):
            if edge is not None:
                ycols = edge[k]
            elif isinstance(A, StreamedOperator) and A.lattice is not None:
                ycols = A.edge[:, k * pl:(k + 1) * pl]
            elif isinstance(A, StreamedOperator):
                ycols = A.slab_into(self._workspace2d("op_slab", self.Ms_pad, pl), iy, iy + 1)
            else:
                ycols = A[:, iy * pl:(iy + 1) * pl]
            key = (func, k)
            vt = self._edgeVt.get(key)
            if vt is None or vt[0] != ycols.data_ptr():
                vt = self._edgeVt[key] = (ycols.data_ptr(), gram.edge_eigen_t(ycols))
            gram.edge_apply_transpose(Lview, nrows, vt[1], outs[k], zx=zx)

    def _z_spectrum_ok(self):
        sp = self._spectral
        f = sp.forms
        return bool(self.z_spectrum_on and f.zx and f.z_mul and sp.fused_ss() and sp.y_mfma and f.y_two_term == "y2t")

    def _convolved_rows(self, Lview, nrows, func, A):
        from .spectral import ConvolvedRows
        gram, pl = self._gram, self.nx * self.nz
        lam = self._lam[func][1]
        hit = self._lamW.get((func, True))
        if hit is None or hit[0] is not lam:
            hit = self._lamW[(func, True)] = (lam, gram.transpose_tables3(lam))
        slab = self._workspace2d("Zslab_" + func, nrows, 2 * pl)
        self._lattice_slabs(Lview, nrows, func, A, [slab[:, k * pl:(k + 1) * pl] for k in (0, 1)], zx=True)
        return ConvolvedRows(gram, Lview, hit[1], slab)

    def _posterior_zpath(self, step, Linv, AK, u, A_g, A_m):
        props, Md, M_pad, amp = step.props, step.Md, step.M_pad, step.prior.amp
        sp, N, Msp, P_c = self._spectral, self.N, self.Ms_pad, len(props)
        nx, ny, nz = self.nx, self.ny, self.nz
        cws = self._workspace("colgemv_ws", (max(hip.colgemv_ws_doubles(M_pad, M_pad), hip.colgemv_ws_doubles(Msp, self.N_pad)),))
        w = self._timed("posterior_mean", 0.0, lambda: hip.colgemv(Linv, u, ws=cws))
        Zg = Zm = None
        zs = False
        lat = (self._gram is not None and self._gram.edge_supported() and Msp == nx * ny and self.route.opt("z_lattice")
               and all(self._lam.get(f) is not None and self._lam[f][0] is A for f, A in (("grav", A_g), ("magn", A_m))))
        if lat:
            gram = self._gram
            fl_conv, fl_slab = 3 * Msp * gram.flops(1, ny), 3 * Msp * 2 * 3 * 2.0 * 128 * 128 * 64

            zx = gram.zx_supported()
            zs = zx and self._z_spectrum_ok()
# ... 139 lines not shown
```

include/geobo_hip.h:

```cpp
#ifndef GEOBO_HIP_H
#define GEOBO_HIP_H

#include <stddef.h>
#include <stdint.h>

#ifdef __cplusplus
extern "C" {
#endif

#define GEOBO_VERSION 213


#define GEOBO_PAD_M 256
#define GEOBO_PAD_N 128

enum { GEOBO_OK = 0, GEOBO_E_ARG = -1, GEOBO_E_ALIGN = -2, GEOBO_E_LAUNCH = -3, GEOBO_E_UNSUPPORTED = -4 };

enum {
  GEOBO_K_D2 = 0,
  GEOBO_K_EXP = 1,
  GEOBO_K_EXP_X = 2,
  GEOBO_K_MATERN32 = 3,
  GEOBO_K_MATERN32_X = 4,
  GEOBO_K_SPARSE = 5,
// ... 57 lines not shown
                    const double* qx, const double* qy, const double* qz, int64_t nq_pad,
                    double l1, double l2, double w, double amp, double* out, int64_t ldo, void* stream);

int geobo_cov_table(int kernel_id, int nx, int ny, int nz, double sx, double sy, double sz, double l1, double l2,
                    double w, double amp, double* table, void* stream);
int geobo_ak_fused_grid(const double* A, int64_t Ms_pad, int64_t N_pad, int64_t lda, int nx, int ny, int nz,
                        const double* table, int64_t col0, int64_t ncols, double* AK, int64_t ldak, void* stream);

#define GEOBO_GEMM_LOWER_ONLY 1
#define GEOBO_GEMM_SMALL_TILES 2
int geobo_gemm_nt(int64_t m, int64_t n, int64_t k, double alpha, const double* X, int64_t ldx,
                  const double* Y, int64_t ldy, double beta, double* C, int64_t ldc, int lower_only, int64_t m_valid,
                  void* stream);

int64_t geobo_tile_order(int nbi, int nbj, int tm, int tn, int lower_only, int x_lower, int y_lower, int* out_host,
                         int64_t capacity);

int geobo_gemm_map(int ymode, int reduce_epilogue, int nbi, int nbj, int tm, int tn, int tri_flags, int batch, int* out);

int geobo_gemm_nt_splitk(int64_t m, int64_t n, int64_t k, int splits, const double* X, int64_t ldx, const double* Y,
                         int64_t ldy, double* C, int64_t ldc, int lower_only, int64_t m_valid, void* ws, size_t ws_bytes,
                         void* stream);

int geobo_gemm_nn(int64_t m, int64_t n, int64_t k, double alpha, const double* X, int64_t ldx,
                  const double* Y, int64_t ldy, double beta, double* C, int64_t ldc,
                  int x_lower, int y_lower, void* stream);

#define GEOBO_GEMM_X_KM 2
int geobo_gemm_batched(int y_is_kn, int64_t m, int64_t n, int64_t k, double alpha, const double* X, int64_t ldx,
                       int64_t strideX, const double* Y, int64_t ldy, int64_t strideY, double beta, double* C, int64_t ldc,
                       int64_t strideC, int64_t m_valid, int64_t n_valid, int batch, void* stream);

int geobo_gemm_fold(int y_is_kn, int inverse, int64_t m, int64_t n, int64_t k, const double* X, int64_t ldx, int64_t strideX,
                    const double* Y, int64_t ldy, int64_t strideY, double* C, int64_t ldc, int64_t strideC, int64_t m_valid,
                    int64_t n_valid, int64_t batch, void* stream);

int geobo_gemm_fold_lamdot(int64_t px, int64_t nz, int64_t k, const double* G, int64_t ldg, const double* Y, int64_t ldy, int64_t strideY,
                           const double* lam, int planes, int64_t batch0, double* out, int64_t batch, void* stream);

int geobo_scale_broadcast(const double* a, const double* b, int64_t n, int64_t nb, double* out, void* stream);
int geobo_scale_broadcast2(const double* a, const double* b0, const double* b1, int64_t n, int64_t nb, double* out0,
                           double* out1, void* stream);

int geobo_xz2d(int inverse, int nx, int nz, int64_t rows, int planes_per_row, const double* in, int64_t in_row,
               int64_t in_plane, const double* Mx, int64_t ldmx, const double* Mz, int64_t ldmz, double* out,
               int64_t out_row, int64_t out_plane, void* stream);

int geobo_xz2d_fold(int inverse, int n, int64_t rows, int planes_per_row, const double* in, int64_t in_row, int64_t in_plane,
                    const double* Fx, const double* Fz, double* out, int64_t out_row, int64_t out_plane, void* stream);

int geobo_xcorr_reduce(int nx, int nz, int64_t rows, int planes, const double* in, int64_t in_row, int64_t in_plane,
                       const double* Mx, int64_t ldmx, const double* lamT, double* out, int64_t out_row, int64_t out_plane,
                       void* stream);

int geobo_xz2d_fold_lattice(int n, int64_t rows, int planes_per_row, const double* Q, const int64_t* row_off, int64_t q_plane,
                            const double* edge, int64_t edge_row, const double* Fx, const double* Fz, double* out,
                            int64_t out_row, int64_t out_plane, void* stream);

int geobo_xz2d_fold_inv_strided(int n, int64_t rows, int planes_per_row, const double* in, int64_t in_row, int64_t in_plane,
                                const double* Fx, const double* Fz, double* out, int64_t out_row, int64_t out_plane,
                                int64_t out_rowstride, void* stream);

int geobo_xz2d_fold_inv_mul(int n, int64_t rows, int planes_per_row, const double* a, int64_t a_plane, const double* b, int64_t b_row,
                            const double* Fx, const double* Fz, double* out, int64_t out_row, int64_t out_plane,
                            int64_t out_rowstride, void* stream);

int geobo_xz2d_fold_conv_fwd(int n, int64_t rows, int planes_per_row, const double* a, int64_t a_plane, const double* b, int64_t b_row,
                             const double* slab, int64_t slab_row, const double* Fx, const double* Fz, double* out, int64_t out_row,
                             int64_t out_plane, void* stream);

int geobo_xz2d_fold_quad(int inverse, int n, int64_t rows, int groups_per_row, const double* in, int64_t in_row, int64_t in_plane,
                         const double* Fx, const double* Fz, double* out, int64_t out_row, int64_t out_plane, void* stream);

int geobo_xz2d_fold_inv_ss_slots(int n, int64_t rows, int planes_per_row);
int geobo_xz2d_fold_inv_ss(int n, int64_t rows, int planes_per_row, const double* in, int64_t in_row, int64_t in_plane,
                           const double* in2, int64_t in2_row, int64_t r2_first, const double* Fx, const double* Fz, double* ss,
                           void* stream);

int geobo_ymul(int m, int k, int64_t C, int64_t rows, const double* G, int64_t ldg, const double* in, int64_t in_row,
               double* out, int64_t out_row, void* stream);
int geobo_ymul_fold(int m, int k, int64_t C, int64_t rows, const double* G, int64_t ldg, const double* in, int64_t in_row,
                    double* out, int64_t out_row, void* stream);

int geobo_xcorr_reduce_fold(int n, int64_t rows, int planes, const double* in, int64_t in_row, int64_t in_plane,
                            const double* F, const double* lamT, double* out, int64_t out_row, int64_t out_plane, void* stream);

int geobo_toeplitz_y(int ny, int64_t C, int64_t plane, int64_t R, int nprop, const double* in, const double* tab0, const double* tab1,
                     double* out0, double* out1, int y0, int y1, void* stream);

int geobo_toeplitz_y2t(int ny, int64_t C, int64_t plane, int64_t R, const double* in_g, const double* in_m, const double* tab_g0,
                       const double* tab_g1, const double* tab_m0, const double* tab_m1, double* out0, double* out1, void* stream);

int geobo_toeplitz_y2s(int ny, int64_t C, int64_t plane, int64_t R, const double* in_g, const double* in_m, const double* tab_d0,
                       const double* tab_x, const double* tab_d1, double* out0, double* out1, void* stream);

int geobo_toeplitz_y3(int ny, int64_t C, int64_t plane, int64_t R, int nprop, const double* in, const double* const* tabs,
                      double* const* outs, int y0, int y1, void* stream);
int geobo_toeplitz_y3_add(int ny, int64_t C, int64_t plane, int64_t R, int nprop, const double* in, const double* const* tabs,
                          double* const* outs, int y0, int y1, void* stream);

int64_t geobo_spectral_y_basis_doubles(int ny);
int geobo_spectral_y_basis(int ny, double* basis, void* stream);
int geobo_spectral_y(int ny, int64_t C, int64_t plane, int64_t R, int nprop, const double* in, const double* tab0, const double* tab1,
                     double* out0, double* out1, int y0, int y1, const double* basis, void* stream);
int geobo_spectral_y2s(int ny, int64_t C, int64_t plane, int64_t R, const double* in_g, const double* in_m, const double* tab_d0,
                       const double* tab_x, const double* tab_d1, double* out0, double* out1, const double* basis, void* stream);

int geobo_spectral_y_lattice(int ny, int64_t C, int64_t plane, int64_t R, int nprop, const double* pool, const int64_t* row_off,
                             const double* edge, int64_t edge_row, const int32_t* order, const double* tab0, const double* tab1,
                             double* out0, double* out1, int y0, int y1, const double* basis, void* stream);

int geobo_spectral_y3(int ny, int64_t C, int64_t plane, int64_t R, int nprop, const double* in, const double* const* tabs,
                      double* const* outs, int y0, int y1, int accumulate, const double* basis, void* stream);

int geobo_spectral_y3t(int ny, int64_t C, int64_t plane, int64_t R, int nprop, const double* in_g, const double* in_m,
                       const double* const* tabs_g, const double* const* tabs_m, double* const* outs, const double* basis, void* stream);

int geobo_spectral_axis(int inverse, int n, int64_t C, int64_t plane_in, int64_t plane_out, int64_t item_in, int64_t item_out, int64_t items,
                        const double* in, double* out, const double* basis, int mask_ends, void* stream);

enum { GEOBO_POTRF_AUTO = 0, GEOBO_POTRF_STREAMS = 1, GEOBO_POTRF_DAG = 2 };
size_t geobo_potrf_ws_bytes(int64_t m);
int geobo_potrf_ctx_create(void** ctx);
int geobo_potrf_ctx_destroy(void* ctx);
int geobo_potrf_inv(int64_t m, double* A, int64_t ld, double* Linv, int64_t ldi, int* info, void* ws,
                    size_t ws_bytes, void* ctx, int schedule, void* stream);

int geobo_rowgemv(int64_t m, int64_t n, const double* X, int64_t ld, const double* v, double* out, void* stream);

int geobo_sumsq_accum(int64_t rows, int64_t n, const double* a, int64_t lda, const double* b, int64_t ldb, int slots, double* ss,
                      int64_t ld_ss, void* stream);

int geobo_lamdot_z(int64_t batch, int planes, int px, int nz, const double* D, const double* lam, double* out, void* stream);

int geobo_centro_fill(double* B, int64_t ld, int64_t n, int64_t r0, void* stream);
int geobo_transpose(int64_t rows, int64_t cols, const double* src, int64_t lds, double* dst, int64_t ldd, void* stream);
int geobo_mirror_rows(double* X, int64_t ld, int64_t m, int64_t r0, int64_t nb, int nz, void* stream);
size_t geobo_mirror_dev_ws_bytes(void);
int geobo_mirror_dev(const double* a, int64_t lda, const double* b, int64_t ldb, int64_t rows, int nx, int nz, double* out2, void* ws,
                     size_t ws_bytes, void* stream);

size_t geobo_posterior_ws_bytes(int64_t m, int64_t ncols);
int geobo_posterior_reduce(int64_t m, int64_t ncols, const double* Linv, int64_t ldi, const double* AK, int64_t ldak,
                           const double* u, double prior_var, double* mu, double* var, int64_t m_valid, void* ws,
                           size_t ws_bytes, void* stream);

size_t geobo_kinv_dot_ws_bytes(int64_t m, int T);
int geobo_kinv_dot(int64_t m, const double* Linv, int64_t ldl, const double* alpha, int T, const double* const* G, int64_t ldg,
                   const int64_t* seg, double* out, void* ws, size_t ws_bytes, void* stream);

int geobo_trmv_stats(int64_t m, const double* Linv, int64_t ldi, const double* y, const double* L, int64_t ld,
                     double* u, double* stats, void* stream);

int geobo_mfma_f64_peak(int blocks, int iters, double* out, void* stream);

int geobo_mfma_mix(int mode, int nv, int blocks, int iters, double* out, void* stream);

enum { GEOBO_RNG_PRIOR = 0, GEOBO_RNG_OBS = 1 };
#define GEOBO_FFT_INVERSE 1
#define GEOBO_FFT_IN_PAIRS 2
#define GEOBO_FFT_OUT_PAIRS 4
#define GEOBO_FFT_MAX 512

int geobo_philox_fill(int mode, uint64_t seed, uint64_t purpose, int64_t sample0, int64_t nsamples, int64_t elem0, int64_t nelem,
                      uint64_t sub, double* out, void* stream);

// ... 67 lines not shown
```

Measured before the change: 2.469 million.

## Fuse gram x-analysis into inverse xz fold and feed AkA from spectral rows

Adds a mode to the inverse xz fold kernel that also computes the x-direction Gram analysis for interior y planes while the data is still in registers and LDS. It can optionally skip storing the full AK block for those planes. A new gram_yz MFMA kernel reduces that intermediate over y and z against the eigenvalues to produce S. The AkA assembly then uses a cheaper back_rows pass instead of recomputing the full gram_rows from AK. The aim is to avoid re-reading AK and redoing the forward transforms in the Gram product, at the cost of an extra GX buffer, more kernel complexity and a narrow applicability route.

```diff
diff --git a/geobo_amd/_lib.py b/geobo_amd/_lib.py
--- a/geobo_amd/_lib.py
+++ b/geobo_amd/_lib.py
@@ -63,6 +63,8 @@
     "geobo_xz2d_fold_inv_ss": (_int, [_int, _i64, _int, _dp, _i64, _i64, _dp, _i64, _i64, _dp, _dp, _dp, _dp]),
     "geobo_ymul": (_int, [_int, _int, _i64, _i64, _dp, _i64, _dp, _i64, _dp, _i64, _dp]),
     "geobo_ymul_fold": (_int, [_int, _int, _i64, _i64, _dp, _i64, _dp, _i64, _dp, _i64, _dp]),
+    "geobo_xz2d_fold_inv_gx": (_int, [_int, _i64, _int, _dp, _i64, _i64, _dp, _dp, _dp, _i64, _i64, _int, _dp, _i64, _i64, _dp]),
+    "geobo_gram_yz": (_int, [_int, _int, _i64, _dp, _i64, _i64, _dp, _i64, _dp, _dp, _i64, _i64, _dp]),
     "geobo_xcorr_reduce": (_int, [_int, _int, _i64, _int, _dp, _i64, _i64, _dp, _i64, _dp, _dp, _i64, _i64, _dp]),
     "geobo_toeplitz_y": (_int, [_int, _i64, _i64, _i64, _int, _dp, _dp, _dp, _dp, _dp, _int, _int, _dp]),
     "geobo_toeplitz_y2t": (_int, [_int, _i64, _i64, _i64, _dp, _dp, _dp, _dp, _dp, _dp, _dp, _dp, _dp]),
diff --git a/geobo_amd/csrc/xz2d.hip b/geobo_amd/csrc/xz2d.hip
--- a/geobo_amd/csrc/xz2d.hip
+++ b/geobo_amd/csrc/xz2d.hip
@@ -427,6 +427,128 @@
     b ^= 1;
   }
   if (prev_tile >= 0) store(prev, prev_tile);
+}
+
+struct GramYZArgs {
+  const double* gx; int64_t gx_row, gx_plane;
+  const double* G; int64_t ldg;
+  const double* lam;
+  double* s; int64_t s_row, s_plane;
+  int64_t R; int ny, rstep;
+};
+
+__global__ void __launch_bounds__(256, 2) gram_yz_kernel(GramYZArgs g) {
+  constexpr int NY = 64, CB = 64, TILE = NY * CB, PX = 128;
+  __shared__ __attribute__((aligned(16))) double xs[2][TILE];
+  const int tid = threadIdx.x, lane = tid & 63;
+  const int w = __builtin_amdgcn_readfirstlane(tid >> 6);
+  const int lr = lane & 15, q = lane >> 4;
+  const int bid = blockIdx.x, o = (bid & 7) * 16 + ((bid >> 3) & 15);
+  int64_t r = bid >> 7;
+  if (r >= g.R) return;
+  const int ny = g.ny;
+  double a[2][8];
+#pragma unroll
+  for (int mt = 0; mt < 2; ++mt)
+#pragma unroll
+    for (int t = 0; t < 8; ++t) {
+      const int b = 16 * w + lr, y = 2 * (4 * t + q) + mt;
+      a[mt][t] = (b < ny && y < ny) ? g.G[(int64_t)(2 * b) * g.ldg + y] : 0.0;
+    }
+  double lam[2][4][4];
+#pragma unroll
+  for (int mt = 0; mt < 2; ++mt)
+#pragma unroll
+    for (int nt = 0; nt < 4; ++nt)
+#pragma unroll
+      for (int r4 = 0; r4 < 4; ++r4) {
+        const int ky = 2 * (16 * w + q + 4 * r4) + mt;
+        lam[mt][nt][r4] = ky < 2 * ny ? g.lam[((int64_t)ky * PX + o) * CB + 16 * nt + lr] : 0.0;
+      }
+  if (ny < NY) {
+    for (int i = tid; i < 2 * TILE; i += 256) (&xs[0][0])[i] = 0.0;
+  }
+  __syncthreads();
+  const int dma_h = lane >> 5;
+  const int64_t dma_lane = (int64_t)dma_h * g.gx_plane + ((lane & 31) ^ (((2 * w + dma_h) & 3) << 3)) * 2;
+  auto stage = [&](int64_t r_, int b) {
+    const double* src = g.gx + r_ * g.gx_row + (int64_t)o * CB + dma_lane;
+#pragma unroll
+    for (int i = 0; i < 8; ++i) {
+      const int pr = w + 4 * i;
+      if (2 * pr < ny)
+        __builtin_amdgcn_global_load_lds((glb_ptr_t)(src + (int64_t)(2 * pr) * g.gx_plane), (lds_ptr_t)(&xs[b][2 * pr * CB]), 16, 0, 0);
+    }
+  };
+  stage(r, 0);
+  int b = 0;
+  const bool h8 = lr & 8, h4 = lr & 4, h2 = lr & 2;
+  const int kyo = 2 * (16 * w + q + 4 * (lr >> 2)) + ((lr >> 1) & 1);
+  for (; r < g.R; r += g.rstep) {
+    __builtin_amdgcn_s_waitcnt(vmcnt_imm(0));
+    __builtin_amdgcn_s_barrier();
+    const int64_t nxt = r + g.rstep;
+    if (nxt < g.R) stage(nxt, b ^ 1);
+    v4d acc[2][4];
+#pragma unroll
+    for (int mt = 0; mt < 2; ++mt)
+#pragma unroll
+      for (int nt = 0; nt < 4; ++nt) acc[mt][nt] = (v4d){0., 0., 0., 0.};
+    unsigned xe[4], xo[4];
+#pragma unroll
+    for (int nt = 0; nt < 4; ++nt) {
+      xe[nt] = (unsigned)(uintptr_t)(lds_ptr_t)&xs[b][(2 * q) * CB + 16 * (nt ^ ((2 * q) & 3)) + lr];
+      xo[nt] = (unsigned)(uintptr_t)(lds_ptr_t)&xs[b][(2 * q + 1) * CB + 16 * (nt ^ ((2 * q + 1) & 3)) + lr];
+    }
+    double be[2][4], bo[2][4];
+#pragma unroll
+    for (int nt = 0; nt < 4; ++nt) {
+      asm volatile("ds_read_b64 %0, %1" : "=v"(be[0][nt]) : "v"(xe[nt]));
+      asm volatile("ds_read_b64 %0, %1" : "=v"(bo[0][nt]) : "v"(xo[nt]));
+    }
+#pragma unroll
+    for (int t = 0; t < 8; ++t) {
+      if (t + 1 < 8) {
+#pragma unroll
+        for (int nt = 0; nt < 4; ++nt) {
+          asm volatile("ds_read_b64 %0, %1 offset:%2" : "=v"(be[(t + 1) & 1][nt]) : "v"(xe[nt]), "n"(8 * (t + 1) * CB * 8));
+          asm volatile("ds_read_b64 %0, %1 offset:%2" : "=v"(bo[(t + 1) & 1][nt]) : "v"(xo[nt]), "n"(8 * (t + 1) * CB * 8));
+        }
+        asm volatile("s_waitcnt lgkmcnt(8)" : "+v"(be[t & 1][0]), "+v"(be[t & 1][1]), "+v"(be[t & 1][2]), "+v"(be[t & 1][3]),
+                     "+v"(bo[t & 1][0]), "+v"(bo[t & 1][1]), "+v"(bo[t & 1][2]), "+v"(bo[t & 1][3]));
+      } else {
+        asm volatile("s_waitcnt lgkmcnt(0)" : "+v"(be[t & 1][0]), "+v"(be[t & 1][1]), "+v"(be[t & 1][2]), "+v"(be[t & 1][3]),
+                     "+v"(bo[t & 1][0]), "+v"(bo[t & 1][1]), "+v"(bo[t & 1][2]), "+v"(bo[t & 1][3]));
+      }
+#pragma unroll
+      for (int nt = 0; nt < 4; ++nt) {
+        acc[0][nt] = __builtin_amdgcn_mfma_f64_16x16x4f64(a[0][t], be[t & 1][nt], acc[0][nt], 0, 0, 0);
+        acc[1][nt] = __builtin_amdgcn_mfma_f64_16x16x4f64(a[1][t], bo[t & 1][nt], acc[1][nt], 0, 0, 0);
+      }
+    }
+    double v[8];
+#pragma unroll
+    for (int r4 = 0; r4 < 4; ++r4)
+#pragma unroll
+      for (int mt = 0; mt < 2; ++mt) {
+        double sum = 0.0;
+#pragma unroll
+        for (int nt = 0; nt < 4; ++nt) {
+          const double d = mt ? acc[0][nt][r4] - acc[1][nt][r4] : acc[0][nt][r4] + acc[1][nt][r4];
+          sum = __builtin_fma(d, lam[mt][nt][r4], sum);
+        }
+        v[2 * r4 + mt] = sum;
+      }
+    double k4[4], k2[2];
+#pragma unroll
+    for (int i = 0; i < 4; ++i) k4[i] = (h8 ? v[4 + i] : v[i]) + __shfl_xor(h8 ? v[i] : v[4 + i], 8);
+#pragma unroll
+    for (int i = 0; i < 2; ++i) k2[i] = (h4 ? k4[2 + i] : k4[i]) + __shfl_xor(h4 ? k4[i] : k4[2 + i], 4);
+    double k1 = (h2 ? k2[1] : k2[0]) + __shfl_xor(h2 ? k2[0] : k2[1], 2);
+    k1 += __shfl_xor(k1, 1);
+    if (!(lr & 1) && kyo < 2 * ny) g.s[r * g.s_row + (int64_t)kyo * g.s_plane + o] = k1;
+    b ^= 1;
+  }
 }
 
 }
@@ -490,6 +612,22 @@
   return hipGetLastError() == hipSuccess ? GEOBO_OK : GEOBO_E_LAUNCH;
 }
 
+extern "C" int geobo_gram_yz(int n, int ny, int64_t rows, const double* gx, int64_t gx_row, int64_t gx_plane, const double* G, int64_t ldg,
+                             const double* lam, double* s, int64_t s_row, int64_t s_plane, void* stream) {
+  if (!gx || !G || !lam || !s) return GEOBO_E_ARG;
+  if (((uintptr_t)gx & 15) || ((uintptr_t)G & 7) || ((uintptr_t)lam & 7) || ((uintptr_t)s & 7)) return GEOBO_E_ARG;
+  if ((gx_row & 1) || (gx_plane & 1) || gx_plane < 2 * (int64_t)n * n || gx_row < 0 || s_plane < 2 * n || s_row < 0) return GEOBO_E_ARG;
+  if (ny < 2 || (ny & 1) || ldg < ny) return GEOBO_E_ARG;
+  if (n != 64 || ny > 64) return GEOBO_E_UNSUPPORTED;
+  if (rows <= 0) return GEOBO_OK;
+  GramYZArgs g;
+  g.gx = gx; g.gx_row = gx_row; g.gx_plane = gx_plane; g.G = G; g.ldg = ldg; g.lam = lam; g.s = s; g.s_row = s_row; g.s_plane = s_plane;
+  g.R = rows; g.ny = ny;
+  g.rstep = rows < 4 ? (int)rows : 4;
+  hipLaunchKernelGGL(gram_yz_kernel, dim3((unsigned)(128 * g.rstep)), dim3(256), 0, (hipStream_t)stream, g);
+  return hipGetLastError() == hipSuccess ? GEOBO_OK : GEOBO_E_LAUNCH;
+}
+
 extern "C" int geobo_ymul_fold(int m, int k, int64_t C, int64_t rows, const double* G, int64_t ldg, const double* in, int64_t in_row,
                                double* out, int64_t out_row, void* stream) {
   if (!G || !in || !out) return GEOBO_E_ARG;
diff --git a/geobo_amd/csrc/xz2d_fold.hip b/geobo_amd/csrc/xz2d_fold.hip
--- a/geobo_amd/csrc/xz2d_fold.hip
+++ b/geobo_amd/csrc/xz2d_fold.hip
@@ -26,8 +26,12 @@
   const double* Fz;
   const double* Fx;
   int ppr; int64_t nplanes;
-  const int64_t* row_off; const double* edge; int64_t edge_row;
-  const double* in2; int64_t in2_row, r2_first; double* ss;
+  const int64_t* row_off; const double* edge;
+  union { int64_t edge_row; int64_t gx_all; };
+  const double* in2;
+  union { int64_t in2_row; int64_t gx_row; };
+  union { int64_t r2_first; int64_t gx_plane; };
+  union { double* ss; double* gx; };
   int in_rowB, in_halfB, in_botB;
   int out_rowB, out_halfB, out_botB;
 };
@@ -350,7 +354,8 @@
 
 template <int N, int MODE, bool QUAD>
 __global__ void __launch_bounds__(256, 2) xz_fold_inv_kernel(FoldArgs g) {
-  constexpr bool RED = MODE == 1, MUL = MODE == 2;
+  constexpr bool RED = MODE == 1, MUL = MODE == 2, GX = MODE == 3;
+  static_assert(!(GX && QUAD), "the x analysis rides on the radix-4 form");
   const int in_rowB = QUAD ? g.in_rowB : 2 * N * 8, in_halfB = QUAD ? g.in_halfB : N * 8, in_botB = QUAD ? g.in_botB : 0;
   const int out_halfB = QUAD ? g.out_halfB : N * 4, out_botB = QUAD ? g.out_botB : 0;
   constexpr bool R4 = !QUAD;
@@ -623,8 +628,56 @@
         sso[m] += od * od;
       }
     } else {
+      bool ak_store = true, drained = false;
+      if constexpr (GX) {
+        const int y = (int)(p % g.ppr);
+        const bool interior = y != 0 && y != g.ppr - 1;
+        ak_store = g.gx_all || !interior;
+        if (interior) {
+          v4d gc[4], gs[4];
+#pragma unroll
+          for (int rho = 0; rho < 4; ++rho) gc[rho] = gs[rho] = (v4d){0., 0., 0., 0.};
+          unsigned fxT = (unsigned)(uintptr_t)(lds_ptr_t)mxf + q * 256 + ((lr ^ q) << 4);
+          asm volatile("" : "+v"(fxT));
+          static_for<0, 4>([&](auto cc) {
+            constexpr int c = decltype(cc)::value;
+            v2d f[4];
+            const unsigned fa4 = fxT ^ (unsigned)(c << 6);
+#pragma unroll
+            for (int rho = 0; rho < 4; ++rho)
+              asm volatile("ds_read_b128 %0, %1 offset:%2" : "=v"(f[rho]) : "v"(fa4), "n"(c * 1024 + rho * 4096));
+            static_for<0, 4>([&](auto rr) {
+              constexpr int rho = decltype(rr)::value;
+              asm volatile("s_waitcnt lgkmcnt(%1)" : "+v"(f[rho]) : "n"(3 - rho));
+              gc[rho] = __builtin_amdgcn_mfma_f64_16x16x4f64(f[rho].x, xe[rho >> 1][rho & 1][c], gc[rho], 0, 0, 0);
+              gs[rho] = __builtin_amdgcn_mfma_f64_16x16x4f64(f[rho].y, xe[rho >> 1][rho & 1][c], gs[rho], 0, 0, 0);
+            });
+          });
+          __builtin_amdgcn_s_waitcnt(vmcnt_imm(0));
+          drained = true;
+          double* const gp = g.gx + (p / g.ppr) * g.gx_row + y * g.gx_plane + (int64_t)(8 * q) * N + 4 * lr + w;
+          const double r2 = 1.4142135623730951;
+#pragma unroll
+          for (int r = 0; r < 4; ++r) {
+            const bool w0 = r == 0 && q == 0;
+            const double u0 = gc[0][r] + gc[2][r], u1 = gc[0][r] - gc[2][r], v0 = gc[1][r] + gc[3][r], v1 = gc[1][r] - gc[3][r];
+            const double ws = gs[0][r] + gs[2][r], wd = gs[0][r] - gs[2][r], z0 = gs[1][r] + gs[3][r], z1 = gs[1][r] - gs[3][r];
+            const double a0 = r2 * gs[0][r], a2 = r2 * gs[2][r];
+            double* const op8 = gp + (int64_t)(32 * r) * N;
+            op8[0 * N] = u0 + v0;
+            op8[1 * N] = u0 - v0;
+            op8[2 * N] = w0 ? u1 + v1 : ws + z0;
+            op8[3 * N] = w0 ? u1 - v1 : ws - z0;
+            op8[4 * N] = w0 ? a0 + z1 : u1 + z1;
+            op8[5 * N] = w0 ? a0 - z1 : u1 - z1;
+            op8[6 * N] = w0 ? a2 + z0 : v1 - wd;
+            op8[7 * N] = w0 ? a2 - z0 : -wd - v1;
+          }
+        }
+      }
       if constexpr (MUL) fetch(curA, curB, 2);
-      else __builtin_amdgcn_s_waitcnt(vmcnt_imm(0));
+      else if (!(GX && drained)) __builtin_amdgcn_s_waitcnt(vmcnt_imm(0));
+      if (ak_store) {
       int64_t ors = g.out_rs;
       asm volatile("" : "+s"(ors));
       double* const op = g.out + (p / g.ppr) * g.out_row + (p % g.ppr) * g.out_plane + 2 * q * ors +
@@ -646,6 +699,7 @@
           om[(int64_t)(2 * j0) * ors] = ev[r];
           om[(int64_t)(2 * j0 + 1) * ors] = od[r];
         }
+      }
       }
     }
   }
@@ -1237,6 +1291,25 @@
   return launch_inv<64, 0>(g, (hipStream_t)stream);
 }
 
+extern "C" int geobo_xz2d_fold_inv_gx(int n, int64_t rows, int planes_per_row, const double* in, int64_t in_row, int64_t in_plane,
+                                      const double* Fx, const double* Fz, double* out, int64_t out_row, int64_t out_plane,
+                                      int store_all, double* gx, int64_t gx_row, int64_t gx_plane, void* stream) {
+  if (!in || !out || !Fx || !Fz || !gx) return GEOBO_E_ARG;
+  if (rows <= 0 || planes_per_row <= 0) return GEOBO_OK;
+  if (gx_plane < 2 * (int64_t)n * n || gx_row < planes_per_row * gx_plane) return GEOBO_E_ARG;
+  if ((in_row & 1) || (in_plane & 1) || ((uintptr_t)in & 15) || ((uintptr_t)Fx & 15) || ((uintptr_t)Fz & 15) || ((uintptr_t)out & 7) ||
+      ((uintptr_t)gx & 7))
+    return GEOBO_E_ALIGN;
+  if (n != 64) return GEOBO_E_UNSUPPORTED;
+  FoldArgs g;
+  g.in = in; g.in_row = in_row; g.in_plane = in_plane; g.out = out; g.out_row = out_row; g.out_plane = out_plane; g.out_rs = n;
+  g.Fz = Fz; g.Fx = Fx; g.ppr = planes_per_row; g.nplanes = rows * planes_per_row;
+  g.row_off = nullptr; g.edge = nullptr; g.in2 = nullptr;
+  g.gx = gx; g.gx_row = gx_row; g.gx_plane = gx_plane; g.gx_all = store_all ? 1 : 0;
+  dense_inv(g, 64);
+  return launch_inv<64, 3>(g, (hipStream_t)stream);
+}
+
 extern "C" int geobo_xz2d_fold_inv_mul(int n, int64_t rows, int planes_per_row, const double* a, int64_t a_plane, const double* b,
                                        int64_t b_row, const double* Fx, const double* Fz, double* out, int64_t out_row,
                                        int64_t out_plane, int64_t out_rowstride, void* stream) {
diff --git a/geobo_amd/engine.py b/geobo_amd/engine.py
--- a/geobo_amd/engine.py
+++ b/geobo_amd/engine.py
@@ -6,7 +6,7 @@
 import torch
 
 from . import geometry, hip
-from .plan import COLUMN_FORM_MAX_BYTES, engine_options, plan_route
+from .plan import COLUMN_FORM_MAX_BYTES, engine_options, feed_options, gram_gx_route, plan_route
 from .columnform import ColumnExchangeMixin
 from .rowform import RowFormMixin
 from .operators import StreamedOperator
@@ -26,6 +26,19 @@
 F64 = hip.F64
 
 
+class _GramFeed:
+
+    def __init__(self, gram, lams, S, store_all=True):
+        self.gram, self.lams, self.S, self.store_all = gram, lams, S, store_all
+        self.ld = gram.Py * gram.Px
+
+    def rows(self, jj, r0, R, GX):
+        self.gram.gx_rows(GX, R, self.lams[jj], self.S[jj][r0 * self.ld:])
+
+    def at(self, r0):
+        return _GramFeed(self.gram, self.lams, [S[r0 * self.ld:] for S in self.S], self.store_all)
+
+
 class CholeskyError(RuntimeError):
 
     def __init__(self, info):
@@ -40,6 +53,11 @@
 
 class _LastStep(dict):
     complete = None
+
+    @staticmethod
+    def chain(fills):
+        fills = list(fills)
+        return (lambda: [f() for f in fills] and None) if fills else None
 
     def __getitem__(self, key):
         if key == "AK_partial" and self.complete is not None:
@@ -136,6 +154,7 @@
         self.route = plan_route(self.nx, self.ny, self.nz, world=world, rank=rank, assembly=assembly, operators=operators, method=method,
                                 env=env)
         self.options = engine_options(env)
+        self.feed = feed_options(env)
         self.use_spectral = self.route.spectral
         if method == "spectral" and not self.use_spectral:
             raise ValueError("spectral method needs grid extents % 16 == 0 and column shards on y-slab boundaries")
@@ -537,24 +556,27 @@
         if self.exchange:
             return self._assemble_AK_spectral_exchange(step, AK)
         for s_, A in ((0, A_g), (1, A_m)):
-            lams, outs = [], []
+            lams, outs, blocks = [], [], []
             for jj, j in enumerate(props):
                 gen = sp.eigenvalues(step.prior.table(self, s_, j))
                 step.gens[(s_, j)] = gen
                 if step.sym and (s_, j) not in ((0, 0), (0, 1), (1, 1)):
                     continue
                 lams.append(gen)
+                blocks.append(j)
                 outs.append(AK[s_ * self.Ms_pad:s_ * self.Ms_pad + self.Ms, jj * nc:(jj + 1) * nc])
             pooled = (isinstance(A, StreamedOperator) and A.lattice is not None and A.lattice.jy is not None and not self.f32
                       and sp.pool_applies())
             Mrun = step.mirror if (s_ == 1 and step.mirror) else self.Ms
             fl = sp.flops(Mrun, len(lams), y1 - y0, fwd_planes=sp.pool_planes(Mrun) if pooled else None)
             fv = sp.flops_valu(Mrun, len(lams), y1 - y0)
-            if not self.f32 and not isinstance(A, StreamedOperator):
-                self._timed("spectral_product", fl, lambda: sp.product(A, Mrun, lams, [o[:Mrun] for o in outs], y0, y1), valu=fv)
-                continue
-
-            def batches():
+            feed = self._gram_feed(step, s_, blocks) if (y0, y1) == (0, self.ny) else None
+            if feed is not None:
+                fl += self._gram.flops_gx(Mrun * len(lams))
+
+            def product_rows(gx, A=A, lams=lams, outs=outs, Mrun=Mrun, pooled=pooled):
+                if not self.f32 and not isinstance(A, StreamedOperator):
+                    return sp.product(A, Mrun, lams, [o[:Mrun] for o in outs], y0, y1, gx=gx)
                 Rb = sp.R
                 abuf = self._op_rows_buffer() if isinstance(A, StreamedOperator) else None
                 scr = [self._workspace2d("ak_rows64_%d" % jj, Rb, nc) for jj in range(len(lams))] if self.f32 else None
@@ -568,11 +590,24 @@
                     else:
                         src = A.rows_into(abuf, r0, R) if abuf is not None else A[r0:r0 + R]
                     dst = [b[:R] for b in scr] if scr is not None else [o[r0:r0 + R] for o in outs]
-                    sp.product(src, R, lams, dst, y0, y1)
+                    sp.product(src, R, lams, dst, y0, y1, gx=gx and gx.at(r0))
                     if scr is not None:
                         for jj in range(len(lams)):
                             hip.convert(dst[jj], outs[jj][r0:r0 + R])
-            self._timed("spectral_product", fl, batches, valu=fv)
+            self._timed("spectral_product", fl, lambda: product_rows(feed), valu=fv)
+            if feed is not None and not feed.store_all:
+                step.ak_fill.append(lambda fill=product_rows: fill(None))
+
+    def _gram_feed(self, step, s_, blocks):
+        gram, sp = self._gram, self._spectral_product()
+        funcs = ("grav", "magn")
+        if not (gram_gx_route(self.feed, self.route.family, step.sym, self.f32, self.world, self.exchange, self.nx, self.ny, self.nz, sp.forms)
+                and gram is not None and gram.gx_applies() and sp.gx_applies() and all(j in (0, 1) and self._lam.get(funcs[j]) is not None for j in blocks)):
+            return None
+        S = [self._workspace("gram_S_%d%d" % (s_, j), (self.Ms * gram.Py * gram.Px,)) for j in blocks]
+        for j, Sj in zip(blocks, S):
+            step.gram_S[(s_, j)] = Sj
+        return _GramFeed(gram, [self._lam[funcs[j]][1] for j in blocks], S, store_all=False)
 
     def _edge_spectrum(self, func, k, ycols):
         key = (func, k)
@@ -871,9 +906,11 @@
         whole = AK is not None and not step.sym
         self.last = _LastStep(L=L, Linv=Linv, u=u, AK=AK if whole else None, AK_partial=None if whole else AK, AK_complete=whole, props=props,
                               sel=sel, ops=(A_g, A_m), step=step, mv=mv, uu=out.get("uu"), logdet=out.get("logdet"))
+        fills = list(step.ak_fill)
         if step.mirror and step.mirror < self.Ms:
             jj, nc, Msp, Mm = props.index(1), self.nc, self.Ms_pad, step.mirror
-            self.last.complete = lambda: hip.mirror_rows(AK[Msp:Msp + self.Ms, jj * nc:jj * nc + self.N], self.Ms, Mm, self.nx * self.ny, self.nz)
+            fills.append(lambda: hip.mirror_rows(AK[Msp:Msp + self.Ms, jj * nc:jj * nc + self.N], self.Ms, Mm, self.nx * self.ny, self.nz))
+        self.last.complete = _LastStep.chain(fills)
         return out
 
     def _derivative_gram(self, A_g, A_m, sel_t, prior, slot):
diff --git a/geobo_amd/hip.py b/geobo_amd/hip.py
--- a/geobo_amd/hip.py
+++ b/geobo_amd/hip.py
@@ -577,6 +577,19 @@
     fn, name = (lib.geobo_ymul_fold, "geobo_ymul_fold") if fold else (lib.geobo_ymul, "geobo_ymul")
     _lib.check(fn(int(m), int(k), int(C), int(rows), _p(_chk(G, "G")), int(G.stride(0)), _p(_chk(src, "src")), int(in_row),
                   _p(_chk(out, "out")), int(out_row), _stream()), name)
+
+
+def xz2d_fold_inv_gx(n, rows, ppr, src, in_row, in_plane, Fx, Fz, out, out_row, out_plane, store_all, gx, gx_row, gx_plane):
+    lib = require_gpu()
+    _lib.check(lib.geobo_xz2d_fold_inv_gx(int(n), int(rows), int(ppr), _p(_chk(src, "src")), int(in_row), int(in_plane), _p(_chk(Fx, "Fx")),
+                                          _p(_chk(Fz, "Fz")), _p(_chk(out, "out")), int(out_row), int(out_plane), 1 if store_all else 0,
+                                          _p(_chk(gx, "gx")), int(gx_row), int(gx_plane), _stream()), "geobo_xz2d_fold_inv_gx")
+
+
+def gram_yz(n, ny, rows, gx, gx_row, gx_plane, G, lam_oz, s, s_row, s_plane):
+    lib = require_gpu()
+    _lib.check(lib.geobo_gram_yz(int(n), int(ny), int(rows), _p(_chk(gx, "gx")), int(gx_row), int(gx_plane), _p(_chk(G, "G")), int(G.stride(0)),
+                                 _p(_chk(lam_oz, "lam_oz")), _p(_chk(s, "s")), int(s_row), int(s_plane), _stream()), "geobo_gram_yz")
 
 
 def xcorr_reduce(nx, nz, rows, planes, src, in_row, in_plane, Mx, lam, out, out_row, out_plane):
diff --git a/geobo_amd/lattice_gram.py b/geobo_amd/lattice_gram.py
--- a/geobo_amd/lattice_gram.py
+++ b/geobo_amd/lattice_gram.py
@@ -238,6 +238,27 @@
         zsum = 0.0 if self.fast(nx, ny, nz) else 2.0 * Py * Px * nz
         hy = 0.5 if (f and Ly in self.sp.forms.ymul_slabs) else 1.0
         return rows * (2.0 * (hy * hip.pad_n(Py) * nx * nz * Ly + h * Py * Px * nx * nz + hb * (ny * Py * Px + ny * nx * Px)) + zsum)
+
+    def gx_applies(self):
+        return self.sp.forms.gram_x == "fold" and self.nx == 64 and self.nz == 64 and self.ny % 2 == 0 and 4 <= self.ny <= 64
+
+    def gx_rows(self, GX, nrows, lam, S):
+        nx, ny, nz, Px, Py = self.nx, self.ny, self.nz, self.Px, self.Py
+        hip.gram_yz(nx, ny, nrows, GX, ny * Px * nz, Px * nz, self.Gy0, self.lam_oz(lam), S, Py * Px, Px)
+
+    def back_rows(self, S, nrows, out):
+        for r0 in range(0, nrows, self.R):
+            R = min(self.R, nrows - r0)
+            self._plane_yx(True, R, S[r0 * self.Py * self.Px:], self.Py * self.Px, out[r0:], out.stride(0))
+
+    def flops_gx(self, rows):
+        nx, ny, nz, Px, Py = self.nx, self.ny, self.nz, self.Px, self.Py
+        return rows * 2.0 * (0.25 * (ny - 2) * Px * nx * nz + 0.5 * hip.pad_n(Py) * 64 * Px * nz)
+
+    def flops_back(self, rows):
+        nx, ny, Px, Py = self.nx, self.ny, self.Px, self.Py
+        hb = 0.25 if self.sp.forms.gram_x == "fold" else 1.0
+        return rows * 2.0 * hb * (ny * Py * Px + ny * nx * Px)
 
     def gram_rows(self, X, nrows, lam, out, y0=0, y1=None):
         nx, ny, nz, Px, Py = self.nx, self.ny, self.nz, self.Px, self.Py
diff --git a/geobo_amd/plan.py b/geobo_amd/plan.py
--- a/geobo_amd/plan.py
+++ b/geobo_amd/plan.py
@@ -50,6 +50,21 @@
 def engine_options(env=None):
     env = {} if env is None else env
     return EngineOptions(**{k: parse(env[var]) if var in env else default for k, (var, default, parse) in ENGINE_OPTIONS.items()})
+
+
+FEED_OPTIONS = {"gram_gx": ("GEOBO_GRAM_GX", True, _on)}
+FeedOptions = make_dataclass("FeedOptions", [(k, type(d)) for k, (_, d, _p) in FEED_OPTIONS.items()], frozen=True)
+
+
+def feed_options(env=None):
+    env = {} if env is None else env
+    return FeedOptions(**{k: parse(env[var]) if var in env else default for k, (var, default, parse) in FEED_OPTIONS.items()})
+
+
+def gram_gx_route(opts, family, sym, f32, world, exchange, nx, ny, nz, forms):
+    return bool(opts.gram_gx and sym and family == "single" and not f32 and world == 1 and not exchange
+                and nx == 64 and nz == 64 and ny % 2 == 0 and 4 <= ny <= 64
+                and forms.xz == "fold" and forms.gram_x == "fold" and forms.y != "spectrum")
 
 
 def half_integer(n):
diff --git a/geobo_amd/spectral.py b/geobo_amd/spectral.py
--- a/geobo_amd/spectral.py
+++ b/geobo_amd/spectral.py
@@ -311,11 +311,32 @@
                 tabs = y2s[1:] if y2s is not None and y2s[0] == j else None
                 sink(r0, R, js, *self._join(specs, [[g[jj] for jj in js] for _, _, g in terms[:nt]], R, ylo, yhi, tabs, squaring))
 
-    def _store(self, slabs, ylo, yhi):
+    def _store(self, slabs, ylo, yhi, gx=None):
         def sink(r0, R, js, outs, _):
             for i, jj in enumerate(js):
-                self.backward_xz(outs[i], R, ylo, yhi, [(ya, yb, o[jj][r0:], o[jj].stride(0)) for ya, yb, o in slabs])
+                if gx is None:
+                    self.backward_xz(outs[i], R, ylo, yhi, [(ya, yb, o[jj][r0:], o[jj].stride(0)) for ya, yb, o in slabs])
+                    continue
+                nx, ny, nz, Cp, gp = self.nx, self.ny, self.nz, self.Cp, self.Px * self.nz
+                o = slabs[0][2][jj]
+                GX = self.gx_buffer()
+                hip.xz2d_fold_inv_gx(nx, R, ny, outs[i], ny * Cp, Cp, self.F["x"], self.F["z"], o[r0:], o.stride(0), nx * nz, gx.store_all,
+                                     GX, ny * gp, gp)
+                gx.rows(jj, r0, R, GX)
         return sink
+
+    def gx_applies(self):
+        return self.forms.xz == "fold" and self.dense_y and self.nx == 64 and self.nz == 64 and self.ny >= 3
+
+    def gx_buffer(self):
+        gp = self.Px * self.nz
+        b = self.buf("GX", self.R * self.ny * gp)
+        if getattr(self, "_gx_zeroed", None) != b.data_ptr():
+            v = b[:self.R * self.ny * gp].view(self.R, self.ny, gp)
+            v[:, 0] = 0.0
+            v[:, self.ny - 1] = 0.0
+            self._gx_zeroed = b.data_ptr()
+        return b
 
     def buf(self, name, n):
         b = self._bufs.get(name)
@@ -460,7 +481,7 @@
         lam.mul_(1.0 / float(self.P3))
         return lam
 
-    def product(self, A, Ms, lam_list, outs, y0=0, y1=None, slabs=None):
+    def product(self, A, Ms, lam_list, outs, y0=0, y1=None, slabs=None, gx=None):
         y1 = self.ny if y1 is None else y1
         if slabs is None:
             slabs = [(y0, y1, outs)]
@@ -471,8 +492,10 @@
             assert self.forms.lattice_feed
         else:
             assert A.stride(1) == 1 and A.stride(0) >= N and A.stride(0) % 2 == 0
+        if gx is not None:
+            assert self.gx_applies() and len(slabs) == 1 and (slabs[0][0], slabs[0][1]) == (0, self.ny)
         if self.dense_y:
-            return self._product_dense_y(A, Ms, lam_list, slabs)
+            return self._product_dense_y(A, Ms, lam_list, slabs, gx)
         for r0 in range(0, Ms, self.R):
             R = min(self.R, Ms - r0)
             spec = self.forward(A[r0:], R, self.G, src_row_stride=A.stride(0))
@@ -493,10 +516,10 @@
                         self.backward(s0, R, ya, yb, o[j][r0:], o[j].stride(0))
                     j += 1
 
-    def _product_dense_y(self, A, Ms, gens, slabs):
+    def _product_dense_y(self, A, Ms, gens, slabs, gx=None):
         ylo, yhi = min(s[0] for s in slabs), max(s[1] for s in slabs)
         batches = [(r0, min(self.R, Ms - r0), 1) for r0 in range(0, Ms, self.R)]
-        self._drive(batches, [(A, 0, gens)], self._store(slabs, ylo, yhi), ylo, yhi)
+        self._drive(batches, [(A, 0, gens)], self._store(slabs, ylo, yhi, gx), ylo, yhi)
 
     def fused_ss(self):
         return self.forms.ss == "fused"
diff --git a/geobo_amd/step.py b/geobo_amd/step.py
--- a/geobo_amd/step.py
+++ b/geobo_amd/step.py
@@ -70,3 +70,5 @@
     mirror: int = 0
     gens: dict = field(default_factory=dict)
     fullrows: dict = field(default_factory=dict)
+    gram_S: dict = field(default_factory=dict)
+    ak_fill: list = field(default_factory=list)
diff --git a/geobo_amd/transposed.py b/geobo_amd/transposed.py
--- a/geobo_amd/transposed.py
+++ b/geobo_amd/transposed.py
@@ -26,8 +26,11 @@
                 return A.edge[:, k * pl:(k + 1) * pl] if A.lattice is not None else A.slab_into(self._workspace2d("op_slab", Msp, pl), iy, iy + 1)
             return A[:, iy * pl:(iy + 1) * pl]
 
-        def rows_times_AT(X, nrows, sp_, out):
-            gram.gram_rows(X, nrows, lam[sp_], out, 0, ny)
+        def rows_times_AT(X, nrows, sp_, out, S=None):
+            if S is not None:
+                gram.back_rows(S, nrows, out)
+            else:
+                gram.gram_rows(X, nrows, lam[sp_], out, 0, ny)
             for k, iy in enumerate((0, ny - 1)):
                 gram.edge_rows(X[:, iy * pl:], nrows, self._edge_spectrum(("grav", "magn")[sp_], k, edge_cols(sp_, k, iy)), out)
         blk = lambda r0, j: AK[r0:, props.index(j) * nc:(props.index(j) + 1) * nc]
@@ -35,14 +38,16 @@
         Mm = step.mirror or self.Ms
 
         def run():
-            rows_times_AT(blk(0, 0), self.Ms, 0, AkA[0:, 0:Msp])
-            rows_times_AT(blk(0, 1), self.Ms, 1, AkA[0:, Msp:2 * Msp])
-            rows_times_AT(blk(Msp, 1), Mm, 1, AkA[Msp:, Msp:2 * Msp])
+            rows_times_AT(blk(0, 0), self.Ms, 0, AkA[0:, 0:Msp], S.get((0, 0)))
+            rows_times_AT(blk(0, 1), self.Ms, 1, AkA[0:, Msp:2 * Msp], S.get((0, 1)))
+            rows_times_AT(blk(Msp, 1), Mm, 1, AkA[Msp:, Msp:2 * Msp], S.get((1, 1)))
             hip.transpose(AkA[:Msp, Msp:2 * Msp], AkA[Msp:2 * Msp, :Msp])
             if Md:
                 rows_times_AT(blk(off_d, 0), Md, 0, AkA[off_d:, 0:Msp])
                 rows_times_AT(blk(off_d, 1), Md, 1, AkA[off_d:, Msp:2 * Msp])
-        self._timed("aka_lattice", gram.flops(2 * self.Ms + Mm + 2 * Md, ny), run)
+        S = step.gram_S
+        nfed = sum(self.Ms if s_ == 0 else Mm for s_, _ in S)
+        self._timed("aka_lattice", gram.flops(2 * self.Ms + Mm + 2 * Md - nfed, ny) + gram.flops_back(nfed), run)
         if step.mirror:
             self._timed("aka_centro_fill", 0.0, lambda: hip.centro_fill(AkA[Msp:Msp + self.Ms, Msp:Msp + self.Ms], self.Ms, (self.Ms + 1) // 2))
         return self._finish_AkA(step, AkA)
diff --git a/include/geobo_hip.h b/include/geobo_hip.h
--- a/include/geobo_hip.h
+++ b/include/geobo_hip.h
@@ -163,6 +163,12 @@
 int geobo_ymul_fold(int m, int k, int64_t C, int64_t rows, const double* G, int64_t ldg, const double* in, int64_t in_row,
                     double* out, int64_t out_row, void* stream);
 
+int geobo_xz2d_fold_inv_gx(int n, int64_t rows, int planes_per_row, const double* in, int64_t in_row, int64_t in_plane,
+                           const double* Fx, const double* Fz, double* out, int64_t out_row, int64_t out_plane, int store_all,
+                           double* gx, int64_t gx_row, int64_t gx_plane, void* stream);
+int geobo_gram_yz(int n, int ny, int64_t rows, const double* gx, int64_t gx_row, int64_t gx_plane, const double* G, int64_t ldg,
+                  const double* lam, double* s, int64_t s_row, int64_t s_plane, void* stream);
+
 int geobo_xcorr_reduce_fold(int n, int64_t rows, int planes, const double* in, int64_t in_row, int64_t in_plane,
                             const double* F, const double* lamT, double* out, int64_t out_row, int64_t out_plane, void* stream);
 
```

Result: faster. 2.523 million, median of 6 (+2.2%).
